# axruff/cuda-flow3d

Hardware: AMD Instinct MI355X
Metric: Mvoxels/s full pyramid solve (higher is better)
Workload: dtype f32; 1 GPU; 512^3 synthetic translated-Gaussian float32 pair (BASELINE config 4), full coarse-to-fine pyramid (40 levels x 40 outer x 5 inner, alpha 7.5, median 5^3, Gaussian sigma 2), frames resident in HBM (value = device-resident rate); parallelism=1 GPU

## Files before the change

### cuda-flow3d_amd/__init__.py

```python
import atexit
import contextlib
import ctypes as C
import os
import weakref

import numpy as np

_HERE = os.path.dirname(os.path.abspath(__file__))
_LIBDIR = os.environ.get("F3D_LIBDIR") or os.path.join(_HERE, "lib")

DEFAULT_PARAMS = dict(
    warp_levels_count=40, warp_scale_factor=0.95, outer_iterations_count=40, inner_iterations_count=5,
    equation_alpha=7.5, equation_smoothness=0.001, equation_data=0.001, median_radius=5, gaussian_sigma=2.0,
)


class F3dError(RuntimeError):
    pass


class Size4(C.Structure):
    _fields_ = [("width", C.c_size_t), ("height", C.c_size_t), ("depth", C.c_size_t), ("pitch", C.c_size_t)]


# ... 187 lines not shown
            raise
        fn.argtypes = args
        fn.restype = C.c_int
    _hip = L
    if hasattr(L, "f3d_crash_maps_enable"):
        _arm_crash_maps(L)
    return L


def _arm_crash_maps(L):
    path = os.environ.get("F3D_CRASH_MAPS")
    if not path:
        blob = " ".join(os.environ.get(k, "") for k in ("LD_PRELOAD", "ROCP_TOOL_LIBRARIES", "HSA_TOOLS_LIB"))
        if "rocprof" not in blob:
            return
        base = os.environ.get("F3D_OUT") or os.getcwd()
        path = os.path.join(base, f"f3d_crash_maps.{os.getpid()}.txt")
    L.f3d_crash_maps_enable(path.encode())


def host():
    global _host
    if _host is not None:
        return _host
    hip()
    L = _load("libf3d_host.so")
    pp = C.POINTER(FlowParams)
    sig = {
        "f3d_flow_create": [C.POINTER(C.c_void_p)], "f3d_flow_initialize": [C.c_void_p, _sz, _sz, _sz],
        "f3d_flow_compute": [C.c_void_p, _fp, _fp, pp, C.c_int, _fp, _fp, _fp],
        "f3d_flow_upload": [C.c_void_p, _fp, _fp],
        "f3d_flow_compute_resident": [C.c_void_p, pp, C.c_int, _fp],
        "f3d_flow_download": [C.c_void_p, _fp, _fp, _fp],
        "f3d_flow_container": [C.c_void_p, C.POINTER(Size4)], "f3d_flow_destroy": [C.c_void_p],
        "f3d_flow_set_level_stats": [C.c_void_p, C.c_int], "f3d_flow_level_stat_count": [C.c_void_p, C.POINTER(_sz)],
        "f3d_flow_level_stat": [C.c_void_p, _sz, C.POINTER(LevelStat)],
        "f3d_flow_final_residual": [C.c_void_p, C.POINTER(C.c_double), C.POINTER(C.c_double)],
        "f3d_flow_trajectory_begin": [C.c_void_p], "f3d_flow_trajectory_append": [C.c_void_p],
        "f3d_flow_trajectory_download": [C.c_void_p, _fp, _fp, _fp, C.POINTER(C.c_ulonglong)],
        "f3d_flow_trajectory_end": [C.c_void_p],
        "f3d_flow_strain_compute": [C.c_void_p, C.c_int, C.c_uint, C.POINTER(_fp), C.POINTER(StrainStats)],
        "f3d_flow_strain_end": [C.c_void_p],
        "f3d_flow_principal_compute": [C.c_void_p, C.c_int, C.c_uint, C.POINTER(_fp), C.POINTER(PrincipalStats)],
        "f3d_flow_principal_end": [C.c_void_p],
        "f3d_flow_inverse_compute": [C.c_void_p, C.c_int, C.c_uint, C.c_float, C.POINTER(_fp), C.POINTER(InverseStats)],
        "f3d_flow_inverse_end": [C.c_void_p],
        "f3d_flow_match_compute": [C.c_void_p, C.c_int, C.c_uint, C.c_uint, C.c_float, C.POINTER(_fp), C.POINTER(CorrelationStats)],
        "f3d_flow_match_end": [C.c_void_p],
        "f3d_motion_solve": [C.POINTER(MotionSums), C.c_int, C.POINTER(MotionFit)],
        "f3d_flow_motion_compute": [C.c_void_p, C.c_int, C.c_int, C.c_float, C.POINTER(_fp), C.POINTER(MotionFit),
                                    C.POINTER(MotionResidual)],
        "f3d_flow_motion_end": [C.c_void_p],
        "f3d_op_create": [C.POINTER(C.c_void_p), C.c_char_p], "f3d_op_initialize": [C.c_void_p, C.POINTER(Size4)],
        "f3d_op_execute": [C.c_void_p, C.POINTER(C.c_char_p), C.POINTER(C.c_void_p), _sz],
        "f3d_op_execute_batch": [C.c_void_p, C.POINTER(C.c_char_p), C.POINTER(C.c_void_p), C.POINTER(_sz), _sz],
        "f3d_op_set_slab": [C.c_void_p, _slabp], "f3d_op_destroy": [C.c_void_p],
        "f3d_level_geometry": [_sz, _sz, _sz, C.c_float, C.c_int, C.POINTER(Size4), _fp, _fp, _fp],
        "f3d_gaussian_taps": [C.c_float, _fp, _sz, C.POINTER(_sz)],
        "f3d_raw_read_u8": [C.c_char_p, _sz, _sz, _sz, _fp], "f3d_raw_read_f32": [C.c_char_p, _sz, _sz, _sz, _fp],
        "f3d_raw_write_u8": [C.c_char_p, _fp, _sz, _sz, _sz], "f3d_raw_write_f32": [C.c_char_p, _fp, _sz, _sz, _sz],
        "f3d_vtk_write_flow": [C.c_char_p, _fp, _fp, _fp, _sz, _sz, _sz],
        "f3d_synth_pair": [_sz, _sz, _sz, _fp, _fp],
        "f3d_synth_planes": [_sz, _sz, _sz, _sz, _sz, _fp, _fp, _fp],
        "f3d_slabflow_create": [C.POINTER(C.c_void_p), C.c_int, C.POINTER(C.c_int), C.c_int, C.c_int],
        "f3d_slabflow_initialize": [C.c_void_p, _sz, _sz, _sz],
        "f3d_slabflow_compute": [C.c_void_p, _fp, _fp, pp, _fp, _fp, _fp],
        "f3d_slabflow_upload": [C.c_void_p, _fp, _fp],
        "f3d_slabflow_compute_resident": [C.c_void_p, pp, _fp],
        "f3d_slabflow_download": [C.c_void_p, _fp, _fp, _fp],
        "f3d_slabflow_overlapped_iterations": [C.c_void_p, C.POINTER(_sz)],
        "f3d_slabflow_batched_exchanges": [C.c_void_p, C.POINTER(_sz)],
        "f3d_slabflow_gathered_warps": [C.c_void_p, C.POINTER(_sz)],
        "f3d_slabflow_stage_exchanges": [C.c_void_p, C.POINTER(_sz)],
        "f3d_slabflow_set_exchange_per_stage": [C.c_void_p, C.c_int],
        "f3d_slabflow_destroy": [C.c_void_p],
        "f3d_plan_owned": [C.c_int, C.c_int, C.c_int, C.POINTER(C.c_int), C.POINTER(C.c_int)],
        "f3d_plan_exchange": [C.c_int] * 5 + [C.POINTER(C.c_int)] * 5 + [C.c_int],
        "f3d_plan_resample_source": [C.c_int] * 4 + [C.POINTER(C.c_int)] * 2,
        "f3d_volume_wrap": [C.POINTER(C.c_void_p), _fp, _sz, _sz, _sz], "f3d_volume_destroy": [C.c_void_p],
        "f3d_op_solve_p_last": [C.c_void_p, C.POINTER(C.c_int), C.POINTER(C.c_int), C.POINTER(C.c_int), C.POINTER(_sz), C.POINTER(C.c_int)],
        "f3d_op_solve_p_fused_weights": [C.c_void_p, C.POINTER(C.c_int)],
        "f3d_plan_solve_piecemeal": [_sz, _sz, _sz, C.c_int, C.c_int, C.c_int, C.c_int, C.c_int] + [C.POINTER(C.c_int)] * 5,
        "f3d_pflow_create": [C.POINTER(C.c_void_p)], "f3d_pflow_initialize": [C.c_void_p, _sz, _sz, _sz],
        "f3d_pflow_compute": [C.c_void_p, _fp, _fp, _sz, _sz, _sz, pp, C.c_int, _fp, _fp, _fp, _fp],
        "f3d_pflow_stats": [C.c_void_p, C.POINTER(_sz), C.POINTER(_sz), C.POINTER(_sz)], "f3d_pflow_destroy": [C.c_void_p],
        "f3d_pflow_set_resident": [C.c_void_p, C.c_int], "f3d_pflow_set_full_pipeline": [C.c_void_p, C.c_int], "f3d_pflow_originals_on_device": [C.c_void_p, C.POINTER(C.c_int)],
        "f3d_pflow_operator_seconds": [C.c_void_p, C.POINTER(C.c_double)],
        "f3d_pflow_levels_registered_inside": [C.c_void_p, C.POINTER(_sz)],
        "f3d_pflow_levels_with_constants_on_device": [C.c_void_p, C.POINTER(_sz)],
        "f3d_host_shutdown": [],
    }
    for name, args in sig.items():
        try:
            fn = getattr(L, name)
        except AttributeError:
            if os.environ.get("F3D_LIBDIR"):
                continue
            raise
        fn.argtypes = args
        fn.restype = C.c_int
    L.f3d_flow_default_params.argtypes = [pp]
    L.f3d_flow_default_params.restype = None
    L.f3d_op_name.argtypes = [C.c_void_p]
    L.f3d_op_name.restype = C.c_char_p
    L.f3d_max_warp_level.argtypes = [_sz, _sz, _sz, C.c_float]
    L.f3d_max_warp_level.restype = _sz
    L.f3d_volume_object.argtypes = [C.c_void_p]
    L.f3d_volume_object.restype = C.c_void_p
    L.f3d_volume_data.argtypes = [C.c_void_p]
    L.f3d_volume_data.restype = C.c_void_p
    L.f3d_piecemeal_budget_bytes.argtypes = []
    L.f3d_piecemeal_budget_bytes.restype = _sz
    if hasattr(L, "f3d_host_last_error"):
        L.f3d_host_last_error.argtypes = []
        L.f3d_host_last_error.restype = C.c_char_p
    _host = L
    return L


def shutdown():
    HostVolume.release_all()
    if _host is not None:
        _host.f3d_host_shutdown()
    elif _hip is not None and _hip.f3d_is_initialized():
        _hip.f3d_comm_destroy()
        _hip.f3d_shutdown()


atexit.register(shutdown)


def check(status, what="f3d call"):
    if status != 0:
        msg = hip().f3d_last_error()
        raise F3dError(f"{what} failed: {msg.decode() if msg else 'status %d' % status}")


def _host_check(status, what):
    if status != 0:
        msg = host().f3d_host_last_error()
        raise F3dError(f"{what} failed: {msg.decode() if msg else 'status %d' % status}")


def _entry(name, argtypes, what):
    try:
        fn = getattr(hip(), name)
    except AttributeError:
        raise F3dError(f"{os.path.join(_LIBDIR, 'libf3d_hip.so')} has no {name}: this device library cannot {what}") from None
    fn.argtypes = argtypes
    fn.restype = C.c_int
    return fn


def _compose_entry():
    return _entry("f3d_compose_flow", [_dp] * 6 + [_sz] * 3 + [C.POINTER(C.c_ulonglong)], "compose flows into a trajectory")


def _strain_entry():
    return _entry("f3d_flow_strain", [_dp] * 3 + [_dpp, C.c_uint] + [_sz] * 3 + [C.POINTER(StrainStats)], "compute strain fields")


def _principal_entry():
    return _entry("f3d_principal_strain", [_dp] * 3 + [_dpp, C.c_uint] + [_sz] * 3 + [C.POINTER(PrincipalStats)],
                  "compute principal strains")


def _inverse_entry():
    return _entry("f3d_invert_displacement", [_dp] * 7 + [_sz] * 3 + [C.c_uint, C.c_float, C.POINTER(InverseStats)],
                  "invert displacements")


def _carry_entry():
    return _entry("f3d_carry_field", [_dp] * 5 + [_sz] * 3 + [C.c_uint, C.POINTER(C.c_ulonglong)],
                  "carry fields through a displacement")


def _correlation_entry():
    return _entry("f3d_local_correlation", [_dp] * 2 + [_dpp, C.c_uint, C.c_uint, C.c_float] + [_sz] * 3 + [C.POINTER(CorrelationStats)],
                  "compute the local correlation of two volumes")


def _motion_entry():
    what = "fit or remove the motion of a displacement"
    return (_entry("f3d_motion_sums", [_dp] * 4 + [C.c_float] + [_sz] * 3 + [C.POINTER(MotionSums)], what),
            _entry("f3d_remove_motion", [_dp] * 6 + [C.POINTER(MotionFit)] + [_sz] * 3 + [C.POINTER(MotionResidual)], what))


def _mask(fields, groups, what):
    if isinstance(fields, str):
        fields = fields.split(",")
    mask = 0
    for f in fields:
        if f not in groups:
            raise ValueError(f"unknown {what} group {f!r} (one of {', '.join(groups)})")
        mask |= groups[f]
    if not mask:
        raise ValueError(f"no {what} group selected")
    return mask


def _source(source):
    src = {"flow": 0, "trajectory": 1}.get(source)
    if src is None:
        raise ValueError(f"source must be 'flow' or 'trajectory', not {source!r}")
    return src


@contextlib.contextmanager
def _on_device(volumes, mismatch):
    vols = [np.ascontiguousarray(a, dtype=np.float32) for a in volumes]
    if any(a.ndim != 3 or a.shape != vols[0].shape for a in vols):
        raise ValueError(mismatch)
    d, h, w = vols[0].shape
    box = Containers(w, h, d)
    previous = Size4()
    check(hip().f3d_get_container(C.byref(previous)), "f3d_get_container")
    try:
        yield box, [box.new(a) for a in vols], (w, h, d)
    finally:
        if previous.pitch:
            hip().f3d_set_container(C.byref(previous))
        box.free()


def compose_flow(acc, inc):
    fn = _compose_entry()
    acc, inc = list(acc), list(inc)
    mismatch = "acc and inc must be three [z, y, x] volumes of one shape each"
    if len(acc) != 3 or len(inc) != 3:
        raise ValueError(mismatch)
    with _on_device(acc + inc, mismatch) as (box, p, dims):
        box.set_current()
        lost = C.c_ulonglong()
        check(fn(*p, *dims, C.byref(lost)), "f3d_compose_flow")
        return tuple(box.download(a, dims) for a in p[:3]) + (int(lost.value),)


STRAIN_NAMES = ("vol", "exx", "eyy", "ezz", "exy", "exz", "eyz", "eq")
STRAIN_GROUPS = {"vol": 1, "e": 2, "eq": 4}
_STRAIN_GROUP_OF = (1, 2, 2, 2, 2, 2, 2, 4)
PRINCIPAL_NAMES = ("e1", "e2", "e3", "gmax", "d1x", "d1y", "d1z", "d3x", "d3y", "d3z")
PRINCIPAL_GROUPS = {"val": 1, "shear": 2, "dir1": 4, "dir3": 8}
_PRINCIPAL_GROUP_OF = (1, 1, 1, 2, 4, 4, 4, 8, 8, 8)
INVERSE_NAMES = ("gu", "gv", "gw", "err")
CARRY_MODES = {"linear": 1, "nearest": 2}


MATCH_NAMES = ("warped", "zncc", "rmsd")
MATCH_GROUPS = {"warped": 1, "zncc": 2, "rmsd": 4}
CORRELATION_GROUPS = {"zncc": 1, "rmsd": 2}


MOTION_MODELS = {"translation": 0, "rigid": 1, "affine": 2}


def _motion_model(model):
    if model not in MOTION_MODELS:
        raise ValueError(f"unknown motion model {model!r} (one of {', '.join(MOTION_MODELS)})")
    return MOTION_MODELS[model]


def _strain_mask(fields):
    return _mask(fields, STRAIN_GROUPS, "strain")


def _principal_mask(fields):
    return _mask(fields, PRINCIPAL_GROUPS, "principal strain")


def _carry_mode(mode):
    if mode not in CARRY_MODES:
        raise ValueError(f"unknown carry mode {mode!r} (one of {', '.join(CARRY_MODES)})")
    return CARRY_MODES[mode]


def _grouped_fields(fn, what, u, v, w, mask, names, group_of, stats):
    with _on_device((u, v, w), "u, v and w must be three [z, y, x] volumes of one shape") as (box, p, dims):
        outs = [box.alloc() if mask & g else 0 for g in group_of]
        box.set_current()
        check(fn(*p, (_dp * len(outs))(*outs), mask, *dims, C.byref(stats)), what)
        res = {n: box.download(o, dims) for n, o in zip(names, outs) if o}
    res["stats"] = stats.as_dict()
    return res


def flow_strain(u, v, w, fields=("vol", "e", "eq")):
    fn = _strain_entry()
    return _grouped_fields(fn, "f3d_flow_strain", u, v, w, _strain_mask(fields), STRAIN_NAMES, _STRAIN_GROUP_OF, StrainStats())


def principal_strain(u, v, w, fields=("val", "shear")):
    fn = _principal_entry()
    return _grouped_fields(fn, "f3d_principal_strain", u, v, w, _principal_mask(fields), PRINCIPAL_NAMES, _PRINCIPAL_GROUP_OF,
                           PrincipalStats())


def invert_displacement(u, v, w, iterations=32, tolerance=1e-3):
    fn = _inverse_entry()
    with _on_device((u, v, w), "u, v and w must be three [z, y, x] volumes of one shape") as (box, p, dims):
        outs = [box.alloc() for _ in INVERSE_NAMES]
        box.set_current()
        stats = InverseStats()
        check(fn(*p, *outs, *dims, iterations, tolerance, C.byref(stats)), "f3d_invert_displacement")
        return tuple(box.download(o, dims) for o in outs) + (stats.as_dict(),)


# ... 215 lines not shown

    def release(self):
        hip().f3d_lane_make_current(None)

    def destroy(self):
        if self._h:
            hip().f3d_lane_destroy(self._h)
            self._h = C.c_void_p()

    def __enter__(self):
        self.make_current()
        return self

    def __exit__(self, *exc):
        self.release()
        self.destroy()
        return False


def mem_info():
    check(hip().f3d_init(-1), "f3d_init")
    free, total = _sz(), _sz()
    check(hip().f3d_mem_info(C.byref(free), C.byref(total)), "f3d_mem_info")
    return free.value, total.value



_PTR_KEYS = {
    "dev_frame_0", "dev_frame_1", "dev_flow_u", "dev_flow_v", "dev_flow_w", "dev_phi", "dev_ksi", "dev_flow_du",
    "dev_flow_dv", "dev_flow_dw", "dev_temp_du", "dev_temp_dv", "dev_temp_dw", "dev_input", "dev_output", "dev_temp",
    "operand_0", "operand_1",
}
_SIZE_T_KEYS = {"outer_iterations_count", "inner_iterations_count", "radius", "warp_levels_count", "median_radius"}
_FLOAT_KEYS = {"equation_alpha", "equation_smoothness", "equation_data", "hx", "hy", "hz", "gaussian_sigma",
               "warp_scale_factor"}
_SIZE4_KEYS = {"data_size", "resample_size", "container_size"}


class Stat3(C.Structure):
    _fields_ = [("min", C.c_float), ("max", C.c_float), ("avg", C.c_float)]


class HostVolume:
    _storage = {}

    def __init__(self, array, pin=False):
        a = np.ascontiguousarray(array, dtype=np.float32)
        if a.ndim != 3:
            raise ValueError("volume must be [z, y, x]")
        if pin and a.nbytes < (32 << 20):
            import mmap
            own = np.frombuffer(mmap.mmap(-1, max(a.nbytes, mmap.PAGESIZE)), dtype=np.float32, count=a.size).reshape(a.shape)
            own[...] = a
            a = own
        if a.ctypes.data in HostVolume._storage:
            raise ValueError("this array is already wrapped by another HostVolume")
        self._h = C.c_void_p()
        d, h, w = a.shape
        check(host().f3d_volume_wrap(C.byref(self._h), a.ctypes.data_as(_fp), w, h, d), "f3d_volume_wrap")
        entry = [a, False]
        HostVolume._storage[a.ctypes.data] = entry
        if pin:
            try:
                check(hip().f3d_init(-1), "f3d_init")
                check(hip().f3d_host_register(C.c_void_p(a.ctypes.data), a.nbytes), "f3d_host_register")
            except Exception:
                self.destroy()
                raise
            entry[1] = True
        self._finalizer = weakref.finalize(self, HostVolume._release, self._h.value)

    @staticmethod
    def _release(handle):
        if not handle or _host is None:
            return
        cur = _host.f3d_volume_data(C.c_void_p(handle))
        _host.f3d_volume_destroy(C.c_void_p(handle))
        entry = HostVolume._storage.pop(cur, None)
        if entry is not None and entry[1] and _hip is not None and _hip.f3d_is_initialized():
            _hip.f3d_host_unregister(C.c_void_p(cur))

    @classmethod
    def release_all(cls):
        for addr, entry in list(cls._storage.items()):
            if entry[1] and _hip is not None and _hip.f3d_is_initialized():
                _hip.f3d_host_unregister(C.c_void_p(addr))
            entry[1] = False

    @property
    def object(self):
        return host().f3d_volume_object(self._h)

    @property
    def array(self):
        return HostVolume._storage[host().f3d_volume_data(self._h)][0]

    def destroy(self):
        if self._h:
            fin = getattr(self, "_finalizer", None)
            if fin is not None:
                fin.detach()
            HostVolume._release(self._h.value)
            self._h = C.c_void_p()


def plan_solve_piecemeal(budget_bytes, width, height, depth, inner_iterations, outer_iterations, forced_outer_per_pass=0,
                         overlap_mode=0):
    out = [C.c_int() for _ in range(5)]
    check(host().f3d_plan_solve_piecemeal(budget_bytes, width, height, depth, inner_iterations, outer_iterations,
                                          forced_outer_per_pass, overlap_mode, *[C.byref(o) for o in out]))
    return tuple(o.value for o in out)


class Operation:

    def __init__(self, name):
        self._h = C.c_void_p()
        if host().f3d_op_create(C.byref(self._h), name.encode()) != 0:
            raise F3dError(f"unknown operation {name!r}")
        self.values = {}

    @property
    def name(self):
        return host().f3d_op_name(self._h).decode()

    def initialize(self, containers=None):
        if containers is None:
            return host().f3d_op_initialize(self._h, None) == 0
        s = containers.size4
        return host().f3d_op_initialize(self._h, C.byref(s)) == 0

    def set_slab(self, slab):
        self._slab = slab
        host().f3d_op_set_slab(self._h, C.byref(slab) if slab is not None else None)

    def execute(self, **params):
        store = {}
        volumes = {}
        for k, v in params.items():
            if isinstance(v, HostVolume):
                volumes[k] = v
            elif k in _PTR_KEYS:
                store[k] = _dp(v)
            elif k in _SIZE_T_KEYS:
                store[k] = _sz(v)
            elif k in _FLOAT_KEYS:
                store[k] = C.c_float(v)
            elif k in _SIZE4_KEYS:
                store[k] = Size4(v[0], v[1], v[2], 0) if not isinstance(v, Size4) else v
            elif k == "max_mag":
                store[k] = _sz(v)
            elif k == "stat":
                store[k] = v
            else:
                raise TypeError(f"unknown parameter key {k!r}")
        n = len(store) + len(volumes)
        keys = (C.c_char_p * n)(*[k.encode() for k in list(store) + list(volumes)])
        ptrs = (C.c_void_p * n)(*([C.cast(C.byref(v), C.c_void_p) for v in store.values()] +
                                  [C.c_void_p(v.object) for v in volumes.values()]))
        check(host().f3d_op_execute(self._h, keys, ptrs, n), "f3d_op_execute")
        self.values = {k: (v.value if hasattr(v, "value") else v) for k, v in store.items()}
        return self.values

    def execute_batch(self, bags):
        stores = []
        for params in bags:
            store = {}
            for k, v in params.items():
                if k in _PTR_KEYS:
                    store[k] = _dp(v)
                elif k in _SIZE_T_KEYS:
                    store[k] = _sz(v)
                elif k in _SIZE4_KEYS:
                    store[k] = Size4(v[0], v[1], v[2], 0) if not isinstance(v, Size4) else v
                else:
                    raise TypeError(f"unknown parameter key {k!r}")
            stores.append(store)
        n = sum(len(s) for s in stores)
        keys = (C.c_char_p * n)(*[k.encode() for s in stores for k in s])
        ptrs = (C.c_void_p * n)(*[C.cast(C.byref(v), C.c_void_p) for s in stores for v in s.values()])
        counts = (C.c_size_t * len(stores))(*[len(s) for s in stores])
        check(host().f3d_op_execute_batch(self._h, keys, ptrs, counts, len(stores)), "f3d_op_execute_batch")

    def solve_p_fused_weights(self):
        f = C.c_int()
        check(host().f3d_op_solve_p_fused_weights(self._h, C.byref(f)), "f3d_op_solve_p_fused_weights")
        return bool(f.value)

    def solve_p_last(self):
        c, n, h, p, o = C.c_int(), C.c_int(), C.c_int(), _sz(), C.c_int()
        check(host().f3d_op_solve_p_last(self._h, C.byref(c), C.byref(n), C.byref(h), C.byref(p), C.byref(o)), "f3d_op_solve_p_last")
        return c.value, n.value, h.value, p.value, bool(o.value)

    def destroy(self):
        if self._h:
            host().f3d_op_destroy(self._h)
            self._h = C.c_void_p()



class OpticalFlow:

    def __init__(self):
        self._h = C.c_void_p()
        check(host().f3d_flow_create(C.byref(self._h)), "f3d_flow_create")
        self.dims = None

    def initialize(self, width, height, depth):
        if host().f3d_flow_initialize(self._h, width, height, depth) != 0:
            raise F3dError("OpticalFlowE::Initialize failed: " + (hip().f3d_last_error() or b"").decode())
        self.dims = (width, height, depth)
        return True

    def compute(self, frame_0, frame_1, silent=True, out=None, **kw):
        f0, p0 = _f32(frame_0)
        f1, p1 = _f32(frame_1)
        w, h, d = self.dims
        if f0.shape != (d, h, w) or f1.shape != (d, h, w):
            raise ValueError(f"frames must be [z,y,x] = {(d, h, w)}")
        if out is None:
            u, v, ww = (np.empty((d, h, w), np.float32) for _ in range(3))
        else:
            u, v, ww = out
            for a in (u, v, ww):
                if a.dtype != np.float32 or a.shape != (d, h, w) or not a.flags["C_CONTIGUOUS"]:
                    raise ValueError(f"out arrays must be C-contiguous float32 [z,y,x] = {(d, h, w)}")
        prm = make_params(**kw)
        check(host().f3d_flow_compute(self._h, p0, p1, C.byref(prm), int(silent), u.ctypes.data_as(_fp),
                                      v.ctypes.data_as(_fp), ww.ctypes.data_as(_fp)), "f3d_flow_compute")
        return u, v, ww

    def upload(self, frame_0, frame_1):
        f0, p0 = _f32(frame_0)
        f1, p1 = _f32(frame_1)
        check(host().f3d_flow_upload(self._h, p0, p1), "f3d_flow_upload")

    def compute_resident(self, silent=True, **kw):
        prm = make_params(**kw)
        secs = C.c_float()
        check(host().f3d_flow_compute_resident(self._h, C.byref(prm), int(silent), C.byref(secs)),
              "f3d_flow_compute_resident")
        return secs.value

    def download(self):
        w, h, d = self.dims
        u, v, ww = (np.empty((d, h, w), np.float32) for _ in range(3))
        check(host().f3d_flow_download(self._h, u.ctypes.data_as(_fp), v.ctypes.data_as(_fp), ww.ctypes.data_as(_fp)))
        return u, v, ww

    def set_level_stats(self, enable=True):
        check(host().f3d_flow_set_level_stats(self._h, int(bool(enable))))

    def level_stats(self):
        n = _sz()
        check(host().f3d_flow_level_stat_count(self._h, C.byref(n)))
        out = []
        for i in range(n.value):
            st = LevelStat()
            check(host().f3d_flow_level_stat(self._h, i, C.byref(st)))
            out.append({k: getattr(st, k) for k, _ in LevelStat._fields_})
        return out

    def final_residual(self):
        a, b = (C.c_double * 3)(), (C.c_double * 3)()
        check(host().f3d_flow_final_residual(self._h, a, b), "f3d_flow_final_residual")
        return tuple(a), tuple(b)

    def trajectory_begin(self):
        _host_check(host().f3d_flow_trajectory_begin(self._h), "f3d_flow_trajectory_begin")

    def trajectory_append(self):
        _host_check(host().f3d_flow_trajectory_append(self._h), "f3d_flow_trajectory_append")

    def trajectory_download(self):
        w, h, d = self.dims
        u, v, ww = (np.empty((d, h, w), np.float32) for _ in range(3))
        lost = C.c_ulonglong()
        _host_check(host().f3d_flow_trajectory_download(self._h, u.ctypes.data_as(_fp), v.ctypes.data_as(_fp),
                                                        ww.ctypes.data_as(_fp), C.byref(lost)), "f3d_flow_trajectory_download")
        return u, v, ww, int(lost.value)

    def trajectory_end(self):
        _host_check(host().f3d_flow_trajectory_end(self._h), "f3d_flow_trajectory_end")

    def _derived(self, compute, src, selected, stats, *args, fit=None):
        w, h, d = self.dims
        arrays = [np.empty((d, h, w), np.float32) if s else None for s in selected]
        ptrs = (_fp * len(arrays))(*[a.ctypes.data_as(_fp) if a is not None else None for a in arrays])
        tail = (C.byref(stats),) if fit is None else (C.byref(fit), C.byref(stats))
        _host_check(getattr(host(), compute)(self._h, src, *args, ptrs, *tail), compute)
        return arrays

    def strain(self, source="flow", fields=("vol", "e", "eq")):
        src, mask, stats = _source(source), _strain_mask(fields), StrainStats()
        arrays = self._derived("f3d_flow_strain_compute", src, [mask & g for g in _STRAIN_GROUP_OF], stats, mask)
        res = {n: a for n, a in zip(STRAIN_NAMES, arrays) if a is not None}
        res["stats"] = stats.as_dict()
        return res

    def strain_end(self):
        _host_check(host().f3d_flow_strain_end(self._h), "f3d_flow_strain_end")

    def principal(self, source="flow", fields=("val", "shear")):
        src, mask, stats = _source(source), _principal_mask(fields), PrincipalStats()
        arrays = self._derived("f3d_flow_principal_compute", src, [mask & g for g in _PRINCIPAL_GROUP_OF], stats, mask)
        res = {n: a for n, a in zip(PRINCIPAL_NAMES, arrays) if a is not None}
# ... 256 lines not shown
```

### cuda-flow3d_amd/csrc/f3d_solve.hip

```cpp
#include <cmath>
#include <cstdio>
#include <algorithm>
#include <cstdlib>
#include <type_traits>

#include "f3d_internal.h"

namespace {

constexpr int kLanes = 64;

__device__ __forceinline__ float lane_left(float v)
{
  const int i = __builtin_bit_cast(int, v);
  return __builtin_bit_cast(float, __builtin_amdgcn_update_dpp(i, i, 0x138 , 0xf, 0xf, false));
}
__device__ __forceinline__ float lane_right(float v)
{
  const int i = __builtin_bit_cast(int, v);
  return __builtin_bit_cast(float, __builtin_amdgcn_update_dpp(i, i, 0x130 , 0xf, 0xf, false));
}

struct SolveArgs {
  const float* in[10];
// ... 110 lines not shown
  const float dux = q[0], duy = q[1], duz = q[2], dvx = q[3], dvy = q[4], dvz = q[5], dwx = q[6], dwy = q[7], dwz = q[8];

  phi = 1.f / (2.f * sqrtf(dux * dux + duy * duy + duz * duz + dvx * dvx + dvy * dvy + dvz * dvz + dwx * dwx +
                           dwy * dwy + dwz * dwz + eps_s * eps_s));

  const float fx = q[9], fy = q[10], fz = q[11];
  const float ft = n.c[F1] - n.c[F0];

  const float J11 = fx * fx, J22 = fy * fy, J33 = fz * fz;
  const float J12 = fx * fy, J13 = fx * fz, J23 = fy * fz;
  const float J14 = fx * ft, J24 = fy * ft, J34 = fz * ft, J44 = ft * ft;

  const float du = n.c[DU], dv_c = n.c[DV], dw = n.c[DW];
  float s = (J11 * du + J12 * dv_c + J13 * dw + J14) * du + (J12 * du + J22 * dv_c + J23 * dw + J24) * dv_c +
            (J13 * du + J23 * dv_c + J33 * dw + J34) * dw + (J14 * du + J24 * dv_c + J34 * dw + J44);
  s = static_cast<float>(s > 0) * s;
  ksi = 1.f / (2.f * sqrtf(s + eps_d * eps_d));
}

bool slab_reach_ok(const F3dGeo& g, int reach, const char* who)
{
  const int dc = static_cast<int>(f3d::container().depth);
  const int lo = g.z_lo - reach < 0 ? 0 : g.z_lo - reach;
  const int hi = g.z_hi + reach > g.D ? g.D : g.z_hi + reach;
  int need_lo = lo, need_hi = hi;
  if (g.z_lo - reach < 0 && reach + 1 > need_hi) need_hi = reach + 1 > g.D ? g.D : reach + 1;
  if (g.z_hi + reach > g.D && g.D - 1 - reach < need_lo) need_lo = g.D - 1 - reach < 0 ? 0 : g.D - 1 - reach;
  if (need_lo < g.z_base || need_hi - g.z_base > dc) {
    f3d::fail("%s: planes [%d,%d) needed but the container holds [%d,%d)", who, need_lo, need_hi, g.z_base,
              g.z_base + dc);
    return false;
  }
  return true;
}


__device__ __forceinline__ float lane_left_or(float v, float edge)
{
  return __builtin_bit_cast(float, __builtin_amdgcn_update_dpp(__builtin_bit_cast(int, edge), __builtin_bit_cast(int, v),
                                                               0x138 , 0xf, 0xf, false));
}
__device__ __forceinline__ float lane_right_or(float v, float edge)
{
  return __builtin_bit_cast(float, __builtin_amdgcn_update_dpp(__builtin_bit_cast(int, edge), __builtin_bit_cast(int, v),
                                                               0x130 , 0xf, 0xf, false));
}

constexpr int kTY3 = 8;
enum { LF0 = 0, LF1 = 1, LPHI = 2, LSU = 3, LSV = 4, LSW = 5, kNL = 6 };

struct Face6 {
  float v[kNL];
};

__device__ __forceinline__ void sweep_voxel_s(const Face6& xm, const Face6& xp, const Face6& ym, const Face6& yp,
                                              const Face6& zm, const Face6& zp, const float (&c)[kNL], float Uc, float Vc,
                                              float Wc, float dVc, float dWc, float ksi, float hx, float hy, float hz,
                                              float alpha, bool has_xp, bool has_xm, bool has_yp, bool has_ym, bool has_zp,
                                              bool has_zm, float& r_du, float& r_dv, float& r_dw)
{
  const float fx = (xp.v[LF0] - xm.v[LF0] + xp.v[LF1] - xm.v[LF1]) / (4.f * hx);
  const float fy = (yp.v[LF0] - ym.v[LF0] + yp.v[LF1] - ym.v[LF1]) / (4.f * hy);
  const float fz = (zp.v[LF0] - zm.v[LF0] + zp.v[LF1] - zm.v[LF1]) / (4.f * hz);
  const float ft = c[LF1] - c[LF0];

  const float J11 = fx * fx, J22 = fy * fy, J33 = fz * fz;
  const float J12 = fx * fy, J13 = fx * fz, J23 = fy * fz;
  const float J14 = fx * ft, J24 = fy * ft, J34 = fz * ft;

  const float hx_2 = alpha / (hx * hx);
  const float hy_2 = alpha / (hy * hy);
  const float hz_2 = alpha / (hz * hz);
  const float wxp = static_cast<float>(has_xp) * hx_2;
  const float wxm = static_cast<float>(has_xm) * hx_2;
  const float wyp = static_cast<float>(has_yp) * hy_2;
  const float wym = static_cast<float>(has_ym) * hy_2;
  const float wzp = static_cast<float>(has_zp) * hz_2;
  const float wzm = static_cast<float>(has_zm) * hz_2;

  const float phi_xp = (xp.v[LPHI] + c[LPHI]) / 2.f;
  const float phi_xm = (xm.v[LPHI] + c[LPHI]) / 2.f;
  const float phi_yp = (yp.v[LPHI] + c[LPHI]) / 2.f;
  const float phi_ym = (ym.v[LPHI] + c[LPHI]) / 2.f;
  const float phi_zp = (zp.v[LPHI] + c[LPHI]) / 2.f;
  const float phi_zm = (zm.v[LPHI] + c[LPHI]) / 2.f;

  const float sumH = (wxp * phi_xp + wxm * phi_xm + wyp * phi_yp + wym * phi_ym + wzp * phi_zp + wzm * phi_zm);
  const float sumU = phi_xp * wxp * (xp.v[LSU] - Uc) + phi_xm * wxm * (xm.v[LSU] - Uc) + phi_yp * wyp * (yp.v[LSU] - Uc) +
                     phi_ym * wym * (ym.v[LSU] - Uc) + phi_zp * wzp * (zp.v[LSU] - Uc) + phi_zm * wzm * (zm.v[LSU] - Uc);
  const float sumV = phi_xp * wxp * (xp.v[LSV] - Vc) + phi_xm * wxm * (xm.v[LSV] - Vc) + phi_yp * wyp * (yp.v[LSV] - Vc) +
                     phi_ym * wym * (ym.v[LSV] - Vc) + phi_zp * wzp * (zp.v[LSV] - Vc) + phi_zm * wzm * (zm.v[LSV] - Vc);
  const float sumW = phi_xp * wxp * (xp.v[LSW] - Wc) + phi_xm * wxm * (xm.v[LSW] - Wc) + phi_yp * wyp * (yp.v[LSW] - Wc) +
                     phi_ym * wym * (ym.v[LSW] - Wc) + phi_zp * wzp * (zp.v[LSW] - Wc) + phi_zm * wzm * (zm.v[LSW] - Wc);

  r_du = (ksi * (-J14 - J12 * dVc - J13 * dWc) + sumU) / (ksi * J11 + sumH);
  r_dv = (ksi * (-J24 - J12 * r_du - J23 * dWc) + sumV) / (ksi * J22 + sumH);
  r_dw = (ksi * (-J34 - J13 * r_du - J23 * r_dv) + sumW) / (ksi * J33 + sumH);
}

struct PlaneRegs {
  float f0, f1, phi, u, v, w, su, dv, dw, sv, sw, ksi;
  float fz, ft;
};

__device__ __forceinline__ void plane_finish(PlaneRegs& p)
{
  p.su = p.u + p.su;
  p.sv = p.v + p.dv;
  p.sw = p.w + p.dw;
}

__device__ __forceinline__ Face6 plane_face(const PlaneRegs& p)
{
  Face6 f;
  f.v[LF0] = p.f0; f.v[LF1] = p.f1; f.v[LPHI] = p.phi; f.v[LSU] = p.su; f.v[LSV] = p.sv; f.v[LSW] = p.sw;
  return f;
}

constexpr int kRing = 4;
typedef __attribute__((address_space(3))) float LdsFloat;

__device__ __forceinline__ float gld(const float* base, unsigned byte_off)
{
  float v;
  asm volatile("s_nop 4\n\tglobal_load_dword %0, %1, %2" : "=v"(v) : "v"(byte_off), "s"(base) : "memory");
  return v;
}
__device__ __forceinline__ void gst(float* base, unsigned byte_off, float v)
{
  asm volatile("s_nop 4\n\tglobal_store_dword %0, %1, %2 nt" ::"v"(byte_off), "v"(v), "s"(base) : "memory");
}
__device__ __forceinline__ void gld_lds(const float* base, unsigned byte_off, float* lds_dst)
{
  const unsigned m0v = static_cast<unsigned>(reinterpret_cast<unsigned long>((LdsFloat*)lds_dst));
  asm volatile("s_nop 4\n\tglobal_load_lds_dword %0, %1" ::"v"(byte_off), "s"(base), "{m0}"(m0v) : "memory");
}
__device__ __forceinline__ void gld_lds_lane(const float* lane_addr, float* lds_dst)
{
  const unsigned m0v = static_cast<unsigned>(reinterpret_cast<unsigned long>((LdsFloat*)lds_dst));
  asm volatile("s_nop 0\n\tglobal_load_lds_dword %0, off" ::"v"(lane_addr), "{m0}"(m0v) : "memory");
}
#define F3D_WAIT_PLANE(N, P)                                                                                           \
  do {                                                                                                                 \
    asm volatile("s_waitcnt vmcnt(" #N ")" ::: "memory");                                                              \
    asm volatile("; f3d_handback %0 %1 %2 %3 %4 %5 %6 %7 %8 %9"                                                        \
                 : "+v"((P).f0), "+v"((P).f1), "+v"((P).phi), "+v"((P).u), "+v"((P).v), "+v"((P).w), "+v"((P).su),     \
                   "+v"((P).dv), "+v"((P).dw), "+v"((P).ksi)::"memory");                                              \
  } while (0)

template <int ABLATE, int TY>
__global__ __launch_bounds__(kLanes* TY, 4) void k_sweep6(SolveArgs a, F3dGeo g, int zchunk, int ntx, int nty, int n_tiles,
                                                            int xcd_remap)
{
  __shared__ float img[2][kNL][TY + 2][kLanes];
  __shared__ float hrow[kRing][2][9][kLanes];
  __shared__ float hcol[kRing][TY][kLanes];

  int tile = static_cast<int>(blockIdx.x);
  if (xcd_remap) {
    const int per_xcd = (n_tiles + 7) / 8;
    tile = (tile % 8) * per_xcd + tile / 8;
  }
  if (tile >= n_tiles) return;
  const int tx = tile % ntx;
  const int ty = (tile / ntx) % nty;
  const int tz = tile / (ntx * nty);

  const int lane = threadIdx.x;
  const int r = __builtin_amdgcn_readfirstlane(static_cast<int>(threadIdx.y));
  const int z0 = g.z_lo + tz * zchunk;
  const int z1 = min(z0 + zchunk, g.z_hi);
  const int y0 = ty * TY;
  const int y = y0 + r;
  const int yy = f3d_clampi(f3d_mir(y, g.H), 0, g.H - 1);
  const int x = tx * kLanes + lane;
  const int xi = f3d_clampi(f3d_mir(x, g.W), 0, g.W - 1);
  const unsigned xb = static_cast<unsigned>(xi) * 4u;
  const bool owner = x < g.W && y < g.H;
  const int side = lane < 32 ? 0 : 1;
  const int xh = f3d_clampi(f3d_mir(side == 0 ? tx * kLanes - 1 : tx * kLanes + kLanes, g.W), 0, g.W - 1);
  const bool edge = (r == 0) || (r == TY - 1);
  const int which = r == 0 ? 0 : 1;
  const int yh_row = f3d_clampi(f3d_mir(r == 0 ? y0 - 1 : y0 + TY, g.H), 0, g.H - 1);
  const int lds_halo = r == 0 ? 0 : TY + 1;

  const int zb = z0 > 0 ? z0 - 1 : 0;
  const size_t base_off = f3d_row(g, 0, zb);
  const unsigned plane_b = static_cast<unsigned>(g.Hc) * static_cast<unsigned>(g.pitch) * 4u;
  const unsigned row_b = static_cast<unsigned>(g.pitch) * 4u;
  constexpr int kOrder[9] = {F0, F1, U, V, Wf, DU, DV, DW, PHI};
  const float* base[10];
#pragma unroll
  for (int i = 0; i < 10; ++i) base[i] = a.in[i] + base_off;
  float* obase[3];
#pragma unroll
  for (int i = 0; i < 3; ++i) obase[i] = a.out[i] + base_off;
  const bool col_lane = (lane & 31) < 9;
  const float* lane_base = base[0];
#pragma unroll
  for (int i = 1; i < 9; ++i)
    if ((lane & 31) == i) lane_base = base[kOrder[i]];
  lane_base += xh;

  auto rowoff = [&](int yrow, int zz) {
    return static_cast<unsigned>(__builtin_amdgcn_readfirstlane(
        static_cast<int>(static_cast<unsigned>(zz - zb) * plane_b + static_cast<unsigned>(yrow) * row_b)));
  };
  auto load_plane = [&](PlaneRegs& p, int zz) {
    const unsigned off = xb + rowoff(yy, zz);
    p.f0 = gld(base[F0], off);
    p.f1 = gld(base[F1], off);
    p.u = gld(base[U], off);
    p.v = gld(base[V], off);
    p.w = gld(base[Wf], off);
    p.su = gld(base[DU], off);
    p.dv = gld(base[DV], off);
    p.dw = gld(base[DW], off);
    p.phi = gld(base[PHI], off);
    p.ksi = gld(base[9], off);
  };
  auto dma_halos = [&](int zz) {
    const int slot = zz & (kRing - 1);
    if (col_lane) gld_lds_lane(lane_base + (rowoff(yy, zz) >> 2), &hcol[slot][r][0]);
    if (edge) {
      const unsigned off = xb + rowoff(yh_row, zz);
#pragma unroll
      for (int i = 0; i < 9; ++i) gld_lds(base[kOrder[i]], off, &hrow[slot][which][i][0]);
    }
  };
  auto ring_row = [&](PlaneRegs& p, int slot) {
    const float* d = &hrow[slot][which][0][lane];
    p.f0 = d[0 * kLanes]; p.f1 = d[1 * kLanes]; p.u = d[2 * kLanes]; p.v = d[3 * kLanes]; p.w = d[4 * kLanes];
    p.su = d[5 * kLanes]; p.dv = d[6 * kLanes]; p.dw = d[7 * kLanes]; p.phi = d[8 * kLanes];
  };
  auto ring_col = [&](PlaneRegs& p, int slot) {
    const float* d = &hcol[slot][r][side * 32];
    p.f0 = d[0]; p.f1 = d[1]; p.u = d[2]; p.v = d[3]; p.w = d[4]; p.su = d[5]; p.dv = d[6]; p.dw = d[7]; p.phi = d[8];
  };

  auto publish = [&](const PlaneRegs& pl, int nb, int ring_slot) {
    const Face6 f = plane_face(pl);
#pragma unroll
    for (int i = 0; i < kNL; ++i) img[nb][i][r + 1][lane] = f.v[i];
    if (edge) {
      PlaneRegs Hc;
      ring_row(Hc, ring_slot);
      plane_finish(Hc);
      const Face6 hf = plane_face(Hc);
#pragma unroll
      for (int i = 0; i < kNL; ++i) img[nb][i][lds_halo][lane] = hf.v[i];
    }
  };

  auto step = [&](auto full, const PlaneRegs& M, const PlaneRegs& C, const PlaneRegs& P, PlaneRegs& Q1, PlaneRegs& Q2, int z) {
    constexpr bool FULL = decltype(full)::value;
    const bool row3 = FULL || z + 3 <= z1;
    const bool halo3 = FULL || z + 3 < z1;
    if (row3) load_plane(Q2, f3d_mir(z + 3, g.D));
    if (halo3 && ABLATE != 2) dma_halos(z + 3);

    const int b = z & 1;
    const int slot = z & (kRing - 1);
    const Face6 cf = plane_face(C);
    if (ABLATE != 3) __syncthreads();

    Face6 ym, yp, xm, xp;
#pragma unroll
    for (int i = 0; i < kNL; ++i) {
      ym.v[i] = img[b][i][r][lane];
      yp.v[i] = img[b][i][r + 2][lane];
    }
    PlaneRegs X;
    ring_col(X, slot);
    if ((FULL || z + 1 < z1) && ABLATE != 3) publish(P, b ^ 1, (z + 1) & (kRing - 1));
    plane_finish(X);
    const Face6 xf = plane_face(X);
#pragma unroll
    for (int i = 0; i < kNL; ++i) {
      xm.v[i] = lane_left_or(cf.v[i], xf.v[i]);
      xp.v[i] = lane_right_or(cf.v[i], xf.v[i]);
    }
    float r_du, r_dv, r_dw;
    if (ABLATE == 1) {
      r_du = xm.v[0] + xp.v[1] + ym.v[2] + yp.v[3] + M.su + P.sv + C.ksi;
      r_dv = xm.v[4] + xp.v[5] + ym.v[0] + yp.v[1] + M.f0 + P.f1 + C.u;
      r_dw = xm.v[2] + xp.v[3] + ym.v[4] + yp.v[5] + M.phi + P.phi + C.dv + C.dw + C.v + C.w;
    } else {
      sweep_voxel_s(xm, xp, ym, yp, plane_face(M), plane_face(P), cf.v, C.u, C.v, C.w, C.dv, C.dw, C.ksi, a.hx, a.hy, a.hz,
                    a.p0, x < g.W - 1, x > 0, y < g.H - 1, y > 0, z < g.D - 1, z > 0, r_du, r_dv, r_dw);
    }
    asm volatile("" ::"v"(r_du), "v"(r_dv), "v"(r_dw));
    __builtin_amdgcn_sched_barrier(0);
    if (FULL && ABLATE == 2) {
      F3D_WAIT_PLANE(10, Q1);
    } else if (FULL) {
      if (edge) F3D_WAIT_PLANE(20, Q1);
      else F3D_WAIT_PLANE(11, Q1);
    } else {
      F3D_WAIT_PLANE(0, Q1);
    }
    if (FULL || z + 2 <= z1) plane_finish(Q1);
    __builtin_amdgcn_sched_barrier(0);
    if (owner) {
      const unsigned off = xb + rowoff(yy, z);
      gst(obase[0], off, r_du);
      gst(obase[1], off, r_dv);
      gst(obase[2], off, r_dw);
    }
    __builtin_amdgcn_sched_barrier(0);
  };

  PlaneRegs A, B, C, D, E;
  E = PlaneRegs{};
  D = PlaneRegs{};
  load_plane(A, f3d_mir(z0 - 1, g.D));
  load_plane(B, z0);
  load_plane(C, f3d_mir(z0 + 1, g.D));
  if (z0 + 2 <= z1) load_plane(D, f3d_mir(z0 + 2, g.D));
  dma_halos(z0);
  if (z0 + 1 < z1) dma_halos(z0 + 1);
  if (z0 + 2 < z1) dma_halos(z0 + 2);
  F3D_WAIT_PLANE(0, A);
  F3D_WAIT_PLANE(0, B);
  F3D_WAIT_PLANE(0, C);
  F3D_WAIT_PLANE(0, D);
  plane_finish(A);
  plane_finish(B);
  plane_finish(C);
  __syncthreads();
  publish(B, z0 & 1, z0 & (kRing - 1));
  __builtin_amdgcn_sched_barrier(0);
  int z = z0;
  for (; z + 7 < z1; z += 5) {
    step(std::true_type{}, A, B, C, D, E, z);
    step(std::true_type{}, B, C, D, E, A, z + 1);
    step(std::true_type{}, C, D, E, A, B, z + 2);
    step(std::true_type{}, D, E, A, B, C, z + 3);
    step(std::true_type{}, E, A, B, C, D, z + 4);
  }
  for (; z < z1; z += 5) {
    step(std::false_type{}, A, B, C, D, E, z);
    if (z + 1 < z1) step(std::false_type{}, B, C, D, E, A, z + 1);
    if (z + 2 < z1) step(std::false_type{}, C, D, E, A, B, z + 2);
    if (z + 3 < z1) step(std::false_type{}, D, E, A, B, C, z + 3);
    if (z + 4 < z1) step(std::false_type{}, E, A, B, C, D, z + 4);
  }
  asm volatile("s_waitcnt vmcnt(0)" ::: "memory");
}

struct Plane8 {
  float v[8];
};

#define F3D_WAIT_PLANE8(N, P)                                                                                          \
  do {                                                                                                                 \
    asm volatile("s_waitcnt vmcnt(" #N ")" ::: "memory");                                                              \
    asm volatile("; f3d_handback %0 %1 %2 %3 %4 %5 %6 %7"                                                              \
                 : "+v"((P).v[0]), "+v"((P).v[1]), "+v"((P).v[2]), "+v"((P).v[3]), "+v"((P).v[4]), "+v"((P).v[5]),     \
                   "+v"((P).v[6]), "+v"((P).v[7])::"memory");                                                         \
  } while (0)

__global__ __launch_bounds__(kLanes* kTY3, 4) void k_phiksi6(SolveArgs a, F3dGeo g, int zchunk, int ntx, int nty, int n_tiles,
                                                             int xcd_remap)
{
  constexpr int NA = 8;
  __shared__ float img[2][NA][kTY3 + 2][kLanes];
  __shared__ float hrow[kRing][2][NA][kLanes];
  __shared__ float hcol[kRing][kTY3][kLanes];
  SolveDivs divs = make_solve_divs(a.hx, a.hy, a.hz);
  divs.ok = divs.ok && !a.plain_division;

  int tile = static_cast<int>(blockIdx.x);
  if (xcd_remap) {
    const int per_xcd = (n_tiles + 7) / 8;
    tile = (tile % 8) * per_xcd + tile / 8;
  }
  if (tile >= n_tiles) return;
  const int tx = tile % ntx;
  const int ty = (tile / ntx) % nty;
  const int tz = tile / (ntx * nty);

  const int lane = threadIdx.x;
  const int r = __builtin_amdgcn_readfirstlane(static_cast<int>(threadIdx.y));
  const bool second = a.z2_hi > a.z2_lo && tz >= a.nz_first;
  const int z0 = second ? a.z2_lo + (tz - a.nz_first) * zchunk : g.z_lo + tz * zchunk;
  const int z1 = min(z0 + zchunk, second ? a.z2_hi : g.z_hi);
  const int y0 = ty * kTY3;
  const int y = y0 + r;
  const int yy = f3d_clampi(f3d_mir(y, g.H), 0, g.H - 1);
  const int x = tx * kLanes + lane;
  const int xi = f3d_clampi(f3d_mir(x, g.W), 0, g.W - 1);
  const unsigned xb = static_cast<unsigned>(xi) * 4u;
  const bool owner = x < g.W && y < g.H;
  const int side = lane < 32 ? 0 : 1;
  const int xh = f3d_clampi(f3d_mir(side == 0 ? tx * kLanes - 1 : tx * kLanes + kLanes, g.W), 0, g.W - 1);
  const bool edge = (r == 0) || (r == kTY3 - 1);
  const int which = r == 0 ? 0 : 1;
  const int yh_row = f3d_clampi(f3d_mir(r == 0 ? y0 - 1 : y0 + kTY3, g.H), 0, g.H - 1);
  const int lds_halo = r == 0 ? 0 : kTY3 + 1;

  const int zb = z0 > 0 ? z0 - 1 : 0;
  const size_t base_off = f3d_row(g, 0, zb);
  const unsigned plane_b = static_cast<unsigned>(g.Hc) * static_cast<unsigned>(g.pitch) * 4u;
  const unsigned row_b = static_cast<unsigned>(g.pitch) * 4u;
  const float* base[NA];
#pragma unroll
  for (int i = 0; i < NA; ++i) base[i] = a.in[i] + base_off;
  float* obase[2] = {a.out[0] + base_off, a.out[1] + base_off};
  const bool col_lane = (lane & 31) < NA;
  const float* lane_base = base[0];
#pragma unroll
  for (int i = 1; i < NA; ++i)
    if ((lane & 31) == i) lane_base = base[i];
  lane_base += xh;

  auto rowoff = [&](int yrow, int zz) {
    return static_cast<unsigned>(__builtin_amdgcn_readfirstlane(
        static_cast<int>(static_cast<unsigned>(zz - zb) * plane_b + static_cast<unsigned>(yrow) * row_b)));
  };
  auto load_plane = [&](Plane8& p, int zz) {
    const unsigned off = xb + rowoff(yy, zz);
#pragma unroll
    for (int i = 0; i < NA; ++i) p.v[i] = gld(base[i], off);
  };
  auto dma_halos = [&](int zz) {
    const int slot = zz & (kRing - 1);
    if (col_lane) gld_lds_lane(lane_base + (rowoff(yy, zz) >> 2), &hcol[slot][r][0]);
    if (edge) {
      const unsigned off = xb + rowoff(yh_row, zz);
#pragma unroll
      for (int i = 0; i < NA; ++i) gld_lds(base[i], off, &hrow[slot][which][i][0]);
    }
  };
  auto publish = [&](const Plane8& pl, int nb, int ring_slot) {
#pragma unroll
    for (int i = 0; i < NA; ++i) img[nb][i][r + 1][lane] = pl.v[i];
    if (edge) {
#pragma unroll
      for (int i = 0; i < NA; ++i) img[nb][i][lds_halo][lane] = hrow[ring_slot][which][i][lane];
    }
  };

  auto step = [&](auto full, const Plane8& M, const Plane8& C, const Plane8& P, Plane8& Q1, Plane8& Q2, int z) {
    constexpr bool FULL = decltype(full)::value;
    const bool row3 = FULL || z + 3 <= z1;
    const bool halo3 = FULL || z + 3 < z1;
    if (row3) load_plane(Q2, f3d_mir(z + 3, g.D));
    if (halo3) dma_halos(z + 3);

    const int b = z & 1;
    const int slot = z & (kRing - 1);
    __syncthreads();

    Hood<8> n;
    float xcol[NA];
#pragma unroll
    for (int i = 0; i < NA; ++i) {
      n.c[i] = C.v[i];
      n.ym[i] = img[b][i][r][lane];
      n.yp[i] = img[b][i][r + 2][lane];
      n.zm[i] = M.v[i];
      n.zp[i] = P.v[i];
      xcol[i] = hcol[slot][r][side * 32 + i];
    }
    if (FULL || z + 1 < z1) publish(P, b ^ 1, (z + 1) & (kRing - 1));
#pragma unroll
    for (int i = 0; i < NA; ++i) {
      n.xm[i] = lane_left_or(C.v[i], xcol[i]);
      n.xp[i] = lane_right_or(C.v[i], xcol[i]);
    }
    float phi, ksi;
    phi_ksi_voxel(n, divs, a.p0, a.p1, phi, ksi);
    asm volatile("" ::"v"(phi), "v"(ksi));
    __builtin_amdgcn_sched_barrier(0);
    if (FULL) {
      if (edge) F3D_WAIT_PLANE8(17, Q1);
      else F3D_WAIT_PLANE8(9, Q1);
    } else {
      F3D_WAIT_PLANE8(0, Q1);
    }
    __builtin_amdgcn_sched_barrier(0);
    if (owner) {
      const unsigned off = xb + rowoff(yy, z);
      gst(obase[0], off, phi);
      gst(obase[1], off, ksi);
    }
    __builtin_amdgcn_sched_barrier(0);
  };

  Plane8 A, B, C, D, E;
  D = Plane8{};
  E = Plane8{};
  load_plane(A, f3d_mir(z0 - 1, g.D));
  load_plane(B, z0);
  load_plane(C, f3d_mir(z0 + 1, g.D));
  if (z0 + 2 <= z1) load_plane(D, f3d_mir(z0 + 2, g.D));
  dma_halos(z0);
  if (z0 + 1 < z1) dma_halos(z0 + 1);
  if (z0 + 2 < z1) dma_halos(z0 + 2);
  F3D_WAIT_PLANE8(0, A);
// ... 323 lines not shown

    if (ABL & 8) {
      asm volatile("" ::"v"(r_du), "v"(r_dv), "v"(r_dw));
      __builtin_amdgcn_sched_barrier(0);
      tk[3] = __builtin_amdgcn_s_memtime();
    }
    const int t = q - 1;
    const bool do2 = core && t >= z0;
    float o_du = 0.f, o_dv = 0.f, o_dw = 0.f;
    if (do2) {
      const int pb = t & 1;
      S3 ym, yp, xm, xp, zm, zp;
      ym.u = img1[pb][0][r - 1][lane]; ym.v = img1[pb][1][r - 1][lane]; ym.w = img1[pb][2][r - 1][lane];
      yp.u = img1[pb][0][r + 1][lane]; yp.v = img1[pb][1][r + 1][lane]; yp.w = img1[pb][2][r + 1][lane];
      const float eu = hc1[pb][0][side][r - 1], ev = hc1[pb][1][side][r - 1], ew = hc1[pb][2][side][r - 1];
      xm.u = lane_left_or(hC.u, eu); xm.v = lane_left_or(hC.v, ev); xm.w = lane_left_or(hC.w, ew);
      xp.u = lane_right_or(hC.u, eu); xp.v = lane_right_or(hC.v, ev); xp.w = lane_right_or(hC.w, ew);
      zm = hM;
      zp = sN;
      if (tile_at_x_face) {
        if (x == 0) xm = xp;
        if (x == g.W - 1) xp = xm;
      }
      if (y == 0) ym = yp;
      if (y == g.H - 1) yp = ym;
      if (t == 0) zm = zp;
      if (t == g.D - 1) zp = zm;
      if (ABL & 2) {
        o_du = xm.u + xp.v + ym.w + kC.J12;
        o_dv = yp.u + zm.v + zp.w + kC.d1;
        o_dw = xm.w + yp.v + zp.u + kC.pw[0] + hC_dv + hC_dw;
      } else
      sweep_stage2(kC, xm, xp, ym, yp, zm, zp, hC_dv, hC_dw, o_du, o_dv, o_dw);
    }
    asm volatile("" ::"v"(o_du), "v"(o_dv), "v"(o_dw), "v"(sN.u), "v"(sN.v), "v"(sN.w));
    hM = hC;
    hC = sN;
    hC_dv = r_dv;
    hC_dw = r_dw;
    kC = kN;
    __builtin_amdgcn_sched_barrier(0);
    if (ABL & 8) tk[4] = __builtin_amdgcn_s_memtime();
    if (!colw) {
      F3D_WAIT_PLANE(0, Q);
      plane_finish(Q);
    }
    __builtin_amdgcn_sched_barrier(0);
    if (ABL & 8) tk[5] = __builtin_amdgcn_s_memtime();
    if (do2 && owner) {
      const unsigned off = xb + rowoff(yy, t);
      gst(obase[0], off, o_du);
      gst(obase[1], off, o_dv);
      gst(obase[2], off, o_dw);
    }
    __builtin_amdgcn_sched_barrier(0);
    if (ABL & 8) {
      tk[6] = __builtin_amdgcn_s_memtime();
#pragma unroll
      for (int i = 0; i < 6; ++i) pr[i] += tk[i + 1] - tk[i];
    }
  };

  PlaneRegs A = {}, B = {}, C = {}, D = {};
  if (!colw) {
    load_plane(A, f3d_mir(qs - 1, g.D));
    load_plane(B, qs);
    load_plane(C, f3d_mir(qs + 1, g.D));
    dma_halos(qs - 1);
    dma_halos(qs);
    dma_halos(qs + 1);
    F3D_WAIT_PLANE(0, A);
    F3D_WAIT_PLANE(0, B);
    F3D_WAIT_PLANE(0, C);
    plane_finish(A);
    plane_finish(B);
    plane_finish(C);
  }
  __syncthreads();
  if (colw) {
    col_raw(A, qs - 1, crow + 1, 1);
    col_raw(B, qs, crow + 1, 1);
    plane_finish(A);
    plane_finish(B);
  } else {
    publish(B, qs);
  }
  __builtin_amdgcn_sched_barrier(0);
  int q = qs;
  for (; q + 3 <= q_end; q += 4) {
    step(A, B, C, D, q);
    step(B, C, D, A, q + 1);
    step(C, D, A, B, q + 2);
    step(D, A, B, C, q + 3);
  }
  if (q <= q_end) step(A, B, C, D, q);
  if (q + 1 <= q_end) step(B, C, D, A, q + 1);
  if (q + 2 <= q_end) step(C, D, A, B, q + 2);
  asm volatile("s_waitcnt vmcnt(0)" ::: "memory");
  if ((ABL & 8) && a.probe && lane == 0) {
#pragma unroll
    for (int i = 0; i < 6; ++i) atomicAdd(&a.probe[r * 8 + i], pr[i]);
    atomicAdd(&a.probe[r * 8 + 6], static_cast<unsigned long long>(q_end - qs + 1));
  }
}

struct Tuning {
  int xcd_remap;
  int zchunk;
  long want_wg;
};

const Tuning& tuning()
{
  static const Tuning t = [] {
    Tuning v = {1, 0, 4096};
    if (const char* e = std::getenv("F3D_XCD_REMAP")) v.xcd_remap = std::atoi(e);
    if (const char* e = std::getenv("F3D_ZCHUNK")) v.zchunk = std::atoi(e);
    if (const char* e = std::getenv("F3D_WANT_WG")) v.want_wg = std::atol(e);
    return v;
  }();
  return t;
}

inline int max_planes_per_chunk(const F3dGeo& g)
{
  static const bool off = std::getenv("F3D_CHUNK_LIMIT") && std::atoi(std::getenv("F3D_CHUNK_LIMIT")) == 0;
  if (off) return 0x3fffffff;
  const unsigned long long plane_bytes = static_cast<unsigned long long>(g.Hc) * static_cast<unsigned long long>(g.pitch) * 4ull;
  const long long planes = static_cast<long long>(0xffffffffull / plane_bytes) - 8;
  return planes < 1 ? 1 : (planes > 0x3fffffff ? 0x3fffffff : static_cast<int>(planes));
}

__global__ __launch_bounds__(256) void k_frame_derivatives(const float* __restrict__ f0, const float* __restrict__ f1, F3dGeo g, float hx,
                                                           float hy, float hz, float* __restrict__ fx, float* __restrict__ fy,
                                                           float* __restrict__ fz, float* __restrict__ ft)
{
  const int x = blockIdx.x * 64 + threadIdx.x;
  const int y = blockIdx.y * 4 + threadIdx.y;
  const int z = g.z_lo + blockIdx.z;
  if (x >= g.W || y >= g.H) return;
  const size_t c = f3d_row(g, y, z) + x;
  const size_t xm = f3d_row(g, y, z) + f3d_mir(x - 1, g.W), xp = f3d_row(g, y, z) + f3d_mir(x + 1, g.W);
  const size_t ym = f3d_row(g, f3d_mir(y - 1, g.H), z) + x, yp = f3d_row(g, f3d_mir(y + 1, g.H), z) + x;
  const size_t zm = f3d_row(g, y, f3d_mir(z - 1, g.D)) + x, zp = f3d_row(g, y, f3d_mir(z + 1, g.D)) + x;
  fx[c] = (f0[xp] - f0[xm] + f1[xp] - f1[xm]) / (4.f * hx);
  fy[c] = (f0[yp] - f0[ym] + f1[yp] - f1[ym]) / (4.f * hy);
  fz[c] = (f0[zp] - f0[zm] + f1[zp] - f1[zm]) / (4.f * hz);
  ft[c] = f1[c] - f0[c];
}

#include "f3d_solve_pair8.h"
#include "f3d_solve_tri.h"

template <bool SWEEP>
void launch_solver(const SolveArgs& args, const F3dGeo& g)
{
  const Tuning& t = tuning();
  const int planes = g.z_hi - g.z_lo;
  const int ntx = (g.W + kLanes - 1) / kLanes;
  const int nty = (g.H + kTY3 - 1) / kTY3;
  long nzc = (t.want_wg + static_cast<long>(ntx) * nty - 1) / (static_cast<long>(ntx) * nty);
  const long max_chunks = planes / 4 > 0 ? planes / 4 : 1;
  if (nzc > max_chunks) nzc = max_chunks;
  if (nzc < 1) nzc = 1;
  int zchunk = static_cast<int>((planes + nzc - 1) / nzc);
  const long tiles_xy = static_cast<long>(ntx) * nty;
  if (tiles_xy * planes <= 4096) {
    double best = -1.0;
    for (int zc = 1; zc <= planes; ++zc) {
      const long wgs = tiles_xy * ((planes + zc - 1) / zc);
      const double cost = static_cast<double>((wgs + 511) / 512) * (zc + 4.5);
      if (best < 0.0 || cost < best) {
        best = cost;
        zchunk = zc;
      }
    }
  }
  else if (planes <= 128) {
    const long chunks = std::max<long>(1, (512 + tiles_xy - 1) / tiles_xy);
    zchunk = static_cast<int>((planes + chunks - 1) / chunks);
  }
  if (t.zchunk > 0) zchunk = t.zchunk;
  zchunk = std::min(zchunk, max_planes_per_chunk(g));
  SolveArgs a = args;
  int nz = (planes + zchunk - 1) / zchunk;
  if (!SWEEP && a.z2_hi > a.z2_lo) {
    a.nz_first = nz;
    nz += (a.z2_hi - a.z2_lo + zchunk - 1) / zchunk;
  }
  const int n_tiles = ntx * nty * nz;
  const int per_xcd = (n_tiles + 7) / 8;
  const int blocks = t.xcd_remap ? per_xcd * 8 : n_tiles;
  const dim3 grid(blocks, 1, 1), block(kLanes, kTY3, 1);
  auto go = [&](auto kern) { hipLaunchKernelGGL(kern, grid, block, 0, f3d::stream(), a, g, zchunk, ntx, nty, n_tiles, t.xcd_remap); };
  if constexpr (SWEEP) {
#ifdef F3D_LAB
    static const int ablate = std::getenv("F3D_ABLATE") ? std::atoi(std::getenv("F3D_ABLATE")) : 0;
    if (ablate == 1) return go(k_sweep6<1, kTY3>);
    if (ablate == 2) return go(k_sweep6<2, kTY3>);
    if (ablate == 3) return go(k_sweep6<3, kTY3>);
#endif
    go(k_sweep6<0, kTY3>);
  } else {
    go(k_phiksi6);
  }
}

template <int TY>
void launch_sweep2_ty(const SolveArgs& a, const F3dGeo& g, long want_wg, int force_zchunk, int xcd_remap)
{
  const int planes = g.z_hi - g.z_lo;
  const int ntx = (g.W + kLanes - 1) / kLanes;
  const int nty = (g.H + TY - 1) / TY;
  const long tiles = static_cast<long>(ntx) * nty;
  const int max_chunks = planes / 2 > 0 ? planes / 2 : 1;
  const int zc_limit = max_planes_per_chunk(g);
  int zchunk = std::min(planes, zc_limit);
  if (want_wg > 0) {
    long nzc = (want_wg + tiles - 1) / tiles;
    if (nzc > max_chunks) nzc = max_chunks;
    if (nzc < 1) nzc = 1;
    zchunk = static_cast<int>((planes + nzc - 1) / nzc);
  } else {
    long best = -1;
    for (int nzc = 1; nzc <= max_chunks; ++nzc) {
      const int zc = (planes + nzc - 1) / nzc;
      if (zc > zc_limit) continue;
      const long wgs = tiles * ((planes + zc - 1) / zc);
      const long cost = ((wgs + 255) / 256) * (zc + 6);
      if (best < 0 || cost < best) {
        best = cost;
        zchunk = zc;
      }
    }
  }
  if (force_zchunk > 0) zchunk = force_zchunk;
  zchunk = std::min(zchunk, zc_limit);
  const int nz = (planes + zchunk - 1) / zchunk;
  const int n_tiles = ntx * nty * nz;
  const int per_xcd = (n_tiles + 7) / 8;
  const int blocks = xcd_remap ? per_xcd * 8 : n_tiles;
  const dim3 grid(blocks, 1, 1), block(kLanes, TY + 3, 1);
  auto go = [&](auto kern) { hipLaunchKernelGGL(kern, grid, block, 0, f3d::stream(), a, g, zchunk, ntx, nty, n_tiles, xcd_remap); };
#ifdef F3D_LAB
  static const int abl = std::getenv("F3D_ABLATE7") ? std::atoi(std::getenv("F3D_ABLATE7")) : 0;
  if constexpr (TY == 9) {
    if (abl == 1) return go(k_sweep7<TY, 1>);
    if (abl == 2) return go(k_sweep7<TY, 2>);
    if (abl == 3) return go(k_sweep7<TY, 3>);
    if (abl == 4) return go(k_sweep7<TY, 4>);
    if (abl == 7) return go(k_sweep7<TY, 7>);
    if (abl == 8) {
      static unsigned long long* probe = nullptr;
      if (!probe) (void)hipMalloc(reinterpret_cast<void**>(&probe), 16 * 8 * sizeof(unsigned long long));
      (void)hipMemsetAsync(probe, 0, 16 * 8 * sizeof(unsigned long long), f3d::stream());
      SolveArgs ap = a;
      ap.probe = probe;
      hipLaunchKernelGGL((k_sweep7<TY, 8>), grid, block, 0, f3d::stream(), ap, g, zchunk, ntx, nty, n_tiles, xcd_remap);
      unsigned long long h[16 * 8];
      (void)hipMemcpyAsync(h, probe, sizeof(h), hipMemcpyDeviceToHost, f3d::stream());
      (void)hipStreamSynchronize(f3d::stream());
      static int shown = 0;
      if (shown++ < 1) {
        std::fprintf(stderr, "k_sweep7 probe (avg cycles per step): wave  issue  barrier  stage1  stage2  vmwait  store\n");
        for (int w = 0; w < TY + 3; ++w) {
          const double n = static_cast<double>(h[w * 8 + 6]);
          std::fprintf(stderr, "  %2d  %7.0f %7.0f %7.0f %7.0f %7.0f %7.0f   (%.0f steps)\n", w, h[w * 8] / n, h[w * 8 + 1] / n,
                       h[w * 8 + 2] / n, h[w * 8 + 3] / n, h[w * 8 + 4] / n, h[w * 8 + 5] / n, n);
        }
      }
      return;
    }
  }
#endif
  go(k_sweep7<TY, 0>);
}

int pair8_enabled()
{
  static const int v = std::getenv("F3D_PAIR8") ? std::atoi(std::getenv("F3D_PAIR8")) : 1;
  return v;
}

PairArgs pair_args(const SolveArgs& a)
{
  PairArgs p = {};
  for (int i = 0; i < 10; ++i) p.in[i] = a.in[i];
  for (int i = 0; i < 3; ++i) p.out[i] = a.out[i];
  p.hx = a.hx; p.hy = a.hy; p.hz = a.hz;
  p.alpha = a.p0;
  p.plain_division = a.plain_division;
  return p;
}

int pair8_rows(const F3dGeo& g)
{
  const char* forced_env = std::getenv("F3D_PAIR8_TY");
  const int forced = forced_env ? std::atoi(forced_env) : 0;
  static const long step12 = std::getenv("F3D_PAIR8_STEP12") ? std::atol(std::getenv("F3D_PAIR8_STEP12")) : 128;
  if (forced == 4 || forced == 8 || forced == 12) return forced;
  const long c8 = pair8_plan(g, 8).cost * 100, c12 = pair8_plan(g, 12).cost * step12;
  static const long step4 = std::getenv("F3D_PAIR8_STEP4") ? std::atol(std::getenv("F3D_PAIR8_STEP4")) : 80;
  if (pair8_plan(g, 4).cost * step4 < std::min(c8, c12)) return 4;
  return c12 < c8 ? 12 : 8;
}

void launch_sweep2(const SolveArgs& a, const F3dGeo& g)
{
  const Tuning& t = tuning();
  if (pair8_enabled() && g.pitch % kLanes == 0) {
    if (launch_pair8_ymarch<PAIR_SS>(pair_args(a), g, t.zchunk, t.xcd_remap)) return;
    const int ty = pair8_rows(g);
    if (ty == 4) launch_pair8<PAIR_SS, 4>(pair_args(a), g, t.zchunk, t.xcd_remap);
    else if (ty == 12) launch_pair8<PAIR_SS, 12>(pair_args(a), g, t.zchunk, t.xcd_remap);
    else launch_pair8<PAIR_SS, 8>(pair_args(a), g, t.zchunk, t.xcd_remap);
    return;
  }
  static const int ty = std::getenv("F3D_SWEEP2_TY") ? std::atoi(std::getenv("F3D_SWEEP2_TY")) : 9;
  static const long want = std::getenv("F3D_SWEEP2_WG") ? std::atol(std::getenv("F3D_SWEEP2_WG")) : 0;
  if (ty == 8) launch_sweep2_ty<8>(a, g, want, t.zchunk, t.xcd_remap);
  else if (ty == 5) launch_sweep2_ty<5>(a, g, want, t.zchunk, t.xcd_remap);
  else launch_sweep2_ty<9>(a, g, want, t.zchunk, t.xcd_remap);
}


int tri_rows(const F3dGeo& g)
{
  const char* forced_env = std::getenv("F3D_TRI_TY");
  const int forced = forced_env ? std::atoi(forced_env) : 0;
  if (forced == 4 || forced == 7) return forced;
  static const long step4 = std::getenv("F3D_TRI_STEP4") ? std::atol(std::getenv("F3D_TRI_STEP4")) : 80;
  const int planes = g.z_hi - g.z_lo;
  const long c4 = tri_plan_dims(g.W, g.H, planes, 4, max_planes_per_chunk(g)).cost * step4;
  const long c7 = tri_plan_dims(g.W, g.H, planes, 7, max_planes_per_chunk(g)).cost * 100;
  return c4 < c7 ? 4 : 7;
}

int tri_launch(const char* who, bool with_weights, const f3d_devptr (&in)[10], size_t width, size_t height, size_t depth, float hx, float hy,
               float hz, float alpha, float eps_s, float eps_d, const f3d_devptr (&out)[5], const f3d_slab* slab)
{
  F3dGeo g;
  if (!f3d::make_geo(&g, width, height, depth, slab, who)) return 1;
  if (g.W < 2 || g.H < 2 || g.D < 2) return f3d::fail("%s: every dimension must be at least 2", who);
  if (!pair_weights_finite(hx, hy, hz, alpha))
    return f3d::fail("%s: alpha / h^2 must be finite and not negative (alpha %g, h %g %g %g)", who, alpha, hx, hy, hz);
  if (g.pitch % kLanes != 0) return f3d::fail("%s: the container pitch must be a multiple of 256 bytes (f3d_alloc_pitched gives that)", who);
  for (int i = 0; i < (with_weights ? 5 : 3); ++i)
    for (int k = 0; k < 10; ++k)
      if (out[i] == in[k]) return f3d::fail("%s: an output buffer is also an input (other tiles still read it)", who);
  if (g.z_lo == g.z_hi) return 0;
  if (!slab_reach_ok(g, 3, who)) return 1;
  PairArgs a = {};
  static const int plain_division = std::getenv("F3D_UDIV") && std::atoi(std::getenv("F3D_UDIV")) == 0;
  a.plain_division = plain_division;
  for (int i = 0; i < 10; ++i) a.in[i] = f3d_ptr<const float>(in[i]);
  for (int i = 0; i < 5; ++i) a.out[i] = f3d_ptr<float>(out[i]);
  a.hx = hx; a.hy = hy; a.hz = hz;
  a.alpha = alpha;
  a.eps_s = eps_s;
  a.eps_d = eps_d;
  const int kid = with_weights ? F3D_K_SWEEP2_PHI_KSI : F3D_K_SWEEP3;
  f3d::prof_begin(kid, static_cast<size_t>(g.W) * g.H * (g.z_hi - g.z_lo));
  const int rows = tri_rows(g);
  if (with_weights) {
    if (rows == 4) launch_tri<TRI_SSP, 4>(a, g, tuning().zchunk, tuning().xcd_remap);
    else launch_tri<TRI_SSP, 7>(a, g, tuning().zchunk, tuning().xcd_remap);
  } else {
    if (rows == 4) launch_tri<TRI_SSS, 4>(a, g, tuning().zchunk, tuning().xcd_remap);
    else launch_tri<TRI_SSS, 7>(a, g, tuning().zchunk, tuning().xcd_remap);
  }
  f3d::prof_end(kid);
  F3D_HIP(hipGetLastError());
  return 0;
}

}

extern "C" {

int f3d_phi_ksi(f3d_devptr frame_0, f3d_devptr frame_1, f3d_devptr flow_u, f3d_devptr flow_v, f3d_devptr flow_w,
                f3d_devptr flow_du, f3d_devptr flow_dv, f3d_devptr flow_dw, size_t width, size_t height,
                size_t depth, float hx, float hy, float hz, float equation_smoothness, float equation_data,
                f3d_devptr phi, f3d_devptr ksi, const f3d_slab* slab)
{
  F3D_REQUIRE_READY("f3d_phi_ksi");
  F3dGeo g;
  if (!f3d::make_geo(&g, width, height, depth, slab, "f3d_phi_ksi")) return 1;
  if (g.W < 2 || g.H < 2 || g.D < 2) return f3d::fail("f3d_phi_ksi: every dimension must be at least 2");
  if (g.z_lo == g.z_hi) return 0;
  if (!slab_reach_ok(g, 1, "f3d_phi_ksi")) return 1;
  SolveArgs a;
  static const int plain_division = std::getenv("F3D_UDIV") && std::atoi(std::getenv("F3D_UDIV")) == 0;
  a.plain_division = plain_division;
  const f3d_devptr in[8] = {frame_0, frame_1, flow_u, flow_v, flow_w, flow_du, flow_dv, flow_dw};
  for (int i = 0; i < 8; ++i) a.in[i] = f3d_ptr<const float>(in[i]);
  a.in[8] = a.in[9] = nullptr;
  a.out[0] = f3d_ptr<float>(phi);
  a.out[1] = f3d_ptr<float>(ksi);
  a.out[2] = nullptr;
  a.hx = hx; a.hy = hy; a.hz = hz;
  a.p0 = equation_smoothness;
  a.p1 = equation_data;
  f3d::prof_begin(F3D_K_PHI_KSI, static_cast<size_t>(g.W) * g.H * (g.z_hi - g.z_lo));
  launch_solver<false>(a, g);
  f3d::prof_end(F3D_K_PHI_KSI);
  F3D_HIP(hipGetLastError());
  return 0;
}

int f3d_phi_ksi_zones(f3d_devptr frame_0, f3d_devptr frame_1, f3d_devptr flow_u, f3d_devptr flow_v, f3d_devptr flow_w,
                      f3d_devptr flow_du, f3d_devptr flow_dv, f3d_devptr flow_dw, size_t width, size_t height, size_t depth, float hx,
                      float hy, float hz, float equation_smoothness, float equation_data, f3d_devptr phi, f3d_devptr ksi,
                      const f3d_slab* zone_a, const f3d_slab* zone_b)
{
  F3D_REQUIRE_READY("f3d_phi_ksi_zones");
  if (!zone_a || !zone_b) return f3d::fail("f3d_phi_ksi_zones: two windows are required");
  if (zone_a->z_base != zone_b->z_base) return f3d::fail("f3d_phi_ksi_zones: both windows must address the same container planes (z_base)");
  F3dGeo g, g2;
  if (!f3d::make_geo(&g, width, height, depth, zone_a, "f3d_phi_ksi_zones")) return 1;
  if (!f3d::make_geo(&g2, width, height, depth, zone_b, "f3d_phi_ksi_zones")) return 1;
  if (g.W < 2 || g.H < 2 || g.D < 2) return f3d::fail("f3d_phi_ksi_zones: every dimension must be at least 2");
  if (g.z_lo == g.z_hi || g2.z_lo == g2.z_hi)
    return f3d_phi_ksi(frame_0, frame_1, flow_u, flow_v, flow_w, flow_du, flow_dv, flow_dw, width, height, depth, hx, hy, hz,
                       equation_smoothness, equation_data, phi, ksi, g.z_lo == g.z_hi ? zone_b : zone_a);
  if (!(g.z_hi <= g2.z_lo || g2.z_hi <= g.z_lo)) return f3d::fail("f3d_phi_ksi_zones: the windows overlap");
  if (!slab_reach_ok(g, 1, "f3d_phi_ksi_zones") || !slab_reach_ok(g2, 1, "f3d_phi_ksi_zones")) return 1;
  SolveArgs a;
  static const int plain_division = std::getenv("F3D_UDIV") && std::atoi(std::getenv("F3D_UDIV")) == 0;
  a.plain_division = plain_division;
  const f3d_devptr in[8] = {frame_0, frame_1, flow_u, flow_v, flow_w, flow_du, flow_dv, flow_dw};
  for (int i = 0; i < 8; ++i) a.in[i] = f3d_ptr<const float>(in[i]);
  a.in[8] = a.in[9] = nullptr;
  a.out[0] = f3d_ptr<float>(phi);
  a.out[1] = f3d_ptr<float>(ksi);
  a.out[2] = nullptr;
  a.hx = hx; a.hy = hy; a.hz = hz;
  a.p0 = equation_smoothness;
  a.p1 = equation_data;
  a.z2_lo = g2.z_lo;
  a.z2_hi = g2.z_hi;
  f3d::prof_begin(F3D_K_PHI_KSI, static_cast<size_t>(g.W) * g.H * (g.z_hi - g.z_lo + g2.z_hi - g2.z_lo));
  launch_solver<false>(a, g);
  f3d::prof_end(F3D_K_PHI_KSI);
  F3D_HIP(hipGetLastError());
  return 0;
}

int f3d_solve_sweep(f3d_devptr frame_0, f3d_devptr frame_1, f3d_devptr flow_u, f3d_devptr flow_v, f3d_devptr flow_w,
                    f3d_devptr flow_du, f3d_devptr flow_dv, f3d_devptr flow_dw, f3d_devptr phi, f3d_devptr ksi,
                    size_t width, size_t height, size_t depth, float hx, float hy, float hz, float equation_alpha,
                    f3d_devptr temp_du, f3d_devptr temp_dv, f3d_devptr temp_dw, const f3d_slab* slab)
{
  F3D_REQUIRE_READY("f3d_solve_sweep");
  F3dGeo g;
  if (!f3d::make_geo(&g, width, height, depth, slab, "f3d_solve_sweep")) return 1;
  if (g.W < 2 || g.H < 2 || g.D < 2) return f3d::fail("f3d_solve_sweep: every dimension must be at least 2");
  if (g.z_lo == g.z_hi) return 0;
  if (!slab_reach_ok(g, 1, "f3d_solve_sweep")) return 1;
  SolveArgs a;
  static const int plain_division = std::getenv("F3D_UDIV") && std::atoi(std::getenv("F3D_UDIV")) == 0;
  a.plain_division = plain_division;
  const f3d_devptr in[10] = {frame_0, frame_1, flow_u, flow_v, flow_w, flow_du, flow_dv, flow_dw, phi, ksi};
  for (int i = 0; i < 10; ++i) a.in[i] = f3d_ptr<const float>(in[i]);
  a.out[0] = f3d_ptr<float>(temp_du);
  a.out[1] = f3d_ptr<float>(temp_dv);
  a.out[2] = f3d_ptr<float>(temp_dw);
  a.hx = hx; a.hy = hy; a.hz = hz;
  a.p0 = equation_alpha;
  a.p1 = 0.f;
  f3d::prof_begin(F3D_K_SWEEP, static_cast<size_t>(g.W) * g.H * (g.z_hi - g.z_lo));
  launch_solver<true>(a, g);
  f3d::prof_end(F3D_K_SWEEP);
  F3D_HIP(hipGetLastError());
  return 0;
}

int f3d_solve_sweep2(f3d_devptr frame_0, f3d_devptr frame_1, f3d_devptr flow_u, f3d_devptr flow_v, f3d_devptr flow_w,
                     f3d_devptr flow_du, f3d_devptr flow_dv, f3d_devptr flow_dw, f3d_devptr phi, f3d_devptr ksi,
                     size_t width, size_t height, size_t depth, float hx, float hy, float hz, float equation_alpha,
                     f3d_devptr temp_du, f3d_devptr temp_dv, f3d_devptr temp_dw, const f3d_slab* slab)
{
  F3D_REQUIRE_READY("f3d_solve_sweep2");
  F3dGeo g;
  if (!f3d::make_geo(&g, width, height, depth, slab, "f3d_solve_sweep2")) return 1;
  if (g.W < 2 || g.H < 2 || g.D < 2) return f3d::fail("f3d_solve_sweep2: every dimension must be at least 2");
  if (!pair_weights_finite(hx, hy, hz, equation_alpha))
    return f3d::fail("f3d_solve_sweep2: alpha / h^2 must be finite and not negative (alpha %g, h %g %g %g)", equation_alpha, hx, hy, hz);
  if (g.z_lo == g.z_hi) return 0;
  if (!slab_reach_ok(g, 2, "f3d_solve_sweep2")) return 1;
  SolveArgs a;
  static const int plain_division = std::getenv("F3D_UDIV") && std::atoi(std::getenv("F3D_UDIV")) == 0;
  a.plain_division = plain_division;
  const f3d_devptr in[10] = {frame_0, frame_1, flow_u, flow_v, flow_w, flow_du, flow_dv, flow_dw, phi, ksi};
  for (int i = 0; i < 10; ++i) a.in[i] = f3d_ptr<const float>(in[i]);
  a.out[0] = f3d_ptr<float>(temp_du);
  a.out[1] = f3d_ptr<float>(temp_dv);
  a.out[2] = f3d_ptr<float>(temp_dw);
  a.hx = hx; a.hy = hy; a.hz = hz;
  a.p0 = equation_alpha;
  a.p1 = 0.f;
  f3d::prof_begin(F3D_K_SWEEP2, static_cast<size_t>(g.W) * g.H * (g.z_hi - g.z_lo));
  launch_sweep2(a, g);
  f3d::prof_end(F3D_K_SWEEP2);
  F3D_HIP(hipGetLastError());
  return 0;
}

int f3d_solve_sweep_phi_ksi_edges(f3d_devptr frame_0, f3d_devptr frame_1, f3d_devptr flow_u, f3d_devptr flow_v, f3d_devptr flow_w,
                                  f3d_devptr flow_du, f3d_devptr flow_dv, f3d_devptr flow_dw, f3d_devptr phi, f3d_devptr ksi,
                                  size_t width, size_t height, size_t depth, float hx, float hy, float hz, float equation_alpha,
                                  float equation_smoothness, float equation_data, f3d_devptr temp_du, f3d_devptr temp_dv,
                                  f3d_devptr temp_dw, f3d_devptr phi_next, f3d_devptr ksi_next, const f3d_slab* slab,
                                  int keep_below, int keep_above)
{
  F3D_REQUIRE_READY("f3d_solve_sweep_phi_ksi");
  F3dGeo g;
  if (!f3d::make_geo(&g, width, height, depth, slab, "f3d_solve_sweep_phi_ksi")) return 1;
  if (g.W < 2 || g.H < 2 || g.D < 2) return f3d::fail("f3d_solve_sweep_phi_ksi: every dimension must be at least 2");
  if (!pair_weights_finite(hx, hy, hz, equation_alpha))
    return f3d::fail("f3d_solve_sweep_phi_ksi: alpha / h^2 must be finite and not negative (alpha %g, h %g %g %g)", equation_alpha, hx, hy, hz);
  if (phi_next == phi || ksi_next == ksi || phi_next == ksi || ksi_next == phi)
    return f3d::fail("f3d_solve_sweep_phi_ksi: phi_next / ksi_next must not alias phi / ksi (other tiles still read them)");
  if (g.pitch % kLanes != 0)
    return f3d::fail("f3d_solve_sweep_phi_ksi: the container pitch must be a multiple of 256 bytes (f3d_alloc_pitched gives that)");
  if (g.z_lo == g.z_hi) return 0;
  if (!slab_reach_ok(g, 2, "f3d_solve_sweep_phi_ksi")) return 1;
  PairArgs a = {};
  a.keep_below = keep_below != 0;
  a.keep_above = keep_above != 0;
  static const int plain_division = std::getenv("F3D_UDIV") && std::atoi(std::getenv("F3D_UDIV")) == 0;
  a.plain_division = plain_division;
  const f3d_devptr in[10] = {frame_0, frame_1, flow_u, flow_v, flow_w, flow_du, flow_dv, flow_dw, phi, ksi};
  for (int i = 0; i < 10; ++i) a.in[i] = f3d_ptr<const float>(in[i]);
  a.out[0] = f3d_ptr<float>(temp_du);
  a.out[1] = f3d_ptr<float>(temp_dv);
  a.out[2] = f3d_ptr<float>(temp_dw);
  a.out[3] = f3d_ptr<float>(phi_next);
  a.out[4] = f3d_ptr<float>(ksi_next);
  a.hx = hx; a.hy = hy; a.hz = hz;
  a.alpha = equation_alpha;
  a.eps_s = equation_smoothness;
  a.eps_d = equation_data;
  f3d::prof_begin(F3D_K_SWEEP_PHI_KSI, static_cast<size_t>(g.W) * g.H * (g.z_hi - g.z_lo));
  if (!a.keep_below && !a.keep_above && launch_pair8_ymarch<PAIR_SP>(a, g, tuning().zchunk, tuning().xcd_remap)) {}
  else if (pair8_rows(g) == 4) launch_pair8<PAIR_SP, 4>(a, g, tuning().zchunk, tuning().xcd_remap);
  else if (pair8_rows(g) == 12) launch_pair8<PAIR_SP, 12>(a, g, tuning().zchunk, tuning().xcd_remap);
  else launch_pair8<PAIR_SP, 8>(a, g, tuning().zchunk, tuning().xcd_remap);
  f3d::prof_end(F3D_K_SWEEP_PHI_KSI);
  F3D_HIP(hipGetLastError());
  return 0;
}

int f3d_solve_sweep_phi_ksi(f3d_devptr frame_0, f3d_devptr frame_1, f3d_devptr flow_u, f3d_devptr flow_v, f3d_devptr flow_w,
                            f3d_devptr flow_du, f3d_devptr flow_dv, f3d_devptr flow_dw, f3d_devptr phi, f3d_devptr ksi,
                            size_t width, size_t height, size_t depth, float hx, float hy, float hz, float equation_alpha,
                            float equation_smoothness, float equation_data, f3d_devptr temp_du, f3d_devptr temp_dv,
                            f3d_devptr temp_dw, f3d_devptr phi_next, f3d_devptr ksi_next, const f3d_slab* slab)
{
  return f3d_solve_sweep_phi_ksi_edges(frame_0, frame_1, flow_u, flow_v, flow_w, flow_du, flow_dv, flow_dw, phi, ksi, width, height,
                                       depth, hx, hy, hz, equation_alpha, equation_smoothness, equation_data, temp_du, temp_dv,
                                       temp_dw, phi_next, ksi_next, slab, 0, 0);
}

namespace {
struct WeightTally {
  unsigned long long checked, excluded, mismatches;
  unsigned first[4];
};
__global__ __launch_bounds__(256) void k_selftest_weights(unsigned lo, unsigned hi, WeightTally* t)
{
  const unsigned long long stride = static_cast<unsigned long long>(gridDim.x) * blockDim.x;
  unsigned long long checked = 0, excluded = 0;
  for (unsigned long long i = lo + static_cast<unsigned long long>(blockIdx.x) * blockDim.x + threadIdx.x; i <= hi; i += stride) {
    const float a = __uint_as_float(static_cast<unsigned>(i));
    float s;
    const float fast = weight_fast(a, s);
    if (!weight_fast_ok(a, s)) {
      ++excluded;
      continue;
    }
    ++checked;
    if (__float_as_uint(fast) != __float_as_uint(weight_ieee(a))) {
      const unsigned long long n = atomicAdd(&t->mismatches, 1ull);
      if (n < 4) t->first[n] = static_cast<unsigned>(i);
    }
  }
  atomicAdd(&t->checked, checked);
  atomicAdd(&t->excluded, excluded);
}
}

int f3d_selftest_weights(unsigned lo_bits, unsigned hi_bits, unsigned long long* checked, unsigned long long* excluded,
                         unsigned long long* mismatches, unsigned* first_mismatch)
{
  F3D_REQUIRE_READY("f3d_selftest_weights");
  if (lo_bits > hi_bits) return f3d::fail("f3d_selftest_weights: empty range");
  WeightTally* d = nullptr;
  F3D_HIP(hipMalloc(reinterpret_cast<void**>(&d), sizeof(WeightTally)));
  F3D_HIP(hipMemsetAsync(d, 0, sizeof(WeightTally), f3d::stream()));
  hipLaunchKernelGGL(k_selftest_weights, dim3(256 * 16), dim3(256), 0, f3d::stream(), lo_bits, hi_bits, d);
  WeightTally h;
  F3D_HIP(hipMemcpyAsync(&h, d, sizeof(h), hipMemcpyDeviceToHost, f3d::stream()));
  F3D_HIP(hipStreamSynchronize(f3d::stream()));
  F3D_HIP(hipFree(d));
  if (checked) *checked = h.checked;
  if (excluded) *excluded = h.excluded;
  if (mismatches) *mismatches = h.mismatches;
  if (first_mismatch) *first_mismatch = h.mismatches ? h.first[0] : 0u;
  return 0;
}

int f3d_frame_derivatives(f3d_devptr frame_0, f3d_devptr frame_1, size_t width, size_t height, size_t depth, float hx, float hy,
                          float hz, f3d_devptr fx, f3d_devptr fy, f3d_devptr fz, f3d_devptr ft, const f3d_slab* slab)
{
  F3D_REQUIRE_READY("f3d_frame_derivatives");
  F3dGeo g;
  if (!f3d::make_geo(&g, width, height, depth, slab, "f3d_frame_derivatives")) return 1;
  if (g.W < 2 || g.H < 2 || g.D < 2) return f3d::fail("f3d_frame_derivatives: every dimension must be at least 2");
  for (f3d_devptr o : {fx, fy, fz, ft})
    if (o == frame_0 || o == frame_1) return f3d::fail("f3d_frame_derivatives: an output aliases a frame");
  if (g.z_lo == g.z_hi) return 0;
  if (!slab_reach_ok(g, 1, "f3d_frame_derivatives")) return 1;
  const dim3 grid((g.W + 63) / 64, (g.H + 3) / 4, g.z_hi - g.z_lo), block(64, 4, 1);
  hipLaunchKernelGGL(k_frame_derivatives, grid, block, 0, f3d::stream(), f3d_ptr<const float>(frame_0), f3d_ptr<const float>(frame_1), g, hx,
                     hy, hz, f3d_ptr<float>(fx), f3d_ptr<float>(fy), f3d_ptr<float>(fz), f3d_ptr<float>(ft));
  F3D_HIP(hipGetLastError());
  return 0;
// ... 120 lines not shown
```

### cuda-flow3d_amd/csrc/f3d_stream_ops.hip

```cpp
#include <cstring>

#include "f3d_internal.h"

#include <cstdint>

namespace {

constexpr int kBX = 64;
constexpr int kBY = 4;

inline dim3 grid_for(int w, int h, int planes) { return dim3((w + kBX - 1) / kBX, (h + kBY - 1) / kBY, planes); }

constexpr int kMaxBatch = 3;
struct Vols {
  const float* in[kMaxBatch];
  float* out[kMaxBatch];
};

__global__ __launch_bounds__(kBX* kBY) void k_warp(const float* __restrict__ f0, const float* __restrict__ f1,
                                                   const float* __restrict__ u, const float* __restrict__ v,
                                                   const float* __restrict__ w, float* __restrict__ out, F3dGeo g,
                                                   float hx, float hy, float hz)
{
  const int x = blockIdx.x * kBX + threadIdx.x;
  const int y = blockIdx.y * kBY + threadIdx.y;
  const int z = g.z_lo + blockIdx.z;
  if (x >= g.W || y >= g.H) return;
  const size_t c = f3d_row(g, y, z) + x;
  const float x_f = static_cast<float>(x) + (u[c] * (1.f / hx));
  const float y_f = static_cast<float>(y) + (v[c] * (1.f / hy));
  const float z_f = static_cast<float>(z) + (w[c] * (1.f / hz));
  if ((x_f < 0.f) || (x_f > static_cast<float>(g.W - 1)) || (y_f < 0.f) || (y_f > static_cast<float>(g.H - 1)) ||
      (z_f < 0.f) || (z_f > static_cast<float>(g.D - 1)) || isnan(x_f) || isnan(y_f) || isnan(z_f)) {
    out[c] = f0[c];
    return;
  }
  const int xi = static_cast<int>(floorf(x_f));
  const int yi = static_cast<int>(floorf(y_f));
  const int zi = static_cast<int>(floorf(z_f));
  const float dx = x_f - static_cast<float>(xi);
  const float dy = y_f - static_cast<float>(yi);
  const float dz = z_f - static_cast<float>(zi);
  const int x1 = min(g.W - 1, xi + 1);
  const int y1 = min(g.H - 1, yi + 1);
  const int z1 = min(g.D - 1, zi + 1);
  const size_t r00 = f3d_row(g, yi, zi), r10 = f3d_row(g, y1, zi);
  const size_t r01 = f3d_row(g, yi, z1), r11 = f3d_row(g, y1, z1);
  const float v0 = (1.f - dx) * (1.f - dy) * f1[r00 + xi] + (dx) * (1.f - dy) * f1[r00 + x1] +
                   (1.f - dx) * (dy)*f1[r10 + xi] + (dx) * (dy)*f1[r10 + x1];
  const float v1 = (1.f - dx) * (1.f - dy) * f1[r01 + xi] + (dx) * (1.f - dy) * f1[r01 + x1] +
                   (1.f - dx) * (dy)*f1[r11 + xi] + (dx) * (dy)*f1[r11 + x1];
  out[c] = (1.f - dz) * v0 + dz * v1;
}

template <int AXIS>
__global__ __launch_bounds__(kBX* kBY) void k_resample(Vols v, F3dGeo gi, F3dGeo g, int in_n, float delta, float normalization)
{
  const float* __restrict__ in = v.in[blockIdx.x];
  float* __restrict__ out = v.out[blockIdx.x];
  const int y = blockIdx.y * kBY + threadIdx.y;
  const int z = g.z_lo + blockIdx.z;
  if (y >= g.H) return;
  float left_f = 0.f, right_f = 0.f;
  int left_i = 0, cnt = 0;
  auto window = [&](int i) {
    left_f = static_cast<float>(i) * delta;
    right_f = static_cast<float>(i + 1) * delta;
    left_i = static_cast<int>(floorf(left_f));
    const int right_i = static_cast<int>(fminf(static_cast<float>(in_n), ceilf(right_f)));
    cnt = right_i - left_i;
  };
  if (AXIS != 0) window(AXIS == 1 ? y : z);
  const size_t out_row = f3d_row(g, y, z);
  const size_t in_row = AXIS == 0 ? f3d_row(gi, y, z) : 0;
  for (int x = threadIdx.x; x < g.W; x += kBX) {
    if (AXIS == 0) window(x);
    float value = 0.f;
    for (int j = 0; j < cnt; ++j) {
      float frac = 1.f;
      if (j == 0) frac = static_cast<float>(left_i + 1) - left_f;
      if (j == cnt - 1) frac = right_f - static_cast<float>(left_i + j);
      if (cnt == 1) frac = delta;
      const int s = left_i + j;
      const size_t a = AXIS == 0 ? in_row + s : (AXIS == 1 ? f3d_row(gi, s, z) + x : f3d_row(gi, y, s) + x);
      value = value + in[a] * frac;
    }
    out[out_row + x] = value * normalization;
  }
}

constexpr int kResampleRowMax = 2048;
__global__ __launch_bounds__(kBX* kBY) void k_resample_x_lds(Vols v, F3dGeo gi, F3dGeo g, int in_n, float delta, float normalization)
{
  __shared__ __attribute__((aligned(16))) float rowbuf[kBY][kResampleRowMax];
  const float* __restrict__ in = v.in[blockIdx.x];
  float* __restrict__ out = v.out[blockIdx.x];
  const int y = blockIdx.y * kBY + threadIdx.y;
  const int z = g.z_lo + blockIdx.z;
  if (y >= g.H) return;
  float* row = rowbuf[threadIdx.y];
  const float* src = in + f3d_row(gi, y, z);
  for (int k = threadIdx.x * 4; k < in_n; k += kBX * 4) *reinterpret_cast<float4*>(row + k) = *reinterpret_cast<const float4*>(src + k);
  __builtin_amdgcn_fence(__ATOMIC_RELEASE, "wavefront");
  __builtin_amdgcn_wave_barrier();
  __builtin_amdgcn_fence(__ATOMIC_ACQUIRE, "wavefront");
  const size_t out_row = f3d_row(g, y, z);
  for (int x = threadIdx.x; x < g.W; x += kBX) {
    const float left_f = static_cast<float>(x) * delta;
    const float right_f = static_cast<float>(x + 1) * delta;
    const int left_i = static_cast<int>(floorf(left_f));
    const int right_i = static_cast<int>(fminf(static_cast<float>(in_n), ceilf(right_f)));
    const int cnt = right_i - left_i;
    float value = 0.f;
    for (int j = 0; j < cnt; ++j) {
      float frac = 1.f;
      if (j == 0) frac = static_cast<float>(left_i + 1) - left_f;
      if (j == cnt - 1) frac = right_f - static_cast<float>(left_i + j);
      if (cnt == 1) frac = delta;
      value = value + row[left_i + j] * frac;
    }
    out[out_row + x] = value * normalization;
  }
}

template <int AXIS>
__global__ __launch_bounds__(kBX* kBY) void k_resample_x4(Vols v, F3dGeo gi, F3dGeo g, int in_n, float delta, float normalization)
{
  static_assert(AXIS == 1 || AXIS == 2, "x is gathered, not streamed");
  const float* __restrict__ in = v.in[blockIdx.x];
  float* __restrict__ out = v.out[blockIdx.x];
  const int y = blockIdx.y * kBY + threadIdx.y;
  const int z = g.z_lo + blockIdx.z;
  if (y >= g.H) return;
  const int i = AXIS == 1 ? y : z;
  const float left_f = static_cast<float>(i) * delta;
  const float right_f = static_cast<float>(i + 1) * delta;
  const int left_i = static_cast<int>(floorf(left_f));
  const int right_i = static_cast<int>(fminf(static_cast<float>(in_n), ceilf(right_f)));
  const int cnt = right_i - left_i;
  const size_t out_row = f3d_row(g, y, z);
  for (int x = threadIdx.x * 4; x < g.W; x += kBX * 4) {
    float v0 = 0.f, v1 = 0.f, v2 = 0.f, v3 = 0.f;
    for (int j = 0; j < cnt; ++j) {
      float frac = 1.f;
      if (j == 0) frac = static_cast<float>(left_i + 1) - left_f;
      if (j == cnt - 1) frac = right_f - static_cast<float>(left_i + j);
      if (cnt == 1) frac = delta;
      const int s = left_i + j;
      const float4 q = *reinterpret_cast<const float4*>(in + (AXIS == 1 ? f3d_row(gi, s, z) : f3d_row(gi, y, s)) + x);
      v0 = v0 + q.x * frac;
      v1 = v1 + q.y * frac;
      v2 = v2 + q.z * frac;
      v3 = v3 + q.w * frac;
    }
    float* o = out + out_row + x;
    if (x + 3 < g.W) {
      *reinterpret_cast<float4*>(o) = make_float4(v0 * normalization, v1 * normalization, v2 * normalization, v3 * normalization);
    } else {
      o[0] = v0 * normalization;
      if (x + 1 < g.W) o[1] = v1 * normalization;
      if (x + 2 < g.W) o[2] = v2 * normalization;
    }
  }
}

__global__ __launch_bounds__(kBX* kBY) void k_add(Vols v, F3dGeo g)
{
  const int planes = g.z_hi - g.z_lo;
  const int vol = static_cast<int>(blockIdx.z) / planes;
  float* __restrict__ a = v.out[vol];
  const float* __restrict__ b = v.in[vol];
  const int x = blockIdx.x * kBX + threadIdx.x;
  const int y = blockIdx.y * kBY + threadIdx.y;
  const int z = g.z_lo + (static_cast<int>(blockIdx.z) - vol * planes);
  if (x >= g.W || y >= g.H) return;
  const size_t c = f3d_row(g, y, z) + x;
  a[c] = a[c] + b[c];
}

__global__ __launch_bounds__(256) void k_clear_box(Vols v, F3dGeo g, int chunks_per_row, int rows, int vec)
{
  const unsigned t = blockIdx.x * 256u + threadIdx.x;
  const unsigned total = static_cast<unsigned>(chunks_per_row) * static_cast<unsigned>(rows);
  if (t >= total) return;
  float* __restrict__ p = v.out[blockIdx.y];
  const int r = static_cast<int>(t / static_cast<unsigned>(chunks_per_row));
  const int c = static_cast<int>(t - static_cast<unsigned>(r) * static_cast<unsigned>(chunks_per_row));
  const int zi = r / g.H, y = r - zi * g.H;
  float* row = p + f3d_row(g, y, g.z_lo + zi);
  if (vec) {
    const int x = c * 4;
    if (x + 3 < g.W) {
      *reinterpret_cast<float4*>(row + x) = make_float4(0.f, 0.f, 0.f, 0.f);
    } else {
      for (int k = x; k < g.W; ++k) row[k] = 0.f;
    }
  } else {
    row[c] = 0.f;
  }
}

template <int AXIS>
__global__ __launch_bounds__(kBX* kBY) void k_conv(float* __restrict__ dst, const float* __restrict__ src, F3dGeo g,
                                                   f3d::ConvTaps taps, int radius)
{
  const int x = blockIdx.x * kBX + threadIdx.x;
  const int y = blockIdx.y * kBY + threadIdx.y;
  const int z = g.z_lo + blockIdx.z;
  if (x >= g.W || y >= g.H) return;
  const int n = AXIS == 0 ? g.W : (AXIS == 1 ? g.H : g.D);
  const int i = AXIS == 0 ? x : (AXIS == 1 ? y : z);
  float sum = 0.f;
  for (int j = -radius; j <= radius; ++j) {
    const int s = i + j;
    float val = 0.f;
    if (s >= 0 && s < n) {
      const size_t a = AXIS == 0 ? f3d_row(g, y, z) + s : (AXIS == 1 ? f3d_row(g, s, z) + x : f3d_row(g, y, s) + x);
      val = src[a];
    }
    sum = sum + taps.k[radius - j] * val;
  }
  dst[f3d_row(g, y, z) + x] = sum;
}

__global__ __launch_bounds__(256) void k_abs_max(const float* __restrict__ f, F3dGeo g, unsigned* result)
{
  const int z = g.z_lo + blockIdx.z;
  float m = 0.f;
  for (int y = blockIdx.y; y < g.H; y += gridDim.y) {
    const size_t r = f3d_row(g, y, z);
    for (int x = threadIdx.x; x < g.W; x += blockDim.x) {
      const float v = fabsf(f[r + x]);
      if (v < __builtin_inff()) m = fmaxf(m, v);
    }
  }
  for (int off = 32; off > 0; off >>= 1) m = fmaxf(m, __shfl_down(m, off));
  __shared__ float wave_max[4];
  if ((threadIdx.x & 63) == 0) wave_max[threadIdx.x >> 6] = m;
  __syncthreads();
  if (threadIdx.x == 0) {
    m = fmaxf(fmaxf(wave_max[0], wave_max[1]), fmaxf(wave_max[2], wave_max[3]));
    atomicMax(result, __float_as_uint(m));
  }
}

struct FlowStats {
  unsigned min_bits, max_bits;
  double sum;
};
__global__ __launch_bounds__(256) void k_flow_stats(const float* __restrict__ u, const float* __restrict__ v,
                                                    const float* __restrict__ w, F3dGeo g, FlowStats* out)
{
  const int z = g.z_lo + blockIdx.z;
  float lo = __uint_as_float(0x7f7fffffu), hi = 0.f;
  double sum = 0.0;
  for (int y = blockIdx.y; y < g.H; y += gridDim.y) {
    const size_t r = f3d_row(g, y, z);
    for (int x = threadIdx.x; x < g.W; x += blockDim.x) {
      const float a = u[r + x], b = v[r + x], c = w[r + x];
      const float m = sqrtf(a * a + b * b + c * c);
      lo = fminf(lo, m);
      hi = fmaxf(hi, m);
      sum += static_cast<double>(m);
    }
  }
  for (int off = 32; off > 0; off >>= 1) {
    lo = fminf(lo, __shfl_down(lo, off));
    hi = fmaxf(hi, __shfl_down(hi, off));
    sum += __shfl_down(sum, off);
  }
  if ((threadIdx.x & 63) == 0) {
    atomicMin(&out->min_bits, __float_as_uint(lo));
    atomicMax(&out->max_bits, __float_as_uint(hi));
    atomicAdd(&out->sum, sum);
  }
}

struct ResidualStats {
  double sum_sq, sum_abs;
  unsigned max_bits;
  unsigned pad;
};
__global__ __launch_bounds__(256) void k_residual_stats(const float* __restrict__ f0, const float* __restrict__ fw, F3dGeo g,
                                                        ResidualStats* out)
{
  const int z = g.z_lo + blockIdx.z;
  double ssq = 0.0, sab = 0.0;
  float hi = 0.f;
  for (int y = blockIdx.y; y < g.H; y += gridDim.y) {
    const size_t r = f3d_row(g, y, z);
    for (int x = threadIdx.x; x < g.W; x += blockDim.x) {
      const float d = fw[r + x] - f0[r + x];
      const float a = fabsf(d);
      hi = fmaxf(hi, a);
      sab += static_cast<double>(a);
      ssq += static_cast<double>(d) * static_cast<double>(d);
    }
  }
  for (int off = 32; off > 0; off >>= 1) {
    hi = fmaxf(hi, __shfl_down(hi, off));
    ssq += __shfl_down(ssq, off);
    sab += __shfl_down(sab, off);
  }
  if ((threadIdx.x & 63) == 0) {
    atomicMax(&out->max_bits, __float_as_uint(hi));
    atomicAdd(&out->sum_sq, ssq);
    atomicAdd(&out->sum_abs, sab);
  }
}

bool same_buffer(f3d_devptr a, f3d_devptr b, const char* who)
{
  if (a == b) {
    f3d::fail("%s: input buffer cannot serve as output buffer", who);
    return true;
  }
  return false;
}

bool planes_inside(const F3dGeo& g, int lo, int hi, const char* who)
{
  const int dc = static_cast<int>(f3d::container().depth);
  if (lo < g.z_base || hi - g.z_base > dc) {
    f3d::fail("%s: planes [%d,%d) needed but the container holds [%d,%d)", who, lo, hi, g.z_base, g.z_base + dc);
    return false;
  }
  return true;
}

}

extern "C" {

int f3d_warp(f3d_devptr frame_0, f3d_devptr frame_1, f3d_devptr flow_u, f3d_devptr flow_v, f3d_devptr flow_w,
             size_t width, size_t height, size_t depth, float hx, float hy, float hz, f3d_devptr output,
             const f3d_slab* slab)
{
  F3D_REQUIRE_READY("f3d_warp");
  F3dGeo g;
  if (!f3d::make_geo(&g, width, height, depth, slab, "f3d_warp")) return 1;
  if (same_buffer(frame_1, output, "f3d_warp")) return 1;
  if (g.z_lo == g.z_hi) return 0;
  hipLaunchKernelGGL(k_warp, grid_for(g.W, g.H, g.z_hi - g.z_lo), dim3(kBX, kBY, 1), 0, f3d::stream(),
                     f3d_ptr<const float>(frame_0), f3d_ptr<const float>(frame_1), f3d_ptr<const float>(flow_u),
                     f3d_ptr<const float>(flow_v), f3d_ptr<const float>(flow_w), f3d_ptr<float>(output), g, hx, hy, hz);
  F3D_HIP(hipGetLastError());
  return 0;
}

static bool batch_ok(size_t count, const char* who)
{
  if (count == 0 || count > static_cast<size_t>(kMaxBatch)) {
    f3d::fail("%s: %zu volumes (one launch takes 1 .. %d)", who, count, kMaxBatch);
    return false;
  }
  return true;
}

static int resample_launch(int axis, const f3d_devptr* inputs, const f3d_devptr* outputs, size_t count, size_t ow, size_t oh,
                           size_t od, size_t in_n, const f3d_slab* slab_in, const f3d_slab* slab, const char* who)
{
  F3D_REQUIRE_READY(who);
  if (!inputs || !outputs) return f3d::fail("%s: null argument", who);
  if (!batch_ok(count, who)) return 1;
  for (size_t i = 0; i < count; ++i)
    for (size_t j = 0; j < count; ++j)
      if (same_buffer(inputs[i], outputs[j], who)) return 1;
  if (in_n == 0) return f3d::fail("%s: empty input axis", who);
  F3dGeo g, gi;
  if (!f3d::make_geo(&g, ow, oh, od, slab, who)) return 1;
  const size_t iw = axis == 0 ? in_n : ow, ih = axis == 1 ? in_n : oh, id = axis == 2 ? in_n : od;
  if (!f3d::make_geo(&gi, iw, ih, id, axis == 2 ? slab_in : slab, who)) return 1;
  if (g.z_lo == g.z_hi) return 0;
  if (axis == 2) {
    const float delta = static_cast<float>(in_n) / static_cast<float>(od);
    const int lo = static_cast<int>(floorf(static_cast<float>(g.z_lo) * delta));
    int hi = static_cast<int>(ceilf(static_cast<float>(g.z_hi) * delta));
    if (hi > static_cast<int>(in_n)) hi = static_cast<int>(in_n);
    if (!planes_inside(gi, lo, hi, who)) return 1;
  }
  const dim3 grid(static_cast<unsigned>(count), (g.H + kBY - 1) / kBY, g.z_hi - g.z_lo), block(kBX, kBY, 1);
  Vols v = {};
  bool x4 = g.pitch % 4 == 0 && gi.pitch % 4 == 0;
  for (size_t i = 0; i < count; ++i) {
    v.in[i] = f3d_ptr<const float>(inputs[i]);
    v.out[i] = f3d_ptr<float>(outputs[i]);
    x4 = x4 && reinterpret_cast<uintptr_t>(v.in[i]) % 16 == 0 && reinterpret_cast<uintptr_t>(v.out[i]) % 16 == 0;
  }
  const int n = static_cast<int>(in_n);
  const int out_n = axis == 0 ? g.W : (axis == 1 ? g.H : g.D);
  const float delta = static_cast<float>(n) / static_cast<float>(out_n);
  const float normalization = static_cast<float>(out_n) / static_cast<float>(n);
  const bool staged = x4 && n <= kResampleRowMax && (n + 3) / 4 * 4 <= gi.pitch;
  if (axis == 0 && staged) hipLaunchKernelGGL(k_resample_x_lds, grid, block, 0, f3d::stream(), v, gi, g, n, delta, normalization);
  if (axis == 0 && !staged) hipLaunchKernelGGL(k_resample<0>, grid, block, 0, f3d::stream(), v, gi, g, n, delta, normalization);
  if (axis == 1 && x4) hipLaunchKernelGGL(k_resample_x4<1>, grid, block, 0, f3d::stream(), v, gi, g, n, delta, normalization);
  if (axis == 2 && x4) hipLaunchKernelGGL(k_resample_x4<2>, grid, block, 0, f3d::stream(), v, gi, g, n, delta, normalization);
  if (axis == 1 && !x4) hipLaunchKernelGGL(k_resample<1>, grid, block, 0, f3d::stream(), v, gi, g, n, delta, normalization);
  if (axis == 2 && !x4) hipLaunchKernelGGL(k_resample<2>, grid, block, 0, f3d::stream(), v, gi, g, n, delta, normalization);
  F3D_HIP(hipGetLastError());
  return 0;
}

int f3d_resample_x(f3d_devptr input, f3d_devptr output, size_t out_width, size_t out_height, size_t out_depth,
                   size_t in_width, const f3d_slab* slab)
{
  return resample_launch(0, &input, &output, 1, out_width, out_height, out_depth, in_width, nullptr, slab, "f3d_resample_x");
}

int f3d_resample_y(f3d_devptr input, f3d_devptr output, size_t out_width, size_t out_height, size_t out_depth,
                   size_t in_height, const f3d_slab* slab)
{
  return resample_launch(1, &input, &output, 1, out_width, out_height, out_depth, in_height, nullptr, slab, "f3d_resample_y");
}

int f3d_resample_z(f3d_devptr input, f3d_devptr output, size_t out_width, size_t out_height, size_t out_depth,
                   size_t in_depth, const f3d_slab* slab_in, const f3d_slab* slab)
{
  return resample_launch(2, &input, &output, 1, out_width, out_height, out_depth, in_depth, slab_in, slab, "f3d_resample_z");
}

int f3d_resample_x_n(const f3d_devptr* inputs, const f3d_devptr* outputs, size_t count, size_t out_width, size_t out_height,
                     size_t out_depth, size_t in_width, const f3d_slab* slab)
{
  return resample_launch(0, inputs, outputs, count, out_width, out_height, out_depth, in_width, nullptr, slab, "f3d_resample_x_n");
}

int f3d_resample_y_n(const f3d_devptr* inputs, const f3d_devptr* outputs, size_t count, size_t out_width, size_t out_height,
                     size_t out_depth, size_t in_height, const f3d_slab* slab)
{
  return resample_launch(1, inputs, outputs, count, out_width, out_height, out_depth, in_height, nullptr, slab, "f3d_resample_y_n");
}

int f3d_resample_z_n(const f3d_devptr* inputs, const f3d_devptr* outputs, size_t count, size_t out_width, size_t out_height,
                     size_t out_depth, size_t in_depth, const f3d_slab* slab_in, const f3d_slab* slab)
{
  return resample_launch(2, inputs, outputs, count, out_width, out_height, out_depth, in_depth, slab_in, slab, "f3d_resample_z_n");
}

static int add_launch(const f3d_devptr* operand_0, const f3d_devptr* operand_1, size_t count, size_t width, size_t height,
                      size_t depth, const f3d_slab* slab, const char* who)
{
  F3D_REQUIRE_READY(who);
  if (!operand_0 || !operand_1) return f3d::fail("%s: null argument", who);
  if (!batch_ok(count, who)) return 1;
  F3dGeo g;
  if (!f3d::make_geo(&g, width, height, depth, slab, who)) return 1;
  if (g.z_lo == g.z_hi) return 0;
  Vols v = {};
  for (size_t i = 0; i < count; ++i) {
    v.out[i] = f3d_ptr<float>(operand_0[i]);
    v.in[i] = f3d_ptr<const float>(operand_1[i]);
  }
  const int planes = g.z_hi - g.z_lo;
  if (static_cast<long>(planes) * static_cast<long>(count) > 65535L) {
    for (size_t i = 0; i < count; ++i) {
      Vols one = {};
      one.in[0] = v.in[i];
      one.out[0] = v.out[i];
      hipLaunchKernelGGL(k_add, grid_for(g.W, g.H, planes), dim3(kBX, kBY, 1), 0, f3d::stream(), one, g);
    }
  } else {
    hipLaunchKernelGGL(k_add, grid_for(g.W, g.H, planes * static_cast<int>(count)), dim3(kBX, kBY, 1), 0, f3d::stream(), v, g);
  }
  F3D_HIP(hipGetLastError());
  return 0;
}

int f3d_add(f3d_devptr operand_0, f3d_devptr operand_1, size_t width, size_t height, size_t depth, const f3d_slab* slab)
{
  return add_launch(&operand_0, &operand_1, 1, width, height, depth, slab, "f3d_add");
}

int f3d_add_n(const f3d_devptr* operand_0, const f3d_devptr* operand_1, size_t count, size_t width, size_t height, size_t depth,
              const f3d_slab* slab)
{
  return add_launch(operand_0, operand_1, count, width, height, depth, slab, "f3d_add_n");
}

int f3d_clear_box_n(const f3d_devptr* volumes, size_t count, size_t width, size_t height, size_t depth, const f3d_slab* slab)
{
  F3D_REQUIRE_READY("f3d_clear_box_n");
  if (!volumes) return f3d::fail("f3d_clear_box_n: null argument");
  if (!batch_ok(count, "f3d_clear_box_n")) return 1;
  F3dGeo g;
  if (!f3d::make_geo(&g, width, height, depth, slab, "f3d_clear_box_n")) return 1;
  if (g.z_lo == g.z_hi) return 0;
  Vols v = {};
  bool vec = g.pitch % 4 == 0;
  for (size_t i = 0; i < count; ++i) {
    v.out[i] = f3d_ptr<float>(volumes[i]);
    vec = vec && reinterpret_cast<uintptr_t>(v.out[i]) % 16 == 0;
  }
  const int chunks = vec ? (g.W + 3) / 4 : g.W;
  const long rows = static_cast<long>(g.H) * (g.z_hi - g.z_lo);
  const long total = rows * chunks;
  if (total >= (1L << 32)) return f3d::fail("f3d_clear_box_n: box too large for one launch");
  const dim3 grid(static_cast<unsigned>((total + 255) / 256), static_cast<unsigned>(count), 1);
  hipLaunchKernelGGL(k_clear_box, grid, dim3(256, 1, 1), 0, f3d::stream(), v, g, chunks, static_cast<int>(rows), vec ? 1 : 0);
  F3D_HIP(hipGetLastError());
  return 0;
}

static int conv_launch(int axis, f3d_devptr dst, f3d_devptr src, size_t w, size_t h, size_t d, size_t radius,
                       const f3d_slab* slab, const char* who)
{
  F3D_REQUIRE_READY(who);
  if (same_buffer(dst, src, who)) return 1;
  const f3d::ConvTaps& taps = f3d::conv_taps();
  if (taps.count != static_cast<int>(2 * radius + 1))
    return f3d::fail("%s: radius %zu does not match the %d taps uploaded with f3d_set_conv_taps", who, radius, taps.count);
  F3dGeo g;
  if (!f3d::make_geo(&g, w, h, d, slab, who)) return 1;
  if (g.z_lo == g.z_hi) return 0;
  const dim3 grid = grid_for(g.W, g.H, g.z_hi - g.z_lo), block(kBX, kBY, 1);
  float* o = f3d_ptr<float>(dst);
  const float* s = f3d_ptr<const float>(src);
  const int r = static_cast<int>(radius);
  if (axis == 0) hipLaunchKernelGGL(k_conv<0>, grid, block, 0, f3d::stream(), o, s, g, taps, r);
  if (axis == 1) hipLaunchKernelGGL(k_conv<1>, grid, block, 0, f3d::stream(), o, s, g, taps, r);
  F3D_HIP(hipGetLastError());
  return 0;
}

int f3d_conv_rows(f3d_devptr dst, f3d_devptr src, size_t width, size_t height, size_t depth, size_t kernel_radius,
                  const f3d_slab* slab)
{
  return conv_launch(0, dst, src, width, height, depth, kernel_radius, slab, "f3d_conv_rows");
}

int f3d_conv_cols(f3d_devptr dst, f3d_devptr src, size_t width, size_t height, size_t depth, size_t kernel_radius,
                  const f3d_slab* slab)
{
  return conv_launch(1, dst, src, width, height, depth, kernel_radius, slab, "f3d_conv_cols");
}

int f3d_abs_max(f3d_devptr field, size_t width, size_t height, size_t depth, const f3d_slab* slab, float* result)
{
  F3D_REQUIRE_READY("f3d_abs_max");
  F3dGeo g;
  if (!f3d::make_geo(&g, width, height, depth, slab, "f3d_abs_max")) return 1;
  static thread_local unsigned* d_result = nullptr;
  if (!d_result) F3D_HIP(hipMalloc(reinterpret_cast<void**>(&d_result), sizeof(unsigned)));
  F3D_HIP(hipMemsetAsync(d_result, 0, sizeof(unsigned), f3d::stream()));
  if (g.z_hi > g.z_lo) {
    const int gy = g.H < 16 ? g.H : 16;
    hipLaunchKernelGGL(k_abs_max, dim3(1, gy, g.z_hi - g.z_lo), dim3(256, 1, 1), 0, f3d::stream(),
// ... 63 lines not shown
```

### cuda-flow3d_amd/host/operations.cpp

```cpp
#include "operations.h"

#include <algorithm>
#include <cmath>
#include <cstdio>
#include <utility>

#include "common_utils.h"
#include "hip_utils.h"


bool CudaOperationBase::IsInitialized() const
{
  if (!initialized_) std::printf("Error: Operation '%s' was not initialized.\n", name_);
  return initialized_;
}

void CudaOperationBase::Execute(OperationParameters&)
{
  std::printf("Warning: '%s' Execute() was not defined.\n", name_);
}

void CudaOperationBase::Destroy() { initialized_ = false; }

CudaOperationBase::~CudaOperationBase()
{
  if (initialized_) Destroy();
}

bool CudaOperationBase::InitializeContainer(const OperationParameters* params)
{
  initialized_ = false;
  if (!params) {
    std::printf("Operation: '%s'. Initialization parameters are missing.\n", GetName());
    return initialized_;
  }
  DataSize4 container_size;
  GET_PARAM_OR_RETURN_VALUE(*params, DataSize4, container_size, "container_size", initialized_);
  dev_container_size_ = container_size;
  f3d_size4 c = {container_size.width, container_size.height, container_size.depth, container_size.pitch};
  if (!CheckDeviceError(f3d_set_container(&c))) initialized_ = true;
  return initialized_;
}


void CudaOperationAdd::Execute(OperationParameters& params)
{
  if (!IsInitialized()) return;
  ProfilerRange range(GetName());
  DevicePtr operand_0, operand_1;
  DataSize4 data_size;
  GET_PARAM_OR_RETURN(params, DevicePtr, operand_0, "operand_0");
  GET_PARAM_OR_RETURN(params, DevicePtr, operand_1, "operand_1");
  GET_PARAM_OR_RETURN(params, DataSize4, data_size, "data_size");
  CheckDeviceError(f3d_add(operand_0, operand_1, data_size.width, data_size.height, data_size.depth, slab_));
}

namespace {
constexpr size_t kBatchMax = 3;
bool SameBox(const DataSize4& a, const DataSize4& b) { return a.width == b.width && a.height == b.height && a.depth == b.depth; }
}

void CudaOperationAdd::ExecuteBatch(OperationParameters* params, size_t count)
{
  if (!IsInitialized() || count == 0) return;
  DevicePtr a[kBatchMax], b[kBatchMax];
  DataSize4 size[kBatchMax];
  bool together = count <= kBatchMax;
  for (size_t i = 0; together && i < count; ++i) {
    void *p0 = params[i].GetValuePtr("operand_0"), *p1 = params[i].GetValuePtr("operand_1"), *ps = params[i].GetValuePtr("data_size");
    if (!p0 || !p1 || !ps) {
      together = false;
      break;
    }
    a[i] = *static_cast<DevicePtr*>(p0);
    b[i] = *static_cast<DevicePtr*>(p1);
    size[i] = *static_cast<DataSize4*>(ps);
    together = SameBox(size[i], size[0]);
    for (size_t j = 0; together && j < i; ++j) together = a[i] != a[j] && a[i] != b[j] && b[i] != a[j];
  }
  if (!together) {
    for (size_t i = 0; i < count; ++i) Execute(params[i]);
    return;
  }
  ProfilerRange range(GetName());
  CheckDeviceError(f3d_add_n(a, b, count, size[0].width, size[0].height, size[0].depth, slab_));
}


void CudaOperationStat::Execute(OperationParameters& params)
{
  if (!IsInitialized()) return;
  ProfilerRange range(GetName());
  DevicePtr dev_flow_u, dev_flow_v, dev_flow_w;
  DataSize4 data_size;
  Stat3* p_stat;
  GET_PARAM_OR_RETURN(params, DevicePtr, dev_flow_u, "dev_flow_u");
  GET_PARAM_OR_RETURN(params, DevicePtr, dev_flow_v, "dev_flow_v");
  GET_PARAM_OR_RETURN(params, DevicePtr, dev_flow_w, "dev_flow_w");
  GET_PARAM_OR_RETURN(params, DataSize4, data_size, "data_size");
  GET_PARAM_PTR_OR_RETURN(params, Stat3, p_stat, "stat");
  if (!silent) std::printf("Compute statistics...\n");
  double sum = 0.0;
  if (CheckDeviceError(f3d_flow_stats(dev_flow_u, dev_flow_v, dev_flow_w, data_size.width, data_size.height, data_size.depth, slab_,
                                      &p_stat->min, &p_stat->max, &sum)))
    return;
  const size_t planes = slab_ ? static_cast<size_t>(slab_->z_hi - slab_->z_lo) : data_size.depth;
  const double count = static_cast<double>(data_size.width) * static_cast<double>(data_size.height) * static_cast<double>(planes);
  p_stat->avg = count > 0 ? static_cast<float>(sum / count) : 0.f;
  if (!silent) std::printf("Min: %8.4f Max: %8.4f Avg: %8.4f\n", p_stat->min, p_stat->max, p_stat->avg);
}


void CudaOperationConvolution3D::ComputeGaussianKernel(float sigma, size_t precision, float pixel_size)
{
  kernel_radius_ = static_cast<size_t>(precision * sigma / pixel_size);
  kernel_length_ = 2 * kernel_radius_ + 1;
  if (kernel_length_ > kMaxKernelLength) {
    std::printf("Operation '%s': Gaussian radius %zu exceeds the supported %zu taps.\n", GetName(), kernel_radius_,
                kMaxKernelLength);
    kernel_length_ = 0;
    return;
  }
  const int r = static_cast<int>(kernel_radius_);
  const double norm = 1.0 / (sigma * std::sqrt(2.0 * 3.1415926));
  for (int i = -r; i <= r; ++i) {
    const float dist2 = i * i * pixel_size * pixel_size;
    kernel_[i + r] = static_cast<float>(norm * std::exp(-dist2 / (2.0 * sigma * sigma)));
  }
  float sum = 0.0f;
  for (size_t i = 0; i < kernel_length_; ++i) sum = sum + kernel_[i];
  for (size_t i = 0; i < kernel_length_; ++i) kernel_[i] = kernel_[i] / sum;
}

void CudaOperationConvolution3D::PrintConvolutionKernel() const
{
  if (kernel_length_ == 0) {
    std::printf("Error: Convolution kernel is not initialized.\n");
    return;
  }
  std::printf("Convolution kernel (radius = %zu)\n", kernel_radius_);
  for (size_t i = 0; i < kernel_length_; ++i) std::printf("%.4f ", kernel_[i]);
  std::printf("\n\n");
}

void CudaOperationConvolution3D::Execute(OperationParameters& params)
{
  if (!IsInitialized()) return;
  ProfilerRange range(GetName());
  DevicePtr dev_input = 0, dev_output = 0, dev_temp = 0;
  DataSize4 data_size;
  float gaussian_sigma;
  GET_PARAM_OR_RETURN(params, DevicePtr, dev_input, "dev_input");
  GET_PARAM_OR_RETURN(params, DevicePtr, dev_output, "dev_output");
  GET_PARAM_OR_RETURN(params, DevicePtr, dev_temp, "dev_temp");
  GET_PARAM_OR_RETURN(params, DataSize4, data_size, "data_size");
  GET_PARAM_OR_RETURN(params, float, gaussian_sigma, "gaussian_sigma");
  if (dev_input == dev_output) {
    std::printf("Operation '%s': Error. Input buffer cannot serve as output buffer.", GetName());
    return;
  }
  ComputeGaussianKernel(gaussian_sigma, 3, 1.0);
// ... 130 lines not shown
    if (!pi || !po || !pt || !ps || !pr) {
      together = false;
      break;
    }
    in[i] = *static_cast<DevicePtr*>(pi);
    out[i] = *static_cast<DevicePtr*>(po);
    tmp[i] = *static_cast<DevicePtr*>(pt);
    from[i] = *static_cast<DataSize4*>(ps);
    to[i] = *static_cast<DataSize4*>(pr);
    together = SameBox(from[i], from[0]) && SameBox(to[i], to[0]);
    for (size_t j = 0; together && j <= i; ++j) {
      const DevicePtr mine[3] = {in[i], out[i], tmp[i]}, theirs[3] = {in[j], out[j], tmp[j]};
      for (int a = 0; a < 3; ++a)
        for (int b = 0; b < 3; ++b)
          if (mine[a] == theirs[b] && !(i == j && a == b)) together = false;
    }
  }
  if (!together) {
    for (size_t i = 0; i < count; ++i) Execute(params[i]);
    return;
  }
  ProfilerRange range(GetName());
  const DataSize4 &s = from[0], &r = to[0];
  if (CheckDeviceError(f3d_resample_x_n(in, out, count, r.width, s.height, s.depth, s.width, slab_))) return;
  if (CheckDeviceError(f3d_resample_y_n(out, tmp, count, r.width, r.height, s.depth, s.height, slab_))) return;
  CheckDeviceError(f3d_resample_z_n(tmp, out, count, r.width, r.height, r.depth, s.depth, nullptr, slab_));
}

void CudaOperationResample::ResampleX(DevicePtr input, DevicePtr output, DataSize4& in, DataSize4& out) const
{
  CheckDeviceError(f3d_resample_x(input, output, out.width, out.height, out.depth, in.width, slab_));
}

void CudaOperationResample::ResampleY(DevicePtr input, DevicePtr output, DataSize4& in, DataSize4& out) const
{
  CheckDeviceError(f3d_resample_y(input, output, out.width, out.height, out.depth, in.height, slab_));
}

void CudaOperationResample::ResampleZ(DevicePtr input, DevicePtr output, DataSize4& in, DataSize4& out) const
{
  CheckDeviceError(f3d_resample_z(input, output, out.width, out.height, out.depth, in.depth, nullptr, slab_));
}


bool CudaOperationSolve::ScratchFits() const
{
  return scratch_size_.width == dev_container_size_.width && scratch_size_.height == dev_container_size_.height &&
         scratch_size_.depth == dev_container_size_.depth && scratch_size_.pitch == dev_container_size_.pitch;
}

void CudaOperationSolve::FreeScratch()
{
  if (phi_alt_) f3d_free(phi_alt_);
  if (ksi_alt_) f3d_free(ksi_alt_);
  phi_alt_ = ksi_alt_ = 0;
  for (DevicePtr& p : fder_) {
    if (p) f3d_free(p);
    p = 0;
  }
  scratch_size_ = {0, 0, 0, 0};
}

bool CudaOperationSolve::Initialize(const OperationParameters* params)
{
  const bool ok = InitializeContainer(params);
  if (!ScratchFits()) FreeScratch();
  return ok;
}

size_t CudaOperationSolve::ScratchVolumes()
{
  size_t n = 0;
  if (FusedSweepsEnabled() && FusedPhiKsiEnabled()) n += 2;
  if (FusedSweepsEnabled() && FrameDerivativesEnabled()) n += 4;
  return n;
}

bool CudaOperationSolve::EnsureWeightScratch()
{
  if (!ScratchFits()) FreeScratch();
  if (phi_alt_ && ksi_alt_) return true;
  scratch_size_ = dev_container_size_;
  const size_t rows = dev_container_size_.height * dev_container_size_.depth;
  for (DevicePtr* p : {&phi_alt_, &ksi_alt_}) {
    if (*p) continue;
    size_t pitch = 0;
    if (f3d_alloc_pitched(p, &pitch, dev_container_size_.width * sizeof(float), rows) != 0 || pitch != dev_container_size_.pitch) {
      if (*p) f3d_free(*p);
      *p = 0;
      return false;
    }
  }
  return true;
}

bool CudaOperationSolve::EnsureDerivativeScratch()
{
  if (!ScratchFits()) FreeScratch();
  scratch_size_ = dev_container_size_;
  const size_t rows = dev_container_size_.height * dev_container_size_.depth;
  for (DevicePtr& p : fder_) {
    if (p) continue;
    size_t pitch = 0;
    if (f3d_alloc_pitched(&p, &pitch, dev_container_size_.width * sizeof(float), rows) != 0 || pitch != dev_container_size_.pitch) {
      if (p) f3d_free(p);
      p = 0;
      return false;
    }
  }
  return true;
}

void CudaOperationSolve::Destroy()
{
  FreeScratch();
  CudaOperationBase::Destroy();
}

void CudaOperationSolve::Execute(OperationParameters& params)
{
  if (!IsInitialized()) return;
  ProfilerRange range(GetName());

  DevicePtr dev_frame_0, dev_frame_1, dev_flow_u, dev_flow_v, dev_flow_w, dev_phi, dev_ksi;
  GET_PARAM_OR_RETURN(params, DevicePtr, dev_frame_0, "dev_frame_0");
  GET_PARAM_OR_RETURN(params, DevicePtr, dev_frame_1, "dev_frame_1");
  GET_PARAM_OR_RETURN(params, DevicePtr, dev_flow_u, "dev_flow_u");
  GET_PARAM_OR_RETURN(params, DevicePtr, dev_flow_v, "dev_flow_v");
  GET_PARAM_OR_RETURN(params, DevicePtr, dev_flow_w, "dev_flow_w");
  GET_PARAM_OR_RETURN(params, DevicePtr, dev_phi, "dev_phi");
  GET_PARAM_OR_RETURN(params, DevicePtr, dev_ksi, "dev_ksi");

  DevicePtr *du_ptr, *dv_ptr, *dw_ptr, *tdu_ptr, *tdv_ptr, *tdw_ptr;
  GET_PARAM_PTR_OR_RETURN(params, DevicePtr, du_ptr, "dev_flow_du");
  GET_PARAM_PTR_OR_RETURN(params, DevicePtr, dv_ptr, "dev_flow_dv");
  GET_PARAM_PTR_OR_RETURN(params, DevicePtr, dw_ptr, "dev_flow_dw");
  GET_PARAM_PTR_OR_RETURN(params, DevicePtr, tdu_ptr, "dev_temp_du");
  GET_PARAM_PTR_OR_RETURN(params, DevicePtr, tdv_ptr, "dev_temp_dv");
  GET_PARAM_PTR_OR_RETURN(params, DevicePtr, tdw_ptr, "dev_temp_dw");

  size_t outer_iterations_count, inner_iterations_count;
  float equation_alpha, equation_smoothness, equation_data, hx, hy, hz;
  DataSize4 data_size;
  GET_PARAM_OR_RETURN(params, size_t, outer_iterations_count, "outer_iterations_count");
  GET_PARAM_OR_RETURN(params, size_t, inner_iterations_count, "inner_iterations_count");
  GET_PARAM_OR_RETURN(params, float, equation_alpha, "equation_alpha");
  GET_PARAM_OR_RETURN(params, float, equation_smoothness, "equation_smoothness");
  GET_PARAM_OR_RETURN(params, float, equation_data, "equation_data");
  GET_PARAM_OR_RETURN(params, float, hx, "hx");
  GET_PARAM_OR_RETURN(params, float, hy, "hy");
  GET_PARAM_OR_RETURN(params, float, hz, "hz");
  GET_PARAM_OR_RETURN(params, DataSize4, data_size, "data_size");
  NoteSolveWeights(equation_alpha, hx, hy, hz);

  {
    const DevicePtr increments[3] = {*du_ptr, *dv_ptr, *dw_ptr};
    f3d_slab all = {0, 0, 0};
    if (slab_) {
      const long top = static_cast<long>(slab_->z_base) + static_cast<long>(dev_container_size_.depth);
      all = {slab_->z_base, std::max(0, slab_->z_base), static_cast<int>(std::min<long>(static_cast<long>(data_size.depth), top))};
    }
    if (slab_ && all.z_lo >= all.z_hi) return;
    if (CheckDeviceError(f3d_clear_box_n(increments, 3, data_size.width, data_size.height, data_size.depth, slab_ ? &all : nullptr)))
      return;
  }

  f3d_event ev_start = nullptr, ev_stop = nullptr;
  if (!silent) {
    CheckDeviceError(f3d_event_create(&ev_start));
    CheckDeviceError(f3d_event_create(&ev_stop));
    CheckDeviceError(f3d_event_record(ev_start));
    Utils::PrintProgressBar(0.f);
    std::printf(" % 3.0f%%", 0.f);
  }

  const size_t w = data_size.width, h = data_size.height, d = data_size.depth;
  const bool fuse_weights = FusedSweepsEnabled() && FusedPhiKsiEnabled() && outer_iterations_count > 1 &&
                            dev_container_size_.pitch % 256 == 0 && EnsureWeightScratch();
  const bool tri = FusedSweepsEnabled() && slab_ == nullptr && dev_container_size_.pitch % 256 == 0 && inner_iterations_count >= 2 &&
                   ThreeStageLaunchesPay(w, h, d);
  auto next_group = [&](size_t remaining, bool more) -> size_t {
    if (!FusedSweepsEnabled()) return 1;
    const bool weights_wanted = more && fuse_weights;
    if (tri) {
      if (weights_wanted) {
        if (remaining == 2) return 2;
        if (remaining == 3) return 1;
        if (remaining == 4) return 2;
      }
      if (remaining >= 3) return 3;
    }
    if (weights_wanted && remaining == 3 && !tri) return 2;
    return remaining >= 2 ? 2 : 1;
  };
  auto carries_weights = [&](size_t group, size_t remaining_after, bool more) {
    return more && fuse_weights && remaining_after == 0 && ((tri && group == 2) || group == 1);
  };
  size_t hand_overs = 0;
  for (size_t i = 0; i + 1 < outer_iterations_count; ++i) {
    size_t remaining = inner_iterations_count, group = 0;
    while (remaining > 0) {
      group = next_group(remaining, true);
      remaining -= group;
    }
    if (carries_weights(group, 0, true)) ++hand_overs;
  }
  DevicePtr phi_cur = dev_phi, ksi_cur = dev_ksi, phi_nxt = phi_alt_, ksi_nxt = ksi_alt_;
  if (hand_overs % 2 == 1) {
    std::swap(phi_cur, phi_nxt);
    std::swap(ksi_cur, ksi_nxt);
  }
  bool weights_ready = false;
  const bool on_derivatives = !tri && FusedSweepsEnabled() && FrameDerivativesEnabled() && slab_ == nullptr && inner_iterations_count >= 2 &&
                              f3d_fused_launches_march_along_y(w, h, d) == 0 &&
                              dev_container_size_.pitch % 256 == 0 && EnsureDerivativeScratch() &&
                              !CheckDeviceError(f3d_frame_derivatives(dev_frame_0, dev_frame_1, w, h, d, hx, hy, hz, fder_[0], fder_[1],
                                                                      fder_[2], fder_[3], nullptr));
  for (size_t i = 0; i < outer_iterations_count; ++i) {
    if (!weights_ready &&
        CheckDeviceError(f3d_phi_ksi(dev_frame_0, dev_frame_1, dev_flow_u, dev_flow_v, dev_flow_w, *du_ptr, *dv_ptr, *dw_ptr, w, h, d,
                                     hx, hy, hz, equation_smoothness, equation_data, phi_cur, ksi_cur, slab_)))
      return;
    weights_ready = false;
    const bool more = i + 1 < outer_iterations_count;
    for (size_t j = 0; j < inner_iterations_count;) {
      const size_t group = next_group(inner_iterations_count - j, more);
      const bool with_weights = carries_weights(group, inner_iterations_count - j - group, more);
      int status;
      if (group == 3)
        status = f3d_solve_sweep3(dev_frame_0, dev_frame_1, dev_flow_u, dev_flow_v, dev_flow_w, *du_ptr, *dv_ptr, *dw_ptr, phi_cur, ksi_cur,
                                  w, h, d, hx, hy, hz, equation_alpha, *tdu_ptr, *tdv_ptr, *tdw_ptr, slab_);
      else if (group == 2 && with_weights)
        status = f3d_solve_sweep2_phi_ksi(dev_frame_0, dev_frame_1, dev_flow_u, dev_flow_v, dev_flow_w, *du_ptr, *dv_ptr, *dw_ptr, phi_cur,
                                          ksi_cur, w, h, d, hx, hy, hz, equation_alpha, equation_smoothness, equation_data, *tdu_ptr,
                                          *tdv_ptr, *tdw_ptr, phi_nxt, ksi_nxt, slab_);
      else if (group == 2 && on_derivatives)
        status = f3d_solve_sweep2_fd(fder_[0], fder_[1], fder_[2], fder_[3], dev_flow_u, dev_flow_v, dev_flow_w, *du_ptr, *dv_ptr,
                                     *dw_ptr, phi_cur, ksi_cur, w, h, d, hx, hy, hz, equation_alpha, *tdu_ptr, *tdv_ptr, *tdw_ptr, slab_);
      else if (group == 2)
        status = f3d_solve_sweep2(dev_frame_0, dev_frame_1, dev_flow_u, dev_flow_v, dev_flow_w, *du_ptr, *dv_ptr, *dw_ptr, phi_cur,
                                  ksi_cur, w, h, d, hx, hy, hz, equation_alpha, *tdu_ptr, *tdv_ptr, *tdw_ptr, slab_);
      else if (with_weights && on_derivatives)
        status = f3d_solve_sweep_phi_ksi_fd(fder_[0], fder_[1], fder_[2], fder_[3], dev_flow_u, dev_flow_v, dev_flow_w, *du_ptr,
                                            *dv_ptr, *dw_ptr, phi_cur, ksi_cur, w, h, d, hx, hy, hz, equation_alpha,
                                            equation_smoothness, equation_data, *tdu_ptr, *tdv_ptr, *tdw_ptr, phi_nxt, ksi_nxt, slab_);
      else if (with_weights)
        status = f3d_solve_sweep_phi_ksi(dev_frame_0, dev_frame_1, dev_flow_u, dev_flow_v, dev_flow_w, *du_ptr, *dv_ptr, *dw_ptr,
                                         phi_cur, ksi_cur, w, h, d, hx, hy, hz, equation_alpha, equation_smoothness, equation_data,
                                         *tdu_ptr, *tdv_ptr, *tdw_ptr, phi_nxt, ksi_nxt, slab_);
      else
        status = f3d_solve_sweep(dev_frame_0, dev_frame_1, dev_flow_u, dev_flow_v, dev_flow_w, *du_ptr, *dv_ptr, *dw_ptr, phi_cur,
                                 ksi_cur, w, h, d, hx, hy, hz, equation_alpha, *tdu_ptr, *tdv_ptr, *tdw_ptr, slab_);
      if (CheckDeviceError(status)) return;
      std::swap(*du_ptr, *tdu_ptr);
      std::swap(*dv_ptr, *tdv_ptr);
      std::swap(*dw_ptr, *tdw_ptr);
      if (with_weights) {
        std::swap(phi_cur, phi_nxt);
        std::swap(ksi_cur, ksi_nxt);
        weights_ready = true;
      }
      j += group;
    }
    if (!silent) {
      CheckDeviceError(f3d_stream_sync());
      const float complete = static_cast<float>(i + 1) / static_cast<float>(outer_iterations_count);
      Utils::PrintProgressBar(complete);
      std::printf(" % 3.0f%%", complete * 100);
    }
  }

  if (!silent) {
    float elapsed_ms = 0.f;
    CheckDeviceError(f3d_event_record(ev_stop));
    CheckDeviceError(f3d_event_sync(ev_stop));
    CheckDeviceError(f3d_event_elapsed_ms(&elapsed_ms, ev_start, ev_stop));
    Utils::PrintProgressBar(1.f);
    std::printf(" %8.4fs\n", elapsed_ms / 1000.);
    f3d_event_destroy(ev_start);
    f3d_event_destroy(ev_stop);
  }
}
```

### cuda-flow3d_amd/host/operator_calls.h

```cpp
#ifndef F3D_HOST_OPERATOR_CALLS_H_
#define F3D_HOST_OPERATOR_CALLS_H_

#include "common_utils.h"
#include "data_types.h"
#include "hip_utils.h"

namespace calls {

struct Spacing {
  float *hx, *hy, *hz;
};
struct Flow {
  DevicePtr *u, *v, *w;
};
struct SolverSettings {
  size_t *outer_iterations, *inner_iterations;
  float *alpha, *smoothness, *data;
};

inline OperationParameters& Convolution(OperationParameters& bag, DevicePtr* input, DevicePtr* output, DevicePtr* temp, DataSize4* size,
                                        float* sigma)
{
  return FillBag(bag, {{"dev_input", input}, {"dev_output", output}, {"dev_temp", temp}, {"data_size", size}, {"gaussian_sigma", sigma}});
}

inline OperationParameters& Resample(OperationParameters& bag, DevicePtr* input, DevicePtr* output, DevicePtr* temp, DataSize4* from,
                                     DataSize4* to)
{
  return FillBag(bag, {{"dev_input", input}, {"dev_output", output}, {"dev_temp", temp}, {"data_size", from}, {"resample_size", to}});
}

inline OperationParameters& Registration(OperationParameters& bag, DevicePtr* frame_0, DevicePtr* frame_1, const Flow& flow,
                                         DevicePtr* output, DataSize4* size, const Spacing& h)
{
  return FillBag(bag, {{"dev_frame_0", frame_0}, {"dev_frame_1", frame_1}, {"dev_flow_u", flow.u}, {"dev_flow_v", flow.v},
                       {"dev_flow_w", flow.w}, {"dev_output", output}, {"data_size", size}, {"hx", h.hx}, {"hy", h.hy}, {"hz", h.hz}});
}

inline OperationParameters& Solve(OperationParameters& bag, DevicePtr* frame_0, DevicePtr* frame_1_registered, const Flow& flow,
                                  const Flow& increment, const Flow& partner, DevicePtr* phi, DevicePtr* ksi, const SolverSettings& s,
                                  DataSize4* size, const Spacing& h)
{
  return FillBag(bag, {{"dev_frame_0", frame_0}, {"dev_frame_1", frame_1_registered}, {"dev_flow_u", flow.u}, {"dev_flow_v", flow.v},
                       {"dev_flow_w", flow.w}, {"dev_flow_du", increment.u}, {"dev_flow_dv", increment.v}, {"dev_flow_dw", increment.w},
                       {"dev_phi", phi}, {"dev_ksi", ksi}, {"dev_temp_du", partner.u}, {"dev_temp_dv", partner.v},
                       {"dev_temp_dw", partner.w}, {"outer_iterations_count", s.outer_iterations},
                       {"inner_iterations_count", s.inner_iterations}, {"equation_alpha", s.alpha}, {"equation_smoothness", s.smoothness},
                       {"equation_data", s.data}, {"data_size", size}, {"hx", h.hx}, {"hy", h.hy}, {"hz", h.hz}});
}

inline OperationParameters& Add(OperationParameters& bag, DevicePtr* accumulator, DevicePtr* addend, DataSize4* size)
{
  return FillBag(bag, {{"operand_0", accumulator}, {"operand_1", addend}, {"data_size", size}});
}

inline OperationParameters& Median(OperationParameters& bag, DevicePtr* input, DevicePtr* output, DataSize4* size, size_t* window)
{
  return FillBag(bag, {{"dev_input", input}, {"dev_output", output}, {"data_size", size}, {"radius", window}});
}

inline OperationParameters& Statistics(OperationParameters& bag, const Flow& flow, DataSize4* size, Stat3* result)
{
  return FillBag(bag, {{"dev_flow_u", flow.u}, {"dev_flow_v", flow.v}, {"dev_flow_w", flow.w}, {"data_size", size}, {"stat", result}});
}

}

#endif
```

### cuda-flow3d_amd/host/optical_flow.cpp

```cpp
#include "optical_flow.h"

#include <algorithm>
#include <cmath>
#include <cstdio>

#include "common_utils.h"
#include "operator_calls.h"
#include "hip_utils.h"
#include "motion_fit.h"

extern "C" int f3d_compose_flow(f3d_devptr acc_u, f3d_devptr acc_v, f3d_devptr acc_w, f3d_devptr inc_u, f3d_devptr inc_v,
                                f3d_devptr inc_w, size_t width, size_t height, size_t depth, unsigned long long* lost)
    __attribute__((weak));
extern "C" int f3d_flow_strain(f3d_devptr u, f3d_devptr v, f3d_devptr w, const f3d_devptr out[8], unsigned fields, size_t width,
                               size_t height, size_t depth, f3d_strain_stats* stats) __attribute__((weak));
extern "C" int f3d_principal_strain(f3d_devptr u, f3d_devptr v, f3d_devptr w, const f3d_devptr out[10], unsigned fields,
                                    size_t width, size_t height, size_t depth, f3d_principal_stats* stats) __attribute__((weak));
extern "C" int f3d_invert_displacement(f3d_devptr d_u, f3d_devptr d_v, f3d_devptr d_w, f3d_devptr g_u, f3d_devptr g_v,
                                       f3d_devptr g_w, f3d_devptr err, size_t width, size_t height, size_t depth,
                                       unsigned iterations, float tolerance, f3d_inverse_stats* stats) __attribute__((weak));
extern "C" int f3d_carry_field(f3d_devptr field, f3d_devptr m_u, f3d_devptr m_v, f3d_devptr m_w, f3d_devptr out, size_t width,
                               size_t height, size_t depth, unsigned mode, unsigned long long* lost) __attribute__((weak));
extern "C" int f3d_local_correlation(f3d_devptr a, f3d_devptr b, const f3d_devptr out[2], unsigned fields, unsigned radius,
                                     float threshold, size_t width, size_t height, size_t depth, f3d_correlation_stats* stats)
// ... 568 lines not shown
  FieldSet& set = derived_[kMatch];
  if (of.kind == Displacement::kTrajectory) {
    set.error.clear();
    return set.Fail("the match quality of a trajectory is not available: frame 0 of a sequence is not kept (use a pair's flow)");
  }
  DevicePtr d[3];
  if (!ResolveDisplacement(set, of, f3d_local_correlation != nullptr, d)) return false;
  if (!f3d_carry_field) return set.Fail("the device library has no f3d_carry_field (match quality carries frame 1 through the flow)");
  if (fields == 0 || (fields & ~kMatchAll)) return set.Fail("fields must be a non-empty combination of kMatchWarped, kMatchZncc, kMatchRmsd");
  if (!frame_0) frame_0 = resident_frame_[0];
  if (!frame_1) frame_1 = resident_frame_[1];
  if (!frame_0 || !frame_1) return set.Fail("no frames on the device (AllocateResidentFrames and UploadResidentFrames first)");
  const unsigned stored = fields & (kMatchZncc | kMatchRmsd) ? fields & (kMatchZncc | kMatchRmsd) : kMatchZncc;
  if (!set.Allocate(kMatchWarped | stored)) return false;
  const f3d_size4 c = Container();
  const DevicePtr out[2] = {set.ptr[1], set.ptr[2]};
  const unsigned device_fields = (stored & kMatchZncc ? F3D_CORRELATION_ZNCC : 0u) | (stored & kMatchRmsd ? F3D_CORRELATION_RMSD : 0u);
  return set.Check(CheckDeviceError(f3d_set_container(&c))) &&
         set.Check(CheckDeviceError(f3d_carry_field(frame_1, d[0], d[1], d[2], set.ptr[0], c.width, c.height, c.depth, F3D_CARRY_LINEAR,
                                                    nullptr))) &&
         set.Check(CheckDeviceError(f3d_local_correlation(frame_0, set.ptr[0], out, device_fields, radius, threshold, c.width, c.height,
                                                          c.depth, stats)));
}

bool OpticalFlowE::ComputeMotion(const Displacement& of, int model, DevicePtr weight, float weight_min, f3d_motion_fit* fit,
                                 f3d_motion_residual* residual)
{
  FieldSet& set = derived_[kMotion];
  DevicePtr d[3];
  if (!ResolveDisplacement(set, of, f3d_motion_sums != nullptr, d)) return false;
  if (!f3d_remove_motion) return set.Fail("the device library has no f3d_remove_motion (motion fit)");
  if (!fit) return set.Fail("no fit to write to");
  if (!set.Allocate(0)) return false;
  const f3d_size4 c = Container();
  struct f3d_motion_sums sums;
  if (!set.Check(CheckDeviceError(f3d_set_container(&c))) ||
      !set.Check(CheckDeviceError(f3d_motion_sums(d[0], d[1], d[2], weight, weight_min, c.width, c.height, c.depth, &sums))))
    return false;
  f3d_motion_fit solved = {};
  solved.centre[0] = 0.5 * static_cast<double>(c.width - 1);
  solved.centre[1] = 0.5 * static_cast<double>(c.height - 1);
  solved.centre[2] = 0.5 * static_cast<double>(c.depth - 1);
  std::string why;
  if (!SolveMotion(sums, model, &solved, &why)) return set.Fail(why.c_str());
  if (!set.Check(CheckDeviceError(f3d_remove_motion(d[0], d[1], d[2], set.ptr[0], set.ptr[1], set.ptr[2], &solved, c.width, c.height,
                                                    c.depth, residual))))
    return false;
  *fit = solved;
  return true;
}

bool OpticalFlowE::RunPyramid(OperationParameters& params, DevicePtr raw_0, DevicePtr raw_1, bool raw_is_pooled)
{
  size_t warp_levels_count, outer_iterations_count, inner_iterations_count, median_radius;
  float warp_scale_factor, equation_alpha, equation_smoothness, equation_data, gaussian_sigma;
  GET_PARAM_OR_RETURN_VALUE(params, size_t, warp_levels_count, "warp_levels_count", false);
  GET_PARAM_OR_RETURN_VALUE(params, float, warp_scale_factor, "warp_scale_factor", false);
  GET_PARAM_OR_RETURN_VALUE(params, size_t, outer_iterations_count, "outer_iterations_count", false);
  GET_PARAM_OR_RETURN_VALUE(params, size_t, inner_iterations_count, "inner_iterations_count", false);
  GET_PARAM_OR_RETURN_VALUE(params, float, equation_alpha, "equation_alpha", false);
  GET_PARAM_OR_RETURN_VALUE(params, float, equation_smoothness, "equation_smoothness", false);
  GET_PARAM_OR_RETURN_VALUE(params, float, equation_data, "equation_data", false);
  GET_PARAM_OR_RETURN_VALUE(params, size_t, median_radius, "median_radius", false);
  GET_PARAM_OR_RETURN_VALUE(params, float, gaussian_sigma, "gaussian_sigma", false);
  calls::SolverSettings settings = {&outer_iterations_count, &inner_iterations_count, &equation_alpha, &equation_smoothness, &equation_data};

  if (!silent) std::printf("\nStarting optical flow computation...\n");

  DataSize4 whole = {dev_container_size_.width, dev_container_size_.height, dev_container_size_.depth, 0};
  const size_t deepest = GetMaxWarpLevel(whole.width, whole.height, whole.depth, warp_scale_factor);
  const int first_level = static_cast<int>(std::min(warp_levels_count, deepest)) - 1;
  const size_t container_rows = dev_container_size_.height * dev_container_size_.depth;
  const size_t container_row_bytes = dev_container_size_.width * sizeof(float);
  auto zero_container = [&](DevicePtr p) { CheckDeviceError(f3d_memset2d(p, dev_container_size_.pitch, 0, container_row_bytes, container_rows)); };
  OperationParameters bag;

  DevicePtr raw[2] = {raw_0, raw_1};
  DevicePtr blurred[2];
  if (gaussian_sigma > 0.0) {
    DevicePtr scratch = Borrow();
    for (int f = 0; f < 2; ++f) {
      blurred[f] = Borrow();
      cuop_convolution_.Execute(calls::Convolution(bag, &raw[f], &blurred[f], &scratch, &whole, &gaussian_sigma));
    }
    GiveBack(scratch);
    if (raw_is_pooled)
      for (DevicePtr p : raw) GiveBack(p);
  } else if (raw_is_pooled) {
    blurred[0] = raw[0];
    blurred[1] = raw[1];
  } else {
    for (int f = 0; f < 2; ++f) {
      blurred[f] = Borrow();
      CheckDeviceError(f3d_copy_d2d(blurred[f], raw[f], dev_container_size_.pitch * container_rows));
    }
  }

  DevicePtr level_frame[2] = {Borrow(), Borrow()};
  DevicePtr flow[3] = {Borrow(), Borrow(), Borrow()};
  DevicePtr step[3] = {Borrow(), Borrow(), Borrow()};
  const calls::Flow flow_roles = {&flow[0], &flow[1], &flow[2]}, step_roles = {&step[0], &step[1], &step[2]};

  level_stats_.clear();
  if (first_level < 0)
    for (DevicePtr p : flow) zero_container(p);

  auto resample_together = [&](DevicePtr* in, DevicePtr* out, size_t count, DataSize4& from, DataSize4& to) {
    OperationParameters bags[3];
    DevicePtr scratch[3] = {0, 0, 0};
    for (size_t i = 0; i < count; ++i) {
      scratch[i] = Borrow();
      calls::Resample(bags[i], &in[i], &out[i], &scratch[i], &from, &to);
    }
    cuop_resample_.ExecuteBatch(bags, count);
    for (size_t i = 0; i < count; ++i) GiveBack(scratch[i]);
  };

  DataSize4 coarser = {0, 0, 0, 0};
  for (int level = first_level; level >= 0; --level) {
    PyramidLevel geometry = GetLevel(whole, warp_scale_factor, level);
    DataSize4 box = geometry.size;
    const calls::Spacing spacing = {&geometry.hx, &geometry.hy, &geometry.hz};
    char range_name[64];
    std::snprintf(range_name, sizeof(range_name), "level %d (%zu x %zu x %zu)", level, box.width, box.height, box.depth);
    ProfilerRange level_range(range_name);
    if (!silent) std::printf("Solve level %2d (%4zu x%4zu x%4zu) \n", level, box.width, box.height, box.depth);

    if (level == 0)
      for (int f = 0; f < 2; ++f) std::swap(blurred[f], level_frame[f]);
    else
      resample_together(blurred, level_frame, 2, whole, box);

    if (coarser.width == 0) {
      for (DevicePtr p : flow) zero_container(p);
    } else {
      resample_together(flow, step, 3, coarser, box);
      for (int c = 0; c < 3; ++c) std::swap(flow[c], step[c]);
    }

    {
      DevicePtr registered = Borrow();
      cuop_register_.Execute(calls::Registration(bag, &level_frame[0], &level_frame[1], flow_roles, &registered, &box, spacing));
      std::swap(level_frame[1], registered);
      GiveBack(registered);
    }
    if (collect_level_statistics) {
      LevelStatistics st;
      st.level = level;
      st.size = box;
      ResidualOf(level_frame[0], level_frame[1], box, st.before);
      level_stats_.push_back(st);
    }

    {
      DevicePtr phi = Borrow(), ksi = Borrow();
      DevicePtr partner[3] = {Borrow(), Borrow(), Borrow()};
      const calls::Flow partner_roles = {&partner[0], &partner[1], &partner[2]};
      cuop_solve_.silent = silent;
      cuop_solve_.Execute(calls::Solve(bag, &level_frame[0], &level_frame[1], flow_roles, step_roles, partner_roles, &phi, &ksi, settings,
                                       &box, spacing));
      for (DevicePtr p : {phi, ksi, partner[0], partner[1], partner[2]}) GiveBack(p);
    }

    {
      OperationParameters bags[3];
      for (int c = 0; c < 3; ++c) calls::Add(bags[c], &flow[c], &step[c], &box);
      cuop_add_.ExecuteBatch(bags, 3);
      for (int c = 0; c < 3; ++c) calls::Median(bags[c], &flow[c], &step[c], &box, &median_radius);
      cuop_median_.ExecuteBatch(bags, 3);
      for (int c = 0; c < 3; ++c) std::swap(flow[c], step[c]);
    }

    if (collect_level_statistics) {
      float mn = 0.f, mx = 0.f;
      double sum = 0.0;
      if (!CheckDeviceError(f3d_flow_stats(flow[0], flow[1], flow[2], box.width, box.height, box.depth, nullptr, &mn, &mx, &sum))) {
        const double n = static_cast<double>(box.width) * static_cast<double>(box.height) * static_cast<double>(box.depth);
        level_stats_.back().flow = {mn, mx, static_cast<float>(sum / n)};
      }
      if (!silent) {
        const LevelStatistics& st = level_stats_.back();
        std::printf("  residual before the solve: rms %.5f  mean |.| %.5f  max %.4f;  flow after it: min %.4f  max %.4f  avg %.4f\n",
                    st.before.rms, st.before.mean_abs, st.before.max_abs, st.flow.min, st.flow.max, st.flow.avg);
      }
    }
    coarser = box;
  }

  for (int c = 0; c < 3; ++c) result_flow_[c] = flow[c];
  for (DevicePtr p : {blurred[0], blurred[1], level_frame[0], level_frame[1], step[0], step[1], step[2]}) GiveBack(p);
  return true;
}

void OpticalFlowE::Destroy()
{
  for (CudaOperationBase* cuop : cuda_operations_) cuop->Destroy();
  ReleaseResult();
  trajectory_.Release();
  for (FieldSet& set : derived_) set.Release();
  size_t freed = 0;
  while (!free_containers_.empty()) {
    CheckDeviceError(f3d_free(free_containers_.back()));
    free_containers_.pop_back();
    ++freed;
  }
  if (sequence_frame_[2]) {
    for (DevicePtr& p : sequence_frame_) {
      if (p) CheckDeviceError(f3d_free(p));
      p = 0;
    }
    resident_frame_[0] = resident_frame_[1] = 0;
  }
  for (DevicePtr& p : resident_frame_) {
    if (p) CheckDeviceError(f3d_free(p));
    p = 0;
  }
  if (freed && freed != kContainers + extra_containers_) std::printf("Warning. Not all device memory allocations were freed.\n");
  extra_containers_ = 0;
  initialized_ = false;
}
```

### include/f3d.h

```cpp
#ifndef F3D_H_
#define F3D_H_

#include <stddef.h>
#include <stdint.h>

#ifdef __cplusplus
extern "C" {
#endif

typedef uint64_t f3d_devptr;

typedef struct f3d_size4 {
  size_t width;
  size_t height;
  size_t depth;
  size_t pitch;
} f3d_size4;

typedef struct f3d_slab {
  int z_base;
  int z_lo;
  int z_hi;
} f3d_slab;

typedef struct f3d_event_s* f3d_event;
typedef struct f3d_queue_s* f3d_queue;


int f3d_init(int device);
int f3d_shutdown(void);
int f3d_is_initialized(void);
typedef struct f3d_lane_s* f3d_lane;
int f3d_lane_create(f3d_lane* lane);
int f3d_lane_make_current(f3d_lane lane);
int f3d_lane_is_private(void);
int f3d_lane_get_current(f3d_lane* lane);
int f3d_lane_destroy(f3d_lane lane);

int f3d_crash_maps_enable(const char* path);
int f3d_device_count(int* count);
int f3d_device_name(char* name, size_t capacity);
int f3d_mem_info(size_t* free_bytes, size_t* total_bytes);
int f3d_lds_per_workgroup(int* bytes);
const char* f3d_last_error(void);

int f3d_alloc_pitched(f3d_devptr* ptr, size_t* pitch, size_t width_bytes, size_t rows);
int f3d_free(f3d_devptr ptr);
int f3d_memset2d(f3d_devptr ptr, size_t pitch, int value, size_t width_bytes, size_t rows);
int f3d_copy3d_h2d(f3d_devptr dst, size_t dev_pitch, size_t dev_height, size_t dev_plane0,
                   const float* src, size_t width, size_t height, size_t depth);
int f3d_copy3d_d2h(float* dst, size_t width, size_t height, size_t depth,
                   f3d_devptr src, size_t dev_pitch, size_t dev_height, size_t dev_plane0);
int f3d_copy_planes_h2d(f3d_devptr dst, size_t dev_pitch, size_t dev_height, size_t dev_plane0, const float* src,
                        size_t src_row_floats, size_t src_rows, size_t width, size_t height, size_t depth);
int f3d_copy_planes_d2h(float* dst, size_t dst_row_floats, size_t dst_rows, size_t width, size_t height, size_t depth,
                        f3d_devptr src, size_t dev_pitch, size_t dev_height, size_t dev_plane0);
int f3d_queue_create(f3d_queue* queue);
int f3d_queue_destroy(f3d_queue queue);
int f3d_queue_sync(f3d_queue queue);
int f3d_event_record_on(f3d_event ev, f3d_queue queue);
int f3d_queue_wait_event(f3d_queue queue, f3d_event ev);
int f3d_copy_planes_h2d_on(f3d_queue queue, f3d_devptr dst, size_t dev_pitch, size_t dev_height, size_t dev_plane0, const float* src,
                           size_t src_row_floats, size_t src_rows, size_t width, size_t height, size_t depth);
int f3d_copy_planes_d2h_on(f3d_queue queue, float* dst, size_t dst_row_floats, size_t dst_rows, size_t width, size_t height,
                           size_t depth, f3d_devptr src, size_t dev_pitch, size_t dev_height, size_t dev_plane0);
int f3d_copy_rect_d2d(f3d_devptr dst, size_t dst_pitch, size_t dst_rows, size_t dst_plane0, f3d_devptr src, size_t src_pitch,
                      size_t src_rows, size_t src_plane0, size_t width, size_t height, size_t depth);
int f3d_host_register(void* ptr, size_t bytes);
int f3d_host_unregister(void* ptr);
int f3d_host_is_pinned(const void* ptr, int* yes);
int f3d_copy_d2d(f3d_devptr dst, f3d_devptr src, size_t bytes);
int f3d_set_container(const f3d_size4* container);
int f3d_get_container(f3d_size4* container);

int f3d_event_create(f3d_event* ev);
int f3d_event_record(f3d_event ev);
int f3d_event_sync(f3d_event ev);
int f3d_event_elapsed_ms(float* ms, f3d_event start, f3d_event stop);
int f3d_event_destroy(f3d_event ev);
int f3d_stream_sync(void);


int f3d_phi_ksi(f3d_devptr frame_0, f3d_devptr frame_1, f3d_devptr flow_u, f3d_devptr flow_v, f3d_devptr flow_w,
                f3d_devptr flow_du, f3d_devptr flow_dv, f3d_devptr flow_dw,
                size_t width, size_t height, size_t depth, float hx, float hy, float hz,
                float equation_smoothness, float equation_data, f3d_devptr phi, f3d_devptr ksi,
                const f3d_slab* slab);

int f3d_phi_ksi_zones(f3d_devptr frame_0, f3d_devptr frame_1, f3d_devptr flow_u, f3d_devptr flow_v, f3d_devptr flow_w,
                      f3d_devptr flow_du, f3d_devptr flow_dv, f3d_devptr flow_dw, size_t width, size_t height, size_t depth, float hx,
                      float hy, float hz, float equation_smoothness, float equation_data, f3d_devptr phi, f3d_devptr ksi,
                      const f3d_slab* zone_a, const f3d_slab* zone_b);

int f3d_solve_sweep(f3d_devptr frame_0, f3d_devptr frame_1, f3d_devptr flow_u, f3d_devptr flow_v, f3d_devptr flow_w,
                    f3d_devptr flow_du, f3d_devptr flow_dv, f3d_devptr flow_dw, f3d_devptr phi, f3d_devptr ksi,
                    size_t width, size_t height, size_t depth, float hx, float hy, float hz, float equation_alpha,
                    f3d_devptr temp_du, f3d_devptr temp_dv, f3d_devptr temp_dw, const f3d_slab* slab);

int f3d_solve_sweep2(f3d_devptr frame_0, f3d_devptr frame_1, f3d_devptr flow_u, f3d_devptr flow_v, f3d_devptr flow_w,
                     f3d_devptr flow_du, f3d_devptr flow_dv, f3d_devptr flow_dw, f3d_devptr phi, f3d_devptr ksi,
                     size_t width, size_t height, size_t depth, float hx, float hy, float hz, float equation_alpha,
                     f3d_devptr temp_du, f3d_devptr temp_dv, f3d_devptr temp_dw, const f3d_slab* slab);

int f3d_solve_sweep_phi_ksi(f3d_devptr frame_0, f3d_devptr frame_1, f3d_devptr flow_u, f3d_devptr flow_v, f3d_devptr flow_w,
                            f3d_devptr flow_du, f3d_devptr flow_dv, f3d_devptr flow_dw, f3d_devptr phi, f3d_devptr ksi,
                            size_t width, size_t height, size_t depth, float hx, float hy, float hz, float equation_alpha,
                            float equation_smoothness, float equation_data, f3d_devptr temp_du, f3d_devptr temp_dv,
                            f3d_devptr temp_dw, f3d_devptr phi_next, f3d_devptr ksi_next, const f3d_slab* slab);

int f3d_solve_sweep_phi_ksi_edges(f3d_devptr frame_0, f3d_devptr frame_1, f3d_devptr flow_u, f3d_devptr flow_v, f3d_devptr flow_w,
                                  f3d_devptr flow_du, f3d_devptr flow_dv, f3d_devptr flow_dw, f3d_devptr phi, f3d_devptr ksi,
                                  size_t width, size_t height, size_t depth, float hx, float hy, float hz, float equation_alpha,
                                  float equation_smoothness, float equation_data, f3d_devptr temp_du, f3d_devptr temp_dv,
                                  f3d_devptr temp_dw, f3d_devptr phi_next, f3d_devptr ksi_next, const f3d_slab* slab,
                                  int keep_below, int keep_above);

int f3d_fused_launches_march_along_y(size_t width, size_t height, size_t depth);

int f3d_solve_sweep3(f3d_devptr frame_0, f3d_devptr frame_1, f3d_devptr flow_u, f3d_devptr flow_v, f3d_devptr flow_w,
                     f3d_devptr flow_du, f3d_devptr flow_dv, f3d_devptr flow_dw, f3d_devptr phi, f3d_devptr ksi, size_t width,
                     size_t height, size_t depth, float hx, float hy, float hz, float equation_alpha, f3d_devptr temp_du,
                     f3d_devptr temp_dv, f3d_devptr temp_dw, const f3d_slab* slab);
int f3d_solve_sweep2_phi_ksi(f3d_devptr frame_0, f3d_devptr frame_1, f3d_devptr flow_u, f3d_devptr flow_v, f3d_devptr flow_w,
                             f3d_devptr flow_du, f3d_devptr flow_dv, f3d_devptr flow_dw, f3d_devptr phi, f3d_devptr ksi, size_t width,
                             size_t height, size_t depth, float hx, float hy, float hz, float equation_alpha,
                             float equation_smoothness, float equation_data, f3d_devptr temp_du, f3d_devptr temp_dv,
                             f3d_devptr temp_dw, f3d_devptr phi_next, f3d_devptr ksi_next, const f3d_slab* slab);

int f3d_frame_derivatives(f3d_devptr frame_0, f3d_devptr frame_1, size_t width, size_t height, size_t depth, float hx, float hy,
                          float hz, f3d_devptr fx, f3d_devptr fy, f3d_devptr fz, f3d_devptr ft, const f3d_slab* slab);
int f3d_solve_sweep2_fd(f3d_devptr fx, f3d_devptr fy, f3d_devptr fz, f3d_devptr ft, f3d_devptr flow_u, f3d_devptr flow_v, f3d_devptr flow_w,
                        f3d_devptr flow_du, f3d_devptr flow_dv, f3d_devptr flow_dw, f3d_devptr phi, f3d_devptr ksi, size_t width,
                        size_t height, size_t depth, float hx, float hy, float hz, float equation_alpha, f3d_devptr temp_du,
                        f3d_devptr temp_dv, f3d_devptr temp_dw, const f3d_slab* slab);
int f3d_solve_sweep_phi_ksi_fd(f3d_devptr fx, f3d_devptr fy, f3d_devptr fz, f3d_devptr ft, f3d_devptr flow_u, f3d_devptr flow_v,
                               f3d_devptr flow_w, f3d_devptr flow_du, f3d_devptr flow_dv, f3d_devptr flow_dw, f3d_devptr phi,
                               f3d_devptr ksi, size_t width, size_t height, size_t depth, float hx, float hy, float hz,
                               float equation_alpha, float equation_smoothness, float equation_data, f3d_devptr temp_du,
                               f3d_devptr temp_dv, f3d_devptr temp_dw, f3d_devptr phi_next, f3d_devptr ksi_next, const f3d_slab* slab);
int f3d_solve_sweep_phi_ksi_edges_fd(f3d_devptr fx, f3d_devptr fy, f3d_devptr fz, f3d_devptr ft, f3d_devptr flow_u, f3d_devptr flow_v,
                                     f3d_devptr flow_w, f3d_devptr flow_du, f3d_devptr flow_dv, f3d_devptr flow_dw, f3d_devptr phi,
                                     f3d_devptr ksi, size_t width, size_t height, size_t depth, float hx, float hy, float hz,
                                     float equation_alpha, float equation_smoothness, float equation_data, f3d_devptr temp_du,
                                     f3d_devptr temp_dv, f3d_devptr temp_dw, f3d_devptr phi_next, f3d_devptr ksi_next,
                                     const f3d_slab* slab, int keep_below, int keep_above);

int f3d_warp(f3d_devptr frame_0, f3d_devptr frame_1, f3d_devptr flow_u, f3d_devptr flow_v, f3d_devptr flow_w,
             size_t width, size_t height, size_t depth, float hx, float hy, float hz, f3d_devptr output,
             const f3d_slab* slab);

int f3d_resample_x(f3d_devptr input, f3d_devptr output, size_t out_width, size_t out_height, size_t out_depth,
                   size_t in_width, const f3d_slab* slab);
int f3d_resample_y(f3d_devptr input, f3d_devptr output, size_t out_width, size_t out_height, size_t out_depth,
                   size_t in_height, const f3d_slab* slab);
int f3d_resample_z(f3d_devptr input, f3d_devptr output, size_t out_width, size_t out_height, size_t out_depth,
                   size_t in_depth, const f3d_slab* slab_in, const f3d_slab* slab);

int f3d_add(f3d_devptr operand_0, f3d_devptr operand_1, size_t width, size_t height, size_t depth,
            const f3d_slab* slab);

int f3d_median(f3d_devptr input, size_t width, size_t height, size_t depth, size_t radius, f3d_devptr output,
               const f3d_slab* slab);

int f3d_resample_x_n(const f3d_devptr* inputs, const f3d_devptr* outputs, size_t count, size_t out_width, size_t out_height,
                     size_t out_depth, size_t in_width, const f3d_slab* slab);
int f3d_resample_y_n(const f3d_devptr* inputs, const f3d_devptr* outputs, size_t count, size_t out_width, size_t out_height,
                     size_t out_depth, size_t in_height, const f3d_slab* slab);
int f3d_resample_z_n(const f3d_devptr* inputs, const f3d_devptr* outputs, size_t count, size_t out_width, size_t out_height,
                     size_t out_depth, size_t in_depth, const f3d_slab* slab_in, const f3d_slab* slab);
int f3d_add_n(const f3d_devptr* operand_0, const f3d_devptr* operand_1, size_t count, size_t width, size_t height, size_t depth,
              const f3d_slab* slab);
int f3d_median_n(const f3d_devptr* inputs, size_t count, size_t width, size_t height, size_t depth, size_t radius,
                 const f3d_devptr* outputs, const f3d_slab* slab);
int f3d_clear_box_n(const f3d_devptr* volumes, size_t count, size_t width, size_t height, size_t depth, const f3d_slab* slab);

int f3d_set_conv_taps(const float* taps, size_t count);
int f3d_conv_rows(f3d_devptr dst, f3d_devptr src, size_t width, size_t height, size_t depth, size_t kernel_radius,
                  const f3d_slab* slab);
int f3d_conv_cols(f3d_devptr dst, f3d_devptr src, size_t width, size_t height, size_t depth, size_t kernel_radius,
                  const f3d_slab* slab);
int f3d_conv_slices(f3d_devptr dst, f3d_devptr src, size_t width, size_t height, size_t depth, size_t kernel_radius,
                    const f3d_slab* slab);
int f3d_conv_rows_cols(f3d_devptr dst, f3d_devptr src, size_t width, size_t height, size_t depth, size_t kernel_radius,
                       const f3d_slab* slab);

int f3d_selftest_weights(unsigned lo_bits, unsigned hi_bits, unsigned long long* checked, unsigned long long* excluded,
                         unsigned long long* mismatches, unsigned* first_mismatch);

int f3d_range_push(const char* name);
int f3d_range_pop(void);


enum { F3D_K_PHI_KSI = 0, F3D_K_SWEEP = 1, F3D_K_SWEEP2 = 2, F3D_K_SWEEP_PHI_KSI = 3, F3D_K_SWEEP3 = 4, F3D_K_SWEEP2_PHI_KSI = 5,
       F3D_K_COUNT = 6 };
int f3d_prof_enable(int enable);
int f3d_prof_reset(void);
int f3d_prof_select(unsigned kernel_mask);
int f3d_prof_read(int kernel, size_t min_voxels, double* total_ms, uint64_t* launches, double* total_voxels);


int f3d_comm_unique_id(void* id128);
int f3d_comm_init(const void* id128, int rank, int n_ranks);
int f3d_comm_destroy(void);
int f3d_comm_rank(int* rank, int* n_ranks);
int f3d_comm_info(int* backend, int* comm_ranks, int* comm_rank, int* comm_device, unsigned long long* sent_bytes,
                  unsigned long long* exchanges);
int f3d_pack_planes(f3d_devptr field, int plane0, int count, size_t width, size_t height, f3d_devptr staging,
                    size_t offset_floats);
int f3d_unpack_planes(f3d_devptr field, int plane0, int count, size_t width, size_t height, f3d_devptr staging,
                      size_t offset_floats);
int f3d_pack_segments(const f3d_devptr* fields, const int* plane0, const int* count, const size_t* offset_floats,
                      int n_segments, size_t width, size_t height, f3d_devptr staging);
int f3d_unpack_segments(const f3d_devptr* fields, const int* plane0, const int* count, const size_t* offset_floats,
                        int n_segments, size_t width, size_t height, f3d_devptr staging);
int f3d_copy_planes(f3d_devptr dst, int dst_plane0, f3d_devptr src, int src_plane0, int count, size_t width,
                    size_t height);
int f3d_copy_plane_segments(const f3d_devptr* dst, const int* dst_plane0, const f3d_devptr* src, const int* src_plane0, const int* count,
                            int n_segments, size_t width, size_t height);
int f3d_comm_sendrecv(f3d_devptr send_buf, const size_t* send_offset, const size_t* send_count, f3d_devptr recv_buf,
                      const size_t* recv_offset, const size_t* recv_count, const int* peers, int n_peers);
int f3d_comm_sendrecv_begin(f3d_devptr send_buf, const size_t* send_offset, const size_t* send_count, f3d_devptr recv_buf,
                            const size_t* recv_offset, const size_t* recv_count, const int* peers, int n_peers);
int f3d_comm_sendrecv_end(void);
int f3d_comm_timing(int enable);
int f3d_comm_mark(int what, int cls);
int f3d_comm_timing_read(int cls, double* total_us, unsigned long long* count, double* min_us, double* max_us,
                         unsigned long long* bytes);
int f3d_comm_allreduce_max_f32(float* value);
int f3d_abs_max(f3d_devptr field, size_t width, size_t height, size_t depth, const f3d_slab* slab, float* result);

int f3d_flow_stats(f3d_devptr flow_u, f3d_devptr flow_v, f3d_devptr flow_w, size_t width, size_t height, size_t depth,
                   const f3d_slab* slab, float* min_magnitude, float* max_magnitude, double* sum_magnitude);

int f3d_residual_stats(f3d_devptr frame_0, f3d_devptr frame_1_warped, size_t width, size_t height, size_t depth,
                       const f3d_slab* slab, double* sum_squares, double* sum_abs, float* max_abs);

int f3d_compose_flow(f3d_devptr acc_u, f3d_devptr acc_v, f3d_devptr acc_w, f3d_devptr inc_u, f3d_devptr inc_v,
                     f3d_devptr inc_w, size_t width, size_t height, size_t depth, unsigned long long* lost);

#define F3D_STRAIN_VOL 1u
#define F3D_STRAIN_E 2u
#define F3D_STRAIN_EQ 4u
typedef struct f3d_strain_stats {
  unsigned long long defined, folded;
  float vol_min, vol_max, eq_max;
  double vol_sum;
} f3d_strain_stats;
int f3d_flow_strain(f3d_devptr u, f3d_devptr v, f3d_devptr w, const f3d_devptr out[8], unsigned fields, size_t width,
                    size_t height, size_t depth, f3d_strain_stats* stats );

// ... 65 lines not shown
```

Measured before the change: 73.07 Mvoxels/s.

## Fuse flow increment addition into final solver sweep and add row-staged x resample

The sweep kernel body moves into a shared header, and a second instantiation writes flow plus increment directly during the last inner sweep of the last outer iteration. The separate per-level Add pass over three full volumes and the buffer swap are then skipped, and the median reads the summed flow straight from the step buffers. An x-axis resample kernel is also added that stages several whole rows per wave in LDS. The fused path depends on a weak symbol and a host flag, and it adds a buffer-aliasing check.

```diff
diff --git a/cuda-flow3d_amd/__init__.py b/cuda-flow3d_amd/__init__.py
--- a/cuda-flow3d_amd/__init__.py
+++ b/cuda-flow3d_amd/__init__.py
@@ -363,6 +363,11 @@
     return fn
 
 
+def solve_sweep_add_entry():
+    return _entry("f3d_solve_sweep_add", [_dp] * 10 + [_sz] * 3 + [C.c_float] * 4 + [_dp] * 3 + [_slabp],
+                  "add the increments to the flow inside the last sweep")
+
+
 def _compose_entry():
     return _entry("f3d_compose_flow", [_dp] * 6 + [_sz] * 3 + [C.POINTER(C.c_ulonglong)], "compose flows into a trajectory")
 
@@ -884,6 +889,8 @@
                 store[k] = _sz(v)
             elif k == "stat":
                 store[k] = v
+            elif k == "flow_update":
+                store[k] = C.c_bool(bool(v))
             else:
                 raise TypeError(f"unknown parameter key {k!r}")
         n = len(store) + len(volumes)
diff --git a/cuda-flow3d_amd/csrc/f3d_solve.hip b/cuda-flow3d_amd/csrc/f3d_solve.hip
--- a/cuda-flow3d_amd/csrc/f3d_solve.hip
+++ b/cuda-flow3d_amd/csrc/f3d_solve.hip
@@ -286,200 +286,17 @@
 __global__ __launch_bounds__(kLanes* TY, 4) void k_sweep6(SolveArgs a, F3dGeo g, int zchunk, int ntx, int nty, int n_tiles,
                                                             int xcd_remap)
 {
-  __shared__ float img[2][kNL][TY + 2][kLanes];
-  __shared__ float hrow[kRing][2][9][kLanes];
-  __shared__ float hcol[kRing][TY][kLanes];
-
-  int tile = static_cast<int>(blockIdx.x);
-  if (xcd_remap) {
-    const int per_xcd = (n_tiles + 7) / 8;
-    tile = (tile % 8) * per_xcd + tile / 8;
-  }
-  if (tile >= n_tiles) return;
-  const int tx = tile % ntx;
-  const int ty = (tile / ntx) % nty;
-  const int tz = tile / (ntx * nty);
-
-  const int lane = threadIdx.x;
-  const int r = __builtin_amdgcn_readfirstlane(static_cast<int>(threadIdx.y));
-  const int z0 = g.z_lo + tz * zchunk;
-  const int z1 = min(z0 + zchunk, g.z_hi);
-  const int y0 = ty * TY;
-  const int y = y0 + r;
-  const int yy = f3d_clampi(f3d_mir(y, g.H), 0, g.H - 1);
-  const int x = tx * kLanes + lane;
-  const int xi = f3d_clampi(f3d_mir(x, g.W), 0, g.W - 1);
-  const unsigned xb = static_cast<unsigned>(xi) * 4u;
-  const bool owner = x < g.W && y < g.H;
-  const int side = lane < 32 ? 0 : 1;
-  const int xh = f3d_clampi(f3d_mir(side == 0 ? tx * kLanes - 1 : tx * kLanes + kLanes, g.W), 0, g.W - 1);
-  const bool edge = (r == 0) || (r == TY - 1);
-  const int which = r == 0 ? 0 : 1;
-  const int yh_row = f3d_clampi(f3d_mir(r == 0 ? y0 - 1 : y0 + TY, g.H), 0, g.H - 1);
-  const int lds_halo = r == 0 ? 0 : TY + 1;
-
-  const int zb = z0 > 0 ? z0 - 1 : 0;
-  const size_t base_off = f3d_row(g, 0, zb);
-  const unsigned plane_b = static_cast<unsigned>(g.Hc) * static_cast<unsigned>(g.pitch) * 4u;
-  const unsigned row_b = static_cast<unsigned>(g.pitch) * 4u;
-  constexpr int kOrder[9] = {F0, F1, U, V, Wf, DU, DV, DW, PHI};
-  const float* base[10];
-#pragma unroll
-  for (int i = 0; i < 10; ++i) base[i] = a.in[i] + base_off;
-  float* obase[3];
-#pragma unroll
-  for (int i = 0; i < 3; ++i) obase[i] = a.out[i] + base_off;
-  const bool col_lane = (lane & 31) < 9;
-  const float* lane_base = base[0];
-#pragma unroll
-  for (int i = 1; i < 9; ++i)
-    if ((lane & 31) == i) lane_base = base[kOrder[i]];
-  lane_base += xh;
-
-  auto rowoff = [&](int yrow, int zz) {
-    return static_cast<unsigned>(__builtin_amdgcn_readfirstlane(
-        static_cast<int>(static_cast<unsigned>(zz - zb) * plane_b + static_cast<unsigned>(yrow) * row_b)));
-  };
-  auto load_plane = [&](PlaneRegs& p, int zz) {
-    const unsigned off = xb + rowoff(yy, zz);
-    p.f0 = gld(base[F0], off);
-    p.f1 = gld(base[F1], off);
-    p.u = gld(base[U], off);
-    p.v = gld(base[V], off);
-    p.w = gld(base[Wf], off);
-    p.su = gld(base[DU], off);
-    p.dv = gld(base[DV], off);
-    p.dw = gld(base[DW], off);
-    p.phi = gld(base[PHI], off);
-    p.ksi = gld(base[9], off);
-  };
-  auto dma_halos = [&](int zz) {
-    const int slot = zz & (kRing - 1);
-    if (col_lane) gld_lds_lane(lane_base + (rowoff(yy, zz) >> 2), &hcol[slot][r][0]);
-    if (edge) {
-      const unsigned off = xb + rowoff(yh_row, zz);
-#pragma unroll
-      for (int i = 0; i < 9; ++i) gld_lds(base[kOrder[i]], off, &hrow[slot][which][i][0]);
-    }
-  };
-  auto ring_row = [&](PlaneRegs& p, int slot) {
-    const float* d = &hrow[slot][which][0][lane];
-    p.f0 = d[0 * kLanes]; p.f1 = d[1 * kLanes]; p.u = d[2 * kLanes]; p.v = d[3 * kLanes]; p.w = d[4 * kLanes];
-    p.su = d[5 * kLanes]; p.dv = d[6 * kLanes]; p.dw = d[7 * kLanes]; p.phi = d[8 * kLanes];
-  };
-  auto ring_col = [&](PlaneRegs& p, int slot) {
-    const float* d = &hcol[slot][r][side * 32];
-    p.f0 = d[0]; p.f1 = d[1]; p.u = d[2]; p.v = d[3]; p.w = d[4]; p.su = d[5]; p.dv = d[6]; p.dw = d[7]; p.phi = d[8];
-  };
-
-  auto publish = [&](const PlaneRegs& pl, int nb, int ring_slot) {
-    const Face6 f = plane_face(pl);
-#pragma unroll
-    for (int i = 0; i < kNL; ++i) img[nb][i][r + 1][lane] = f.v[i];
-    if (edge) {
-      PlaneRegs Hc;
-      ring_row(Hc, ring_slot);
-      plane_finish(Hc);
-      const Face6 hf = plane_face(Hc);
-#pragma unroll
-      for (int i = 0; i < kNL; ++i) img[nb][i][lds_halo][lane] = hf.v[i];
-    }
-  };
-
-  auto step = [&](auto full, const PlaneRegs& M, const PlaneRegs& C, const PlaneRegs& P, PlaneRegs& Q1, PlaneRegs& Q2, int z) {
-    constexpr bool FULL = decltype(full)::value;
-    const bool row3 = FULL || z + 3 <= z1;
-    const bool halo3 = FULL || z + 3 < z1;
-    if (row3) load_plane(Q2, f3d_mir(z + 3, g.D));
-    if (halo3 && ABLATE != 2) dma_halos(z + 3);
-
-    const int b = z & 1;
-    const int slot = z & (kRing - 1);
-    const Face6 cf = plane_face(C);
-    if (ABLATE != 3) __syncthreads();
-
-    Face6 ym, yp, xm, xp;
-#pragma unroll
-    for (int i = 0; i < kNL; ++i) {
-      ym.v[i] = img[b][i][r][lane];
-      yp.v[i] = img[b][i][r + 2][lane];
-    }
-    PlaneRegs X;
-    ring_col(X, slot);
-    if ((FULL || z + 1 < z1) && ABLATE != 3) publish(P, b ^ 1, (z + 1) & (kRing - 1));
-    plane_finish(X);
-    const Face6 xf = plane_face(X);
-#pragma unroll
-    for (int i = 0; i < kNL; ++i) {
-      xm.v[i] = lane_left_or(cf.v[i], xf.v[i]);
-      xp.v[i] = lane_right_or(cf.v[i], xf.v[i]);
-    }
-    float r_du, r_dv, r_dw;
-    if (ABLATE == 1) {
-      r_du = xm.v[0] + xp.v[1] + ym.v[2] + yp.v[3] + M.su + P.sv + C.ksi;
-      r_dv = xm.v[4] + xp.v[5] + ym.v[0] + yp.v[1] + M.f0 + P.f1 + C.u;
-      r_dw = xm.v[2] + xp.v[3] + ym.v[4] + yp.v[5] + M.phi + P.phi + C.dv + C.dw + C.v + C.w;
-    } else {
-      sweep_voxel_s(xm, xp, ym, yp, plane_face(M), plane_face(P), cf.v, C.u, C.v, C.w, C.dv, C.dw, C.ksi, a.hx, a.hy, a.hz,
-                    a.p0, x < g.W - 1, x > 0, y < g.H - 1, y > 0, z < g.D - 1, z > 0, r_du, r_dv, r_dw);
-    }
-    asm volatile("" ::"v"(r_du), "v"(r_dv), "v"(r_dw));
-    __builtin_amdgcn_sched_barrier(0);
-    if (FULL && ABLATE == 2) {
-      F3D_WAIT_PLANE(10, Q1);
-    } else if (FULL) {
-      if (edge) F3D_WAIT_PLANE(20, Q1);
-      else F3D_WAIT_PLANE(11, Q1);
-    } else {
-      F3D_WAIT_PLANE(0, Q1);
-    }
-    if (FULL || z + 2 <= z1) plane_finish(Q1);
-    __builtin_amdgcn_sched_barrier(0);
-    if (owner) {
-      const unsigned off = xb + rowoff(yy, z);
-      gst(obase[0], off, r_du);
-      gst(obase[1], off, r_dv);
-      gst(obase[2], off, r_dw);
-    }
-    __builtin_amdgcn_sched_barrier(0);
-  };
-
-  PlaneRegs A, B, C, D, E;
-  E = PlaneRegs{};
-  D = PlaneRegs{};
-  load_plane(A, f3d_mir(z0 - 1, g.D));
-  load_plane(B, z0);
-  load_plane(C, f3d_mir(z0 + 1, g.D));
-  if (z0 + 2 <= z1) load_plane(D, f3d_mir(z0 + 2, g.D));
-  dma_halos(z0);
-  if (z0 + 1 < z1) dma_halos(z0 + 1);
-  if (z0 + 2 < z1) dma_halos(z0 + 2);
-  F3D_WAIT_PLANE(0, A);
-  F3D_WAIT_PLANE(0, B);
-  F3D_WAIT_PLANE(0, C);
-  F3D_WAIT_PLANE(0, D);
-  plane_finish(A);
-  plane_finish(B);
-  plane_finish(C);
-  __syncthreads();
-  publish(B, z0 & 1, z0 & (kRing - 1));
-  __builtin_amdgcn_sched_barrier(0);
-  int z = z0;
-  for (; z + 7 < z1; z += 5) {
-    step(std::true_type{}, A, B, C, D, E, z);
-    step(std::true_type{}, B, C, D, E, A, z + 1);
-    step(std::true_type{}, C, D, E, A, B, z + 2);
-    step(std::true_type{}, D, E, A, B, C, z + 3);
-    step(std::true_type{}, E, A, B, C, D, z + 4);
-  }
-  for (; z < z1; z += 5) {
-    step(std::false_type{}, A, B, C, D, E, z);
-    if (z + 1 < z1) step(std::false_type{}, B, C, D, E, A, z + 1);
-    if (z + 2 < z1) step(std::false_type{}, C, D, E, A, B, z + 2);
-    if (z + 3 < z1) step(std::false_type{}, D, E, A, B, C, z + 3);
-    if (z + 4 < z1) step(std::false_type{}, E, A, B, C, D, z + 4);
-  }
-  asm volatile("s_waitcnt vmcnt(0)" ::: "memory");
+  constexpr bool kAddFlow = false;
+#include "f3d_solve_sweep6_body.h"
+}
+
+template <int TY>
+__global__ __launch_bounds__(kLanes* TY, 4) void k_last_sweep_flow(SolveArgs a, F3dGeo g, int zchunk, int ntx, int nty, int n_tiles,
+                                                                     int xcd_remap)
+{
+  constexpr int ABLATE = 0;
+  constexpr bool kAddFlow = true;
+#include "f3d_solve_sweep6_body.h"
 }
 
 struct Plane8 {
@@ -1109,7 +926,7 @@
 #include "f3d_solve_pair8.h"
 #include "f3d_solve_tri.h"
 
-template <bool SWEEP>
+template <bool SWEEP, bool ADD_FLOW = false>
 void launch_solver(const SolveArgs& args, const F3dGeo& g)
 {
   const Tuning& t = tuning();
@@ -1150,7 +967,9 @@
   const int blocks = t.xcd_remap ? per_xcd * 8 : n_tiles;
   const dim3 grid(blocks, 1, 1), block(kLanes, kTY3, 1);
   auto go = [&](auto kern) { hipLaunchKernelGGL(kern, grid, block, 0, f3d::stream(), a, g, zchunk, ntx, nty, n_tiles, t.xcd_remap); };
-  if constexpr (SWEEP) {
+  if constexpr (SWEEP && ADD_FLOW) {
+    go(k_last_sweep_flow<kTY3>);
+  } else if constexpr (SWEEP) {
 #ifdef F3D_LAB
     static const int ablate = std::getenv("F3D_ABLATE") ? std::atoi(std::getenv("F3D_ABLATE")) : 0;
     if (ablate == 1) return go(k_sweep6<1, kTY3>);
@@ -1331,6 +1150,38 @@
   return 0;
 }
 
+template <bool ADD_FLOW>
+int sweep_launch(const char* who, const f3d_devptr (&in)[10], size_t width, size_t height, size_t depth, float hx, float hy, float hz,
+                 float equation_alpha, f3d_devptr temp_du, f3d_devptr temp_dv, f3d_devptr temp_dw, const f3d_slab* slab)
+{
+  F3dGeo g;
+  if (!f3d::make_geo(&g, width, height, depth, slab, who)) return 1;
+  if (g.W < 2 || g.H < 2 || g.D < 2) return f3d::fail("%s: every dimension must be at least 2", who);
+  if (ADD_FLOW) {
+    const f3d_devptr out[3] = {temp_du, temp_dv, temp_dw};
+    for (int i = 0; i < 3; ++i)
+      for (int k = 0; k < 10; ++k)
+        if (out[i] == in[k]) return f3d::fail("%s: an output buffer is also an input (other tiles still read it)", who);
+  }
+  if (g.z_lo == g.z_hi) return 0;
+  if (!slab_reach_ok(g, 1, who)) return 1;
+  SolveArgs a;
+  static const int plain_division = std::getenv("F3D_UDIV") && std::atoi(std::getenv("F3D_UDIV")) == 0;
+  a.plain_division = plain_division;
+  for (int i = 0; i < 10; ++i) a.in[i] = f3d_ptr<const float>(in[i]);
+  a.out[0] = f3d_ptr<float>(temp_du);
+  a.out[1] = f3d_ptr<float>(temp_dv);
+  a.out[2] = f3d_ptr<float>(temp_dw);
+  a.hx = hx; a.hy = hy; a.hz = hz;
+  a.p0 = equation_alpha;
+  a.p1 = 0.f;
+  f3d::prof_begin(F3D_K_SWEEP, static_cast<size_t>(g.W) * g.H * (g.z_hi - g.z_lo));
+  launch_solver<true, ADD_FLOW>(a, g);
+  f3d::prof_end(F3D_K_SWEEP);
+  F3D_HIP(hipGetLastError());
+  return 0;
+}
+
 }
 
 extern "C" {
@@ -1409,27 +1260,18 @@
                     f3d_devptr temp_du, f3d_devptr temp_dv, f3d_devptr temp_dw, const f3d_slab* slab)
 {
   F3D_REQUIRE_READY("f3d_solve_sweep");
-  F3dGeo g;
-  if (!f3d::make_geo(&g, width, height, depth, slab, "f3d_solve_sweep")) return 1;
-  if (g.W < 2 || g.H < 2 || g.D < 2) return f3d::fail("f3d_solve_sweep: every dimension must be at least 2");
-  if (g.z_lo == g.z_hi) return 0;
-  if (!slab_reach_ok(g, 1, "f3d_solve_sweep")) return 1;
-  SolveArgs a;
-  static const int plain_division = std::getenv("F3D_UDIV") && std::atoi(std::getenv("F3D_UDIV")) == 0;
-  a.plain_division = plain_division;
   const f3d_devptr in[10] = {frame_0, frame_1, flow_u, flow_v, flow_w, flow_du, flow_dv, flow_dw, phi, ksi};
-  for (int i = 0; i < 10; ++i) a.in[i] = f3d_ptr<const float>(in[i]);
-  a.out[0] = f3d_ptr<float>(temp_du);
-  a.out[1] = f3d_ptr<float>(temp_dv);
-  a.out[2] = f3d_ptr<float>(temp_dw);
-  a.hx = hx; a.hy = hy; a.hz = hz;
-  a.p0 = equation_alpha;
-  a.p1 = 0.f;
-  f3d::prof_begin(F3D_K_SWEEP, static_cast<size_t>(g.W) * g.H * (g.z_hi - g.z_lo));
-  launch_solver<true>(a, g);
-  f3d::prof_end(F3D_K_SWEEP);
-  F3D_HIP(hipGetLastError());
-  return 0;
+  return sweep_launch<false>("f3d_solve_sweep", in, width, height, depth, hx, hy, hz, equation_alpha, temp_du, temp_dv, temp_dw, slab);
+}
+
+int f3d_solve_sweep_add(f3d_devptr frame_0, f3d_devptr frame_1, f3d_devptr flow_u, f3d_devptr flow_v, f3d_devptr flow_w,
+                        f3d_devptr flow_du, f3d_devptr flow_dv, f3d_devptr flow_dw, f3d_devptr phi, f3d_devptr ksi,
+                        size_t width, size_t height, size_t depth, float hx, float hy, float hz, float equation_alpha,
+                        f3d_devptr sum_u, f3d_devptr sum_v, f3d_devptr sum_w, const f3d_slab* slab)
+{
+  F3D_REQUIRE_READY("f3d_solve_sweep_add");
+  const f3d_devptr in[10] = {frame_0, frame_1, flow_u, flow_v, flow_w, flow_du, flow_dv, flow_dw, phi, ksi};
+  return sweep_launch<true>("f3d_solve_sweep_add", in, width, height, depth, hx, hy, hz, equation_alpha, sum_u, sum_v, sum_w, slab);
 }
 
 int f3d_solve_sweep2(f3d_devptr frame_0, f3d_devptr frame_1, f3d_devptr flow_u, f3d_devptr flow_v, f3d_devptr flow_w,
diff --git a/cuda-flow3d_amd/csrc/f3d_solve_sweep6_body.h b/cuda-flow3d_amd/csrc/f3d_solve_sweep6_body.h
--- /dev/null
+++ b/cuda-flow3d_amd/csrc/f3d_solve_sweep6_body.h
@@ -0,0 +1,194 @@
+  __shared__ float img[2][kNL][TY + 2][kLanes];
+  __shared__ float hrow[kRing][2][9][kLanes];
+  __shared__ float hcol[kRing][TY][kLanes];
+
+  int tile = static_cast<int>(blockIdx.x);
+  if (xcd_remap) {
+    const int per_xcd = (n_tiles + 7) / 8;
+    tile = (tile % 8) * per_xcd + tile / 8;
+  }
+  if (tile >= n_tiles) return;
+  const int tx = tile % ntx;
+  const int ty = (tile / ntx) % nty;
+  const int tz = tile / (ntx * nty);
+
+  const int lane = threadIdx.x;
+  const int r = __builtin_amdgcn_readfirstlane(static_cast<int>(threadIdx.y));
+  const int z0 = g.z_lo + tz * zchunk;
+  const int z1 = min(z0 + zchunk, g.z_hi);
+  const int y0 = ty * TY;
+  const int y = y0 + r;
+  const int yy = f3d_clampi(f3d_mir(y, g.H), 0, g.H - 1);
+  const int x = tx * kLanes + lane;
+  const int xi = f3d_clampi(f3d_mir(x, g.W), 0, g.W - 1);
+  const unsigned xb = static_cast<unsigned>(xi) * 4u;
+  const bool owner = x < g.W && y < g.H;
+  const int side = lane < 32 ? 0 : 1;
+  const int xh = f3d_clampi(f3d_mir(side == 0 ? tx * kLanes - 1 : tx * kLanes + kLanes, g.W), 0, g.W - 1);
+  const bool edge = (r == 0) || (r == TY - 1);
+  const int which = r == 0 ? 0 : 1;
+  const int yh_row = f3d_clampi(f3d_mir(r == 0 ? y0 - 1 : y0 + TY, g.H), 0, g.H - 1);
+  const int lds_halo = r == 0 ? 0 : TY + 1;
+
+  const int zb = z0 > 0 ? z0 - 1 : 0;
+  const size_t base_off = f3d_row(g, 0, zb);
+  const unsigned plane_b = static_cast<unsigned>(g.Hc) * static_cast<unsigned>(g.pitch) * 4u;
+  const unsigned row_b = static_cast<unsigned>(g.pitch) * 4u;
+  constexpr int kOrder[9] = {F0, F1, U, V, Wf, DU, DV, DW, PHI};
+  const float* base[10];
+#pragma unroll
+  for (int i = 0; i < 10; ++i) base[i] = a.in[i] + base_off;
+  float* obase[3];
+#pragma unroll
+  for (int i = 0; i < 3; ++i) obase[i] = a.out[i] + base_off;
+  const bool col_lane = (lane & 31) < 9;
+  const float* lane_base = base[0];
+#pragma unroll
+  for (int i = 1; i < 9; ++i)
+    if ((lane & 31) == i) lane_base = base[kOrder[i]];
+  lane_base += xh;
+
+  auto rowoff = [&](int yrow, int zz) {
+    return static_cast<unsigned>(__builtin_amdgcn_readfirstlane(
+        static_cast<int>(static_cast<unsigned>(zz - zb) * plane_b + static_cast<unsigned>(yrow) * row_b)));
+  };
+  auto load_plane = [&](PlaneRegs& p, int zz) {
+    const unsigned off = xb + rowoff(yy, zz);
+    p.f0 = gld(base[F0], off);
+    p.f1 = gld(base[F1], off);
+    p.u = gld(base[U], off);
+    p.v = gld(base[V], off);
+    p.w = gld(base[Wf], off);
+    p.su = gld(base[DU], off);
+    p.dv = gld(base[DV], off);
+    p.dw = gld(base[DW], off);
+    p.phi = gld(base[PHI], off);
+    p.ksi = gld(base[9], off);
+  };
+  auto dma_halos = [&](int zz) {
+    const int slot = zz & (kRing - 1);
+    if (col_lane) gld_lds_lane(lane_base + (rowoff(yy, zz) >> 2), &hcol[slot][r][0]);
+    if (edge) {
+      const unsigned off = xb + rowoff(yh_row, zz);
+#pragma unroll
+      for (int i = 0; i < 9; ++i) gld_lds(base[kOrder[i]], off, &hrow[slot][which][i][0]);
+    }
+  };
+  auto ring_row = [&](PlaneRegs& p, int slot) {
+    const float* d = &hrow[slot][which][0][lane];
+    p.f0 = d[0 * kLanes]; p.f1 = d[1 * kLanes]; p.u = d[2 * kLanes]; p.v = d[3 * kLanes]; p.w = d[4 * kLanes];
+    p.su = d[5 * kLanes]; p.dv = d[6 * kLanes]; p.dw = d[7 * kLanes]; p.phi = d[8 * kLanes];
+  };
+  auto ring_col = [&](PlaneRegs& p, int slot) {
+    const float* d = &hcol[slot][r][side * 32];
+    p.f0 = d[0]; p.f1 = d[1]; p.u = d[2]; p.v = d[3]; p.w = d[4]; p.su = d[5]; p.dv = d[6]; p.dw = d[7]; p.phi = d[8];
+  };
+
+  auto publish = [&](const PlaneRegs& pl, int nb, int ring_slot) {
+    const Face6 f = plane_face(pl);
+#pragma unroll
+    for (int i = 0; i < kNL; ++i) img[nb][i][r + 1][lane] = f.v[i];
+    if (edge) {
+      PlaneRegs Hc;
+      ring_row(Hc, ring_slot);
+      plane_finish(Hc);
+      const Face6 hf = plane_face(Hc);
+#pragma unroll
+      for (int i = 0; i < kNL; ++i) img[nb][i][lds_halo][lane] = hf.v[i];
+    }
+  };
+
+  auto step = [&](auto full, const PlaneRegs& M, const PlaneRegs& C, const PlaneRegs& P, PlaneRegs& Q1, PlaneRegs& Q2, int z) {
+    constexpr bool FULL = decltype(full)::value;
+    const bool row3 = FULL || z + 3 <= z1;
+    const bool halo3 = FULL || z + 3 < z1;
+    if (row3) load_plane(Q2, f3d_mir(z + 3, g.D));
+    if (halo3 && ABLATE != 2) dma_halos(z + 3);
+
+    const int b = z & 1;
+    const int slot = z & (kRing - 1);
+    const Face6 cf = plane_face(C);
+    if (ABLATE != 3) __syncthreads();
+
+    Face6 ym, yp, xm, xp;
+#pragma unroll
+    for (int i = 0; i < kNL; ++i) {
+      ym.v[i] = img[b][i][r][lane];
+      yp.v[i] = img[b][i][r + 2][lane];
+    }
+    PlaneRegs X;
+    ring_col(X, slot);
+    if ((FULL || z + 1 < z1) && ABLATE != 3) publish(P, b ^ 1, (z + 1) & (kRing - 1));
+    plane_finish(X);
+    const Face6 xf = plane_face(X);
+#pragma unroll
+    for (int i = 0; i < kNL; ++i) {
+      xm.v[i] = lane_left_or(cf.v[i], xf.v[i]);
+      xp.v[i] = lane_right_or(cf.v[i], xf.v[i]);
+    }
+    float r_du, r_dv, r_dw;
+    if (ABLATE == 1) {
+      r_du = xm.v[0] + xp.v[1] + ym.v[2] + yp.v[3] + M.su + P.sv + C.ksi;
+      r_dv = xm.v[4] + xp.v[5] + ym.v[0] + yp.v[1] + M.f0 + P.f1 + C.u;
+      r_dw = xm.v[2] + xp.v[3] + ym.v[4] + yp.v[5] + M.phi + P.phi + C.dv + C.dw + C.v + C.w;
+    } else {
+      sweep_voxel_s(xm, xp, ym, yp, plane_face(M), plane_face(P), cf.v, C.u, C.v, C.w, C.dv, C.dw, C.ksi, a.hx, a.hy, a.hz,
+                    a.p0, x < g.W - 1, x > 0, y < g.H - 1, y > 0, z < g.D - 1, z > 0, r_du, r_dv, r_dw);
+    }
+    asm volatile("" ::"v"(r_du), "v"(r_dv), "v"(r_dw));
+    __builtin_amdgcn_sched_barrier(0);
+    if (FULL && ABLATE == 2) {
+      F3D_WAIT_PLANE(10, Q1);
+    } else if (FULL) {
+      if (edge) F3D_WAIT_PLANE(20, Q1);
+      else F3D_WAIT_PLANE(11, Q1);
+    } else {
+      F3D_WAIT_PLANE(0, Q1);
+    }
+    if (FULL || z + 2 <= z1) plane_finish(Q1);
+    __builtin_amdgcn_sched_barrier(0);
+    if (owner) {
+      const unsigned off = xb + rowoff(yy, z);
+      gst(obase[0], off, kAddFlow ? C.u + r_du : r_du);
+      gst(obase[1], off, kAddFlow ? C.v + r_dv : r_dv);
+      gst(obase[2], off, kAddFlow ? C.w + r_dw : r_dw);
+    }
+    __builtin_amdgcn_sched_barrier(0);
+  };
+
+  PlaneRegs A, B, C, D, E;
+  E = PlaneRegs{};
+  D = PlaneRegs{};
+  load_plane(A, f3d_mir(z0 - 1, g.D));
+  load_plane(B, z0);
+  load_plane(C, f3d_mir(z0 + 1, g.D));
+  if (z0 + 2 <= z1) load_plane(D, f3d_mir(z0 + 2, g.D));
+  dma_halos(z0);
+  if (z0 + 1 < z1) dma_halos(z0 + 1);
+  if (z0 + 2 < z1) dma_halos(z0 + 2);
+  F3D_WAIT_PLANE(0, A);
+  F3D_WAIT_PLANE(0, B);
+  F3D_WAIT_PLANE(0, C);
+  F3D_WAIT_PLANE(0, D);
+  plane_finish(A);
+  plane_finish(B);
+  plane_finish(C);
+  __syncthreads();
+  publish(B, z0 & 1, z0 & (kRing - 1));
+  __builtin_amdgcn_sched_barrier(0);
+  int z = z0;
+  for (; z + 7 < z1; z += 5) {
+    step(std::true_type{}, A, B, C, D, E, z);
+    step(std::true_type{}, B, C, D, E, A, z + 1);
+    step(std::true_type{}, C, D, E, A, B, z + 2);
+    step(std::true_type{}, D, E, A, B, C, z + 3);
+    step(std::true_type{}, E, A, B, C, D, z + 4);
+  }
+  for (; z < z1; z += 5) {
+    step(std::false_type{}, A, B, C, D, E, z);
+    if (z + 1 < z1) step(std::false_type{}, B, C, D, E, A, z + 1);
+    if (z + 2 < z1) step(std::false_type{}, C, D, E, A, B, z + 2);
+    if (z + 3 < z1) step(std::false_type{}, D, E, A, B, C, z + 3);
+    if (z + 4 < z1) step(std::false_type{}, E, A, B, C, D, z + 4);
+  }
+  asm volatile("s_waitcnt vmcnt(0)" ::: "memory");
diff --git a/cuda-flow3d_amd/csrc/f3d_stream_ops.hip b/cuda-flow3d_amd/csrc/f3d_stream_ops.hip
--- a/cuda-flow3d_amd/csrc/f3d_stream_ops.hip
+++ b/cuda-flow3d_amd/csrc/f3d_stream_ops.hip
@@ -123,6 +123,77 @@
   }
 }
 
+typedef float Float4 __attribute__((ext_vector_type(4)));
+template <int KOUT, int NLOAD>
+__global__ __launch_bounds__(kBX* kBY) void k_resample_x_rows(Vols v, F3dGeo gi, F3dGeo g, int in_n, float delta, float normalization,
+                                                              int rows_per_wave, int row_floats)
+{
+  extern __shared__ __attribute__((aligned(16))) float rowbufs[];
+  const float* __restrict__ in = v.in[blockIdx.x];
+  float* __restrict__ out = v.out[blockIdx.x];
+  const int lane = threadIdx.x;
+  const int z = g.z_lo + blockIdx.z;
+  const int y0 = (blockIdx.y * kBY + threadIdx.y) * rows_per_wave;
+  if (y0 >= g.H) return;
+  const int y1 = min(y0 + rows_per_wave, g.H);
+  float* cur = rowbufs + threadIdx.y * 2 * row_floats;
+  float* nxt = cur + row_floats;
+
+  int left_i[KOUT], cnt[KOUT];
+  float frac_first[KOUT], frac_last[KOUT];
+#pragma unroll
+  for (int k = 0; k < KOUT; ++k) {
+    const int x = lane + k * kBX;
+    const float left_f = static_cast<float>(x) * delta;
+    const float right_f = static_cast<float>(x + 1) * delta;
+    left_i[k] = static_cast<int>(floorf(left_f));
+    const int right_i = static_cast<int>(fminf(static_cast<float>(in_n), ceilf(right_f)));
+    cnt[k] = x < g.W ? right_i - left_i[k] : 0;
+    frac_first[k] = cnt[k] == 1 ? delta : static_cast<float>(left_i[k] + 1) - left_f;
+    frac_last[k] = right_f - static_cast<float>(left_i[k] + cnt[k] - 1);
+  }
+
+  int piece[NLOAD];
+#pragma unroll
+  for (int i = 0; i < NLOAD; ++i) piece[i] = min((i * kBX + lane) * 4, row_floats - 4);
+  Float4 q[NLOAD];
+  {
+    const float* src = in + f3d_row(gi, y0, z);
+#pragma unroll
+    for (int i = 0; i < NLOAD; ++i) q[i] = *reinterpret_cast<const Float4*>(src + piece[i]);
+#pragma unroll
+    for (int i = 0; i < NLOAD; ++i)
+      if ((i * kBX + lane) * 4 < in_n) *reinterpret_cast<Float4*>(cur + piece[i]) = q[i];
+  }
+  for (int y = y0; y < y1; ++y) {
+    __builtin_amdgcn_fence(__ATOMIC_RELEASE, "wavefront", "local");
+    __builtin_amdgcn_wave_barrier();
+    __builtin_amdgcn_fence(__ATOMIC_ACQUIRE, "wavefront", "local");
+    const float* src = in + f3d_row(gi, min(y + 1, y1 - 1), z);
+#pragma unroll
+    for (int i = 0; i < NLOAD; ++i) q[i] = *reinterpret_cast<const Float4*>(src + piece[i]);
+    const size_t out_row = f3d_row(g, y, z);
+#pragma unroll
+    for (int k = 0; k < KOUT; ++k) {
+      const int x = lane + k * kBX;
+      float value = 0.f;
+      for (int j = 0; j < cnt[k]; ++j) {
+        float frac = 1.f;
+        if (j == cnt[k] - 1) frac = frac_last[k];
+        if (j == 0) frac = frac_first[k];
+        value = value + cur[left_i[k] + j] * frac;
+      }
+      if (x < g.W) out[out_row + x] = value * normalization;
+    }
+#pragma unroll
+    for (int i = 0; i < NLOAD; ++i)
+      if ((i * kBX + lane) * 4 < in_n) *reinterpret_cast<Float4*>(nxt + piece[i]) = q[i];
+    float* t = cur;
+    cur = nxt;
+    nxt = t;
+  }
+}
+
 template <int AXIS>
 __global__ __launch_bounds__(kBX* kBY) void k_resample_x4(Vols v, F3dGeo gi, F3dGeo g, int in_n, float delta, float normalization)
 {
@@ -392,7 +463,19 @@
   const float delta = static_cast<float>(n) / static_cast<float>(out_n);
   const float normalization = static_cast<float>(out_n) / static_cast<float>(n);
   const bool staged = x4 && n <= kResampleRowMax && (n + 3) / 4 * 4 <= gi.pitch;
-  if (axis == 0 && staged) hipLaunchKernelGGL(k_resample_x_lds, grid, block, 0, f3d::stream(), v, gi, g, n, delta, normalization);
+  const bool rows = axis == 0 && staged && n <= 1024 && g.W <= 1024;
+  if (rows) {
+    const long waves = static_cast<long>(count) * g.H * (g.z_hi - g.z_lo);
+    const int rpw = waves >= 8 * 16384 ? 8 : (waves >= 4 * 16384 ? 4 : (waves >= 2 * 16384 ? 2 : 1));
+    const int row_floats = (n + 3) / 4 * 4;
+    const dim3 grid_rows(static_cast<unsigned>(count), (g.H + kBY * rpw - 1) / (kBY * rpw), g.z_hi - g.z_lo);
+    const size_t lds = static_cast<size_t>(kBY) * 2 * row_floats * sizeof(float);
+    if (n <= 512 && g.W <= 512)
+      hipLaunchKernelGGL((k_resample_x_rows<8, 2>), grid_rows, block, lds, f3d::stream(), v, gi, g, n, delta, normalization, rpw, row_floats);
+    else
+      hipLaunchKernelGGL((k_resample_x_rows<16, 4>), grid_rows, block, lds, f3d::stream(), v, gi, g, n, delta, normalization, rpw, row_floats);
+  }
+  if (axis == 0 && staged && !rows) hipLaunchKernelGGL(k_resample_x_lds, grid, block, 0, f3d::stream(), v, gi, g, n, delta, normalization);
   if (axis == 0 && !staged) hipLaunchKernelGGL(k_resample<0>, grid, block, 0, f3d::stream(), v, gi, g, n, delta, normalization);
   if (axis == 1 && x4) hipLaunchKernelGGL(k_resample_x4<1>, grid, block, 0, f3d::stream(), v, gi, g, n, delta, normalization);
   if (axis == 2 && x4) hipLaunchKernelGGL(k_resample_x4<2>, grid, block, 0, f3d::stream(), v, gi, g, n, delta, normalization);
diff --git a/cuda-flow3d_amd/host/operations.cpp b/cuda-flow3d_amd/host/operations.cpp
--- a/cuda-flow3d_amd/host/operations.cpp
+++ b/cuda-flow3d_amd/host/operations.cpp
@@ -7,6 +7,11 @@
 
 #include "common_utils.h"
 #include "hip_utils.h"
+
+extern "C" int f3d_solve_sweep_add(f3d_devptr frame_0, f3d_devptr frame_1, f3d_devptr flow_u, f3d_devptr flow_v, f3d_devptr flow_w,
+                                   f3d_devptr flow_du, f3d_devptr flow_dv, f3d_devptr flow_dw, f3d_devptr phi, f3d_devptr ksi,
+                                   size_t width, size_t height, size_t depth, float hx, float hy, float hz, float equation_alpha,
+                                   f3d_devptr sum_u, f3d_devptr sum_v, f3d_devptr sum_w, const f3d_slab* slab) __attribute__((weak));
 
 
 bool CudaOperationBase::IsInitialized() const
@@ -443,6 +448,8 @@
   GET_PARAM_OR_RETURN(params, float, hz, "hz");
   GET_PARAM_OR_RETURN(params, DataSize4, data_size, "data_size");
   NoteSolveWeights(equation_alpha, hx, hy, hz);
+  bool* flow_update = static_cast<bool*>(params.GetValuePtr("flow_update"));
+  if (flow_update) *flow_update = false;
 
   {
     const DevicePtr increments[3] = {*du_ptr, *dv_ptr, *dw_ptr};
@@ -539,7 +546,11 @@
         status = f3d_solve_sweep_phi_ksi(dev_frame_0, dev_frame_1, dev_flow_u, dev_flow_v, dev_flow_w, *du_ptr, *dv_ptr, *dw_ptr,
                                          phi_cur, ksi_cur, w, h, d, hx, hy, hz, equation_alpha, equation_smoothness, equation_data,
                                          *tdu_ptr, *tdv_ptr, *tdw_ptr, phi_nxt, ksi_nxt, slab_);
-      else
+      else if (flow_update && f3d_solve_sweep_add && !more && j + 1 == inner_iterations_count) {
+        status = f3d_solve_sweep_add(dev_frame_0, dev_frame_1, dev_flow_u, dev_flow_v, dev_flow_w, *du_ptr, *dv_ptr, *dw_ptr, phi_cur,
+                                     ksi_cur, w, h, d, hx, hy, hz, equation_alpha, *tdu_ptr, *tdv_ptr, *tdw_ptr, slab_);
+        *flow_update = status == 0;
+      } else
         status = f3d_solve_sweep(dev_frame_0, dev_frame_1, dev_flow_u, dev_flow_v, dev_flow_w, *du_ptr, *dv_ptr, *dw_ptr, phi_cur,
                                  ksi_cur, w, h, d, hx, hy, hz, equation_alpha, *tdu_ptr, *tdv_ptr, *tdw_ptr, slab_);
       if (CheckDeviceError(status)) return;
diff --git a/cuda-flow3d_amd/host/operator_calls.h b/cuda-flow3d_amd/host/operator_calls.h
--- a/cuda-flow3d_amd/host/operator_calls.h
+++ b/cuda-flow3d_amd/host/operator_calls.h
@@ -49,6 +49,15 @@
                        {"equation_data", s.data}, {"data_size", size}, {"hx", h.hx}, {"hy", h.hy}, {"hz", h.hz}});
 }
 
+inline OperationParameters& SolveAndUpdate(OperationParameters& bag, DevicePtr* frame_0, DevicePtr* frame_1_registered, const Flow& flow,
+                                           const Flow& increment, const Flow& partner, DevicePtr* phi, DevicePtr* ksi,
+                                           const SolverSettings& s, DataSize4* size, const Spacing& h, bool* flow_updated)
+{
+  Solve(bag, frame_0, frame_1_registered, flow, increment, partner, phi, ksi, s, size, h);
+  bag.PushValuePtr("flow_update", flow_updated);
+  return bag;
+}
+
 inline OperationParameters& Add(OperationParameters& bag, DevicePtr* accumulator, DevicePtr* addend, DataSize4* size)
 {
   return FillBag(bag, {{"operand_0", accumulator}, {"operand_1", addend}, {"data_size", size}});
diff --git a/cuda-flow3d_amd/host/optical_flow.cpp b/cuda-flow3d_amd/host/optical_flow.cpp
--- a/cuda-flow3d_amd/host/optical_flow.cpp
+++ b/cuda-flow3d_amd/host/optical_flow.cpp
@@ -744,23 +744,29 @@
       level_stats_.push_back(st);
     }
 
+    bool flow_updated = false;
     {
       DevicePtr phi = Borrow(), ksi = Borrow();
       DevicePtr partner[3] = {Borrow(), Borrow(), Borrow()};
       const calls::Flow partner_roles = {&partner[0], &partner[1], &partner[2]};
       cuop_solve_.silent = silent;
-      cuop_solve_.Execute(calls::Solve(bag, &level_frame[0], &level_frame[1], flow_roles, step_roles, partner_roles, &phi, &ksi, settings,
-                                       &box, spacing));
+      cuop_solve_.Execute(calls::SolveAndUpdate(bag, &level_frame[0], &level_frame[1], flow_roles, step_roles, partner_roles, &phi, &ksi,
+                                                settings, &box, spacing, &flow_updated));
       for (DevicePtr p : {phi, ksi, partner[0], partner[1], partner[2]}) GiveBack(p);
     }
 
     {
       OperationParameters bags[3];
-      for (int c = 0; c < 3; ++c) calls::Add(bags[c], &flow[c], &step[c], &box);
-      cuop_add_.ExecuteBatch(bags, 3);
-      for (int c = 0; c < 3; ++c) calls::Median(bags[c], &flow[c], &step[c], &box, &median_radius);
-      cuop_median_.ExecuteBatch(bags, 3);
-      for (int c = 0; c < 3; ++c) std::swap(flow[c], step[c]);
+      if (flow_updated) {
+        for (int c = 0; c < 3; ++c) calls::Median(bags[c], &step[c], &flow[c], &box, &median_radius);
+        cuop_median_.ExecuteBatch(bags, 3);
+      } else {
+        for (int c = 0; c < 3; ++c) calls::Add(bags[c], &flow[c], &step[c], &box);
+        cuop_add_.ExecuteBatch(bags, 3);
+        for (int c = 0; c < 3; ++c) calls::Median(bags[c], &flow[c], &step[c], &box, &median_radius);
+        cuop_median_.ExecuteBatch(bags, 3);
+        for (int c = 0; c < 3; ++c) std::swap(flow[c], step[c]);
+      }
     }
 
     if (collect_level_statistics) {
diff --git a/include/f3d.h b/include/f3d.h
--- a/include/f3d.h
+++ b/include/f3d.h
@@ -96,6 +96,11 @@
                     f3d_devptr flow_du, f3d_devptr flow_dv, f3d_devptr flow_dw, f3d_devptr phi, f3d_devptr ksi,
                     size_t width, size_t height, size_t depth, float hx, float hy, float hz, float equation_alpha,
                     f3d_devptr temp_du, f3d_devptr temp_dv, f3d_devptr temp_dw, const f3d_slab* slab);
+
+int f3d_solve_sweep_add(f3d_devptr frame_0, f3d_devptr frame_1, f3d_devptr flow_u, f3d_devptr flow_v, f3d_devptr flow_w,
+                        f3d_devptr flow_du, f3d_devptr flow_dv, f3d_devptr flow_dw, f3d_devptr phi, f3d_devptr ksi,
+                        size_t width, size_t height, size_t depth, float hx, float hy, float hz, float equation_alpha,
+                        f3d_devptr sum_u, f3d_devptr sum_v, f3d_devptr sum_w, const f3d_slab* slab);
 
 int f3d_solve_sweep2(f3d_devptr frame_0, f3d_devptr frame_1, f3d_devptr flow_u, f3d_devptr flow_v, f3d_devptr flow_w,
                      f3d_devptr flow_du, f3d_devptr flow_dv, f3d_devptr flow_dw, f3d_devptr phi, f3d_devptr ksi,
```

New measurement: 73.80 Mvoxels/s (median of 6 runs). +1.0%, better.
